# trinhvg/MoMA

Measured on AMD Instinct MI355X. Metric: images/sec MoMA train step (EffNet-B0 224px, K=65536), higher is better.
Workload: dtype bf16

## Files before the change

include/moma_hip.h:

```cpp
#ifndef MOMA_HIP_H
#define MOMA_HIP_H

#include <stddef.h>
#include <stdint.h>

#ifdef __cplusplus
extern "C" {
#endif

#define MOMA_ABI_VERSION 4

enum { MOMA_PREC_F32 = 0, MOMA_PREC_BF16 = 1 };
enum { MOMA_DT_F32 = 0, MOMA_DT_BF16 = 1 };

enum {
    MOMA_OK = 0,
    MOMA_E_NULL = -1,
    MOMA_E_SHAPE = -2,
    MOMA_E_DTYPE = -3,
    MOMA_E_ALIGN = -4,
    MOMA_E_WORKSPACE = -5,
    MOMA_E_UNSUPPORTED = -6
};

typedef void* moma_stream_t;

int moma_version(void);
const char* moma_error_string(int code);
int moma_debug_set_k2_target_wg(int n);

#define MOMA_EMA_BLOCK_ELEMS 4096
int moma_ema_multi(const int64_t* table, int n_tensors, int64_t total_blocks,
                   float m, float one_minus_m, moma_stream_t stream);

int moma_enqueue(void* queue, const float* rows, int n, int64_t index, int K, int d,
                 int qdtype, moma_stream_t stream);
int moma_enqueue_mirror(float* queue, void* mirror_bf16, const float* rows, int n, int64_t index, int K, int d,
                        moma_stream_t stream);

int moma_queue_prefetch(const void* queue, size_t bytes, moma_stream_t stream);

int moma_infonce_logits(const float* q, const float* k, const void* queue, float* out,
                        int B, int d, int K, float inv_T, int qdtype, int prec, moma_stream_t stream);
int moma_infonce_logits_bwd(const float* dlogits, const float* k, const void* queue, float* dq,
                            int B, int d, int K, float inv_T, int qdtype, int prec,
                            moma_stream_t stream);
size_t moma_infonce_logits_bwd_workspace_bytes(int B, int d, int K);
int moma_infonce_logits_bwd_ws(const float* dlogits, const float* k, const void* queue, float* dq,
                               int B, int d, int K, float inv_T, int qdtype, int prec,
                               void* workspace, size_t workspace_bytes, moma_stream_t stream);
int moma_infonce_logits_bwd_kq(const float* dlogits, const float* q, float* dk, float* dqueue,
                               int B, int d, int K, float inv_T, int prec, moma_stream_t stream);
size_t moma_infonce_fused_workspace_bytes(int B, int d, int K, int qdtype, int prec);
int moma_infonce_fused(const float* q, const float* k, const void* queue, int B, int d, int K,
                       float inv_T, float* loss_rows, float* lse, int32_t* top1, float* dq,
                       void* workspace, size_t workspace_bytes, int qdtype, int prec,
                       moma_stream_t stream);
int moma_infonce_fused_ex(const float* q, const float* k, const void* queue, int B, int d, int K,
                          float inv_T, float* loss_rows, float* lse, int32_t* top1, float* dq,
                          void* workspace, size_t workspace_bytes, int qdtype, int prec,
                          moma_stream_t stream, void* ev_begin, void* ev_end);
size_t moma_infonce_qpack_bytes(int B, int d);
int moma_infonce_fused_q(const float* q, const void* q_packed, const float* k, const void* queue, int B, int d, int K,
                         float inv_T, float* loss_rows, float* lse, int32_t* top1, float* dq,
                         void* workspace, size_t workspace_bytes, int qdtype, int prec,
                         moma_stream_t stream, void* ev_begin, void* ev_end, void* ev_call_end);
int moma_infonce_fused_enqueue(const float* q, const void* q_packed, const float* k, void* queue, int B, int d, int K,
                               float inv_T, float* loss_rows, float* lse, int32_t* top1, float* dq, void* workspace,
                               size_t workspace_bytes, int qdtype, int prec, const float* rows, int n, int64_t index,
                               float* queue_f32, moma_stream_t stream, void* ev_begin, void* ev_end, void* ev_call_end);

typedef struct moma_infonce_term {
    const float* q;
    const float* k;
    const void* queue;
    float* loss_rows;
    float* lse;
    int32_t* top1;
    float* dq;
} moma_infonce_term_t;
size_t moma_infonce_fused_multi_workspace_bytes(int n_terms, int B, int d, int K, int qdtype, int prec);
int moma_infonce_fused_multi(const moma_infonce_term_t* terms, int n_terms, int B, int d, int K, float inv_T,
                             void* workspace, size_t workspace_bytes, int qdtype, int prec, moma_stream_t stream);

size_t moma_crd_workspace_bytes(int B, int d, int K1);
int moma_crd_fused(const float* v1, const float* v2, const float* memory_v1, const float* memory_v2, const int64_t* idx,
                   int B, int d, int K1, int64_t n_data, float T, float* Z, int set_z, float* loss, float* dv1, float* dv2,
                   int32_t* bad_index, void* workspace, size_t workspace_bytes, moma_stream_t stream);
int moma_crd_scores(const float* v1, const float* v2, const float* memory_v1, const float* memory_v2, const int64_t* idx,
                    int B, int d, int K1, int64_t n_data, float T, float* Z, int set_z, float* out_v1, float* out_v2,
                    int32_t* bad_index, void* workspace, size_t workspace_bytes, moma_stream_t stream);
int moma_crd_scores_bwd(const float* dout_v1, const float* dout_v2, const float* out_v1, const float* out_v2,
                        const float* memory_v1, const float* memory_v2, const int64_t* idx, int B, int d, int K1,
                        int64_t n_data, float T, float* dv1, float* dv2, int32_t* bad_index, void* workspace,
                        size_t workspace_bytes, moma_stream_t stream);
int moma_crd_update(float* memory_v1, float* memory_v2, const float* v1, const float* v2, const int64_t* y, int B, int d,
                    int64_t n_data, float momentum, int32_t* bad_index, moma_stream_t stream);

enum { MOMA_LAYOUT_NCHW = 0, MOMA_LAYOUT_NHWC = 1 };
size_t moma_at_workspace_bytes(int B, int C, int H, int W, int oh, int ow, int dtype, int layout);
int moma_at_map(const void* f, float* a, int B, int C, int H, int W, int oh, int ow, int dtype, int layout, void* workspace,
                size_t workspace_bytes, moma_stream_t stream);
int moma_at_pair(const float* a_s, const float* a_t, int B, int n, float* norms, float* partials, float* loss, float* g_s,
                 float* g_t, float* ah_s, float* ah_t, moma_stream_t stream);
int moma_at_bwd(const void* f, const float* g_a, const float* g_loss, void* dF, int B, int C, int H, int W, int oh, int ow,
                int dtype, int layout, moma_stream_t stream);

enum { MOMA_MHA_SAVE_PROBS = 0, MOMA_MHA_SAVE_LSE = 1 };
int moma_mha_saved_state(int N, int d, int H, int prec);
int moma_mha_fwd(const float* x, const float* w_qkv, const float* b_qkv, const float* w_proj,
                 const float* b_proj, float* y, float* qkv, float* probs, float* attn_out,
                 int N, int d, int H, int prec, moma_stream_t stream);
size_t moma_mha_bwd_workspace_bytes(int N, int d, int H, int prec);
int moma_mha_bwd(const float* x, const float* w_qkv, const float* w_proj, const float* qkv,
                 const float* probs, const float* attn_out, const float* dy, float* dx,
                 float* dw_qkv, float* db_qkv, float* dw_proj, float* db_proj, void* workspace,
                 size_t workspace_bytes, int N, int d, int H, int prec, moma_stream_t stream);

typedef struct moma_mha_module {
    const void* x;
    const void* pack;
    const float* b_qkv;
    const float* b_proj;
    float* y;
    void* qkv16;
    void* attn16;
    float* lse;
    void* qpack;
    float qpack_scale;
    int x_dtype;
} moma_mha_module_t;
size_t moma_mha_pack_bytes(int d);
int moma_mha_pack_weights(const float* w_qkv, const float* w_proj, void* pack, int d, int with_transposed,
                          moma_stream_t stream);
int moma_mha_fwd_fast(const moma_mha_module_t* modules, int n_modules, int N, int d, int H, moma_stream_t stream);
size_t moma_mha_bwd_fast_workspace_bytes(int N, int d, int H);
int moma_mha_bwd_fast(const void* pack, const void* x, int x_dtype, const void* qkv16, const void* attn16, const float* lse,
                      const float* dy, float* dx, float* dw_qkv, float* db_qkv, float* dw_proj, float* db_proj,
                      void* workspace, size_t workspace_bytes, int N, int d, int H, moma_stream_t stream);

enum { MOMA_ACT_NONE = 0, MOMA_ACT_SILU = 1, MOMA_ACT_RELU = 2 };
size_t moma_bn_workspace_bytes(int C);
int moma_bn_fwd(const void* x, void* out, const float* gamma, const float* beta, float* running_mean,
                float* running_var, float* save_mean, float* save_invstd, void* workspace,
                size_t workspace_bytes, int N, int C, int HW, int dtype, int act, int training,
                float momentum, float eps, void* plane_mean, moma_stream_t stream);
int moma_bn_bwd(const void* x, const void* dout, const float* gamma, const float* beta,
                const float* save_mean, const float* save_invstd, void* dx, float* dgamma, float* dbeta,
                void* workspace, size_t workspace_bytes, int N, int C, int HW, int dtype, int act,
                int training, const void* dplane_mean, moma_stream_t stream);

size_t moma_dwconv_workspace_bytes(int C, int K);
int moma_dwconv_fwd(const void* x, const float* w, void* y, int N, int C, int H, int W, int OH, int OW,
                    int K, int stride, int pad_top, int pad_left, int dtype, moma_stream_t stream);
int moma_dwconv_bwd_data(const void* dy, const float* w, void* dx, int N, int C, int H, int W, int OH,
                         int OW, int K, int stride, int pad_top, int pad_left, int dtype,
                         moma_stream_t stream);
int moma_dwconv_bwd_weight(const void* x, const void* dy, float* dw, void* workspace,
                           size_t workspace_bytes, int N, int C, int H, int W, int OH, int OW, int K,
                           int stride, int pad_top, int pad_left, int dtype, moma_stream_t stream);

int moma_plane_mean(const void* x, void* mean, int NC, int HW, int dtype, moma_stream_t stream);
int moma_se_gate_fwd(const void* x, const void* s, void* out, int NC, int HW, int dtype, moma_stream_t stream);
int moma_se_gate_bwd(const void* x, const void* s, const void* dout, void* dx, void* ds, int NC, int HW,
                     int dtype, moma_stream_t stream);

#ifdef __cplusplus
}
#endif
#endif
```

moma_amd/_lib.py:

```python
from __future__ import annotations

import ctypes as C
import os

_HERE = os.path.dirname(os.path.abspath(__file__))
LIB_PATH = os.environ.get("MOMA_HIP_LIB", os.path.join(_HERE, "lib", "libmoma_hip.so"))

PREC_F32, PREC_BF16 = 0, 1
DT_F32, DT_BF16 = 0, 1
LAYOUT_NCHW, LAYOUT_NHWC = 0, 1
MHA_SAVE_PROBS, MHA_SAVE_LSE = 0, 1
ABI_VERSION = 4
EMA_BLOCK_ELEMS = 4096

_p = C.c_void_p
_i = C.c_int
_l = C.c_int64
_f = C.c_float
_z = C.c_size_t

SIGNATURES = {
    "moma_version": (_i, []),
    "moma_error_string": (C.c_char_p, [_i]),
    "moma_debug_set_k2_target_wg": (_i, [_i]),
    "moma_ema_multi": (_i, [_p, _i, _l, _f, _f, _p]),
    "moma_enqueue": (_i, [_p, _p, _i, _l, _i, _i, _i, _p]),
    "moma_enqueue_mirror": (_i, [_p, _p, _p, _i, _l, _i, _i, _p]),
    "moma_queue_prefetch": (_i, [_p, _z, _p]),
    "moma_infonce_logits": (_i, [_p, _p, _p, _p, _i, _i, _i, _f, _i, _i, _p]),
    "moma_infonce_logits_bwd": (_i, [_p, _p, _p, _p, _i, _i, _i, _f, _i, _i, _p]),
    "moma_infonce_logits_bwd_workspace_bytes": (_z, [_i, _i, _i]),
    "moma_infonce_logits_bwd_ws": (_i, [_p, _p, _p, _p, _i, _i, _i, _f, _i, _i, _p, _z, _p]),
    "moma_infonce_logits_bwd_kq": (_i, [_p, _p, _p, _p, _i, _i, _i, _f, _i, _p]),
    "moma_infonce_fused_workspace_bytes": (_z, [_i, _i, _i, _i, _i]),
    "moma_infonce_fused": (_i, [_p, _p, _p, _i, _i, _i, _f, _p, _p, _p, _p, _p, _z, _i, _i, _p]),
    "moma_infonce_fused_ex": (_i, [_p, _p, _p, _i, _i, _i, _f, _p, _p, _p, _p, _p, _z, _i, _i, _p, _p, _p]),
    "moma_infonce_qpack_bytes": (_z, [_i, _i]),
    "moma_infonce_fused_q": (_i, [_p, _p, _p, _p, _i, _i, _i, _f, _p, _p, _p, _p, _p, _z, _i, _i, _p, _p, _p, _p]),
    "moma_infonce_fused_enqueue": (_i, [_p, _p, _p, _p, _i, _i, _i, _f, _p, _p, _p, _p, _p, _z, _i, _i, _p, _i, _l, _p, _p, _p, _p, _p]),
    "moma_infonce_fused_multi_workspace_bytes": (_z, [_i, _i, _i, _i, _i, _i]),
    "moma_infonce_fused_multi": (_i, [_p, _i, _i, _i, _i, _f, _p, _z, _i, _i, _p]),
    "moma_crd_workspace_bytes": (_z, [_i, _i, _i]),
    "moma_crd_fused": (_i, [_p, _p, _p, _p, _p, _i, _i, _i, _l, _f, _p, _i, _p, _p, _p, _p, _p, _z, _p]),
    "moma_crd_scores": (_i, [_p, _p, _p, _p, _p, _i, _i, _i, _l, _f, _p, _i, _p, _p, _p, _p, _z, _p]),
    "moma_crd_scores_bwd": (_i, [_p, _p, _p, _p, _p, _p, _p, _i, _i, _i, _l, _f, _p, _p, _p, _p, _z, _p]),
    "moma_crd_update": (_i, [_p, _p, _p, _p, _p, _i, _i, _l, _f, _p, _p]),
    "moma_at_workspace_bytes": (_z, [_i] * 8),
    "moma_at_map": (_i, [_p, _p] + [_i] * 8 + [_p, _z, _p]),
    "moma_at_pair": (_i, [_p, _p, _i, _i, _p, _p, _p, _p, _p, _p, _p, _p]),
    "moma_at_bwd": (_i, [_p, _p, _p, _p] + [_i] * 8 + [_p]),
    "moma_mha_fwd": (_i,[_p, _p, _p, _p, _p, _p, _p, _p, _p, _i, _i, _i, _i, _p]),
    "moma_mha_saved_state": (_i, [_i, _i, _i, _i]),
    "moma_mha_pack_bytes": (_z, [_i]),
    "moma_mha_pack_weights": (_i, [_p, _p, _p, _i, _i, _p]),
    "moma_mha_fwd_fast": (_i, [_p, _i, _i, _i, _i, _p]),
    "moma_mha_bwd_fast_workspace_bytes": (_z, [_i, _i, _i]),
    "moma_mha_bwd_fast": (_i, [_p, _p, _i, _p, _p, _p, _p, _p, _p, _p, _p, _p, _p, _z, _i, _i, _i, _p]),
    "moma_dwconv_workspace_bytes": (_z, [_i, _i]),
    "moma_dwconv_fwd": (_i, [_p, _p, _p] + [_i] * 11 + [_p]),
    "moma_dwconv_bwd_data": (_i, [_p, _p, _p] + [_i] * 11 + [_p]),
    "moma_dwconv_bwd_weight": (_i, [_p, _p, _p, _p, _z] + [_i] * 11 + [_p]),
    "moma_plane_mean": (_i, [_p, _p, _i, _i, _i, _p]),
    "moma_se_gate_fwd": (_i, [_p, _p, _p, _i, _i, _i, _p]),
    "moma_se_gate_bwd": (_i, [_p, _p, _p, _p, _p, _i, _i, _i, _p]),
    "moma_bn_workspace_bytes": (_z, [_i]),
    "moma_bn_fwd": (_i, [_p, _p, _p, _p, _p, _p, _p, _p, _p, _z, _i, _i, _i, _i, _i, _i, _f, _f, _p, _p]),
    "moma_bn_bwd": (_i, [_p, _p, _p, _p, _p, _p, _p, _p, _p, _p, _z, _i, _i, _i, _i, _i, _i, _p, _p]),
    "moma_mha_bwd_workspace_bytes": (_z, [_i, _i, _i, _i]),
    "moma_mha_bwd": (_i, [_p, _p, _p, _p, _p, _p, _p, _p, _p, _p, _p, _p, _p, _z, _i, _i, _i, _i, _p]),
}



class InfoNCETerm(C.Structure):
    _fields_ = [("q", _p), ("k", _p), ("queue", _p), ("loss_rows", _p), ("lse", _p), ("top1", _p), ("dq", _p)]


class MhaModule(C.Structure):
    _fields_ = [("x", _p), ("pack", _p), ("b_qkv", _p), ("b_proj", _p), ("y", _p), ("qkv16", _p), ("attn16", _p),
                ("lse", _p), ("qpack", _p), ("qpack_scale", _f), ("x_dtype", _i)]


_lib = None


class MomaHipError(RuntimeError):
    pass


def load():
    global _lib
    if _lib is not None:
        return _lib
    import torch
    if not os.path.exists(LIB_PATH):
        raise MomaHipError(
            f"libmoma_hip.so not found at {LIB_PATH}: build it with `python -m moma_amd.build` "
            "(hipcc --offload-arch=gfx950). There is no CPU fallback for the MoMA hot path.")
    lib = C.CDLL(LIB_PATH)
    for name, (res, args) in SIGNATURES.items():
        try:
            fn = getattr(lib, name)
        except AttributeError as e:
            raise MomaHipError(f"{LIB_PATH} does not export {name}") from e
        fn.restype = res
        fn.argtypes = args
    v = lib.moma_version()
    if v != ABI_VERSION:
        raise MomaHipError(f"libmoma_hip ABI version {v} != binding version {ABI_VERSION}; rebuild")
    _lib = lib
    return lib


def check(rc: int, what: str):
    if rc != 0:
        msg = load().moma_error_string(rc)
        raise MomaHipError(f"{what} failed: rc={rc} ({msg.decode() if msg else '?'})")
```

moma_amd/backbones/efficientnet.py:

```python
import math
import os

import torch
import torch.nn as nn
import torch.nn.functional as F

_DW_MODE = os.environ.get("MOMA_DW", "hip")
_BN_MODE = os.environ.get("MOMA_BN", "hip")
_SE_MODE = os.environ.get("MOMA_SE", "hip")

_B0_STAGES = [
    (1, 3, 1, 1, 32, 16, 0.25),
    (2, 3, 2, 6, 16, 24, 0.25),
    (2, 5, 2, 6, 24, 40, 0.25),
    (3, 3, 2, 6, 40, 80, 0.25),
    (3, 5, 1, 6, 80, 112, 0.25),
    (4, 5, 2, 6, 112, 192, 0.25),
    (1, 3, 1, 6, 192, 320, 0.25),
]
_BN_MOM, _BN_EPS = 0.01, 1e-3


class _DepthwiseNative(torch.autograd.Function):

    @staticmethod
    def forward(ctx, x, w, stride, padding, groups):
        w = w.to(x.dtype)
        with torch.backends.cudnn.flags(enabled=False):
            y = F.conv2d(x, w, None, stride, padding, 1, groups)
        ctx.save_for_backward(x, w)
        ctx.cfg = (stride, padding, groups)
        return y

    @staticmethod
    def backward(ctx, gy):
        x, w = ctx.saved_tensors
        stride, padding, groups = ctx.cfg
        pad = padding if isinstance(padding, (tuple, list)) else (padding, padding)
        with torch.backends.cudnn.flags(enabled=False):
            gx, gw, _ = torch.ops.aten.convolution_backward(
                gy.contiguous(), x, w, None, list(stride), list(pad), [1, 1], False, [0, 0], groups,
                [ctx.needs_input_grad[0], ctx.needs_input_grad[1], False])
        return gx, (gw.float() if gw is not None else None), None, None, None


class _CachedCast(torch.autograd.Function):

    @staticmethod
    def forward(ctx, master, cached):
        ctx.dtype = master.dtype
        return cached.view_as(cached)

    @staticmethod
    def backward(ctx, g):
        return g.to(ctx.dtype), None


_WCACHE = os.environ.get("MOMA_WCACHE", "1") == "1"


class SamePadConv2d(nn.Conv2d):

    def __init__(self, cin, cout, kernel_size, stride=1, groups=1, bias=True):
        super().__init__(cin, cout, kernel_size, stride=stride, padding=0, groups=groups, bias=bias)
        self._wc = self._bc = None
        self._wc_live = False

    def _params(self, x):
        if self._wc_live and x.is_cuda and x.dtype == torch.bfloat16:
            track = torch.is_grad_enabled()
            w = _CachedCast.apply(self.weight, self._wc) if (track and self.weight.requires_grad) else self._wc
            b = None
            if self.bias is not None:
                b = _CachedCast.apply(self.bias, self._bc) if (track and self.bias.requires_grad) else self._bc
            return w, b
        return self.weight, self.bias

    def forward(self, x):
        ih, iw = x.shape[-2:]
        kh, kw = self.kernel_size
        sh, sw = self.stride
        ph = max((math.ceil(ih / sh) - 1) * sh + kh - ih, 0)
        pw = max((math.ceil(iw / sw) - 1) * sw + kw - iw, 0)
        depthwise = self.groups > 1 and self.groups == self.in_channels == self.out_channels and self.bias is None
        if depthwise and x.is_cuda and _DW_MODE == "hip" and kh == kw and sh == sw and self.dilation == (1, 1):
            from .. import ops
            if ops.dwconv_supported(kh, sh):
                if torch.is_autocast_enabled():
                    x = x.to(torch.get_autocast_dtype("cuda"))
                if x.dtype in (torch.float32, torch.bfloat16):
                    return ops.dwconv(x, self.weight, sh, ph // 2, pw // 2, math.ceil(ih / sh), math.ceil(iw / sw))
        pad = (ph // 2, pw // 2)
        if ph % 2 or pw % 2:
            x = F.pad(x, [pw // 2, pw - pw // 2, ph // 2, ph - ph // 2])
            pad = 0
        if depthwise and x.is_cuda and _DW_MODE in ("hip", "aten"):
            if torch.is_autocast_enabled():
                x = x.to(torch.get_autocast_dtype("cuda"))
            return _DepthwiseNative.apply(x, self.weight, self.stride, pad, self.groups)
        if self._wc_live and torch.is_autocast_enabled() and x.is_cuda and x.dtype != torch.bfloat16 and \
                torch.get_autocast_dtype("cuda") == torch.bfloat16:
            x = x.to(torch.bfloat16)
        w, b = self._params(x)
        return F.conv2d(x, w, b, self.stride, pad, self.dilation, self.groups)


class BatchNorm2d(nn.BatchNorm2d):

    _nbt_pending = 0

    def _flush_nbt(self):
        if self._nbt_pending and self.num_batches_tracked is not None:
            self.num_batches_tracked.add_(self._nbt_pending)
        self._nbt_pending = 0

    def _save_to_state_dict(self, destination, prefix, keep_vars):
        self._flush_nbt()
        super()._save_to_state_dict(destination, prefix, keep_vars)

    def _load_from_state_dict(self, *args, **kwargs):
        self._nbt_pending = 0
        super()._load_from_state_dict(*args, **kwargs)

    def forward(self, x, act=None, want_mean=False):
        if _BN_MODE == "hip" and x.is_cuda and x.dtype in (torch.float32, torch.bfloat16) and self.momentum is not None:
            from .. import ops
            use_batch = self.training or self.running_mean is None
            if self.training and self.track_running_stats and self.num_batches_tracked is not None:
                self._nbt_pending += 1
            return ops.bn_act(x, self.weight, self.bias, self.running_mean, self.running_var, use_batch,
                              self.momentum, self.eps, act, want_mean)
        if _BN_MODE == "aten" and x.is_cuda:
            with torch.backends.cudnn.flags(enabled=False):
                y = super().forward(x)
        else:
            y = super().forward(x)
        y = F.silu(y) if act == "silu" else (F.relu(y) if act == "relu" else y)
        return (y, F.adaptive_avg_pool2d(y, 1)) if want_mean else y


def _drop_connect(x, p, training):
    if not training or not p:
        return x
    keep = 1.0 - p
    mask = torch.floor(keep + torch.rand([x.shape[0], 1, 1, 1], dtype=x.dtype, device=x.device))
    return x / keep * mask


class MBConvBlock(nn.Module):
    def __init__(self, kernel, stride, expand, cin, cout, se_ratio):
        super().__init__()
        mid = cin * expand
        self.expand, self.stride, self.cin, self.cout = expand, stride, cin, cout
        if expand != 1:
            self._expand_conv = SamePadConv2d(cin, mid, 1, bias=False)
            self._bn0 = BatchNorm2d(mid, momentum=_BN_MOM, eps=_BN_EPS)
        self._depthwise_conv = SamePadConv2d(mid, mid, kernel, stride=stride, groups=mid, bias=False)
        self._bn1 = BatchNorm2d(mid, momentum=_BN_MOM, eps=_BN_EPS)
        sq = max(1, int(cin * se_ratio))
        self._se_reduce = SamePadConv2d(mid, sq, 1)
        self._se_expand = SamePadConv2d(sq, mid, 1)
        self._project_conv = SamePadConv2d(mid, cout, 1, bias=False)
        self._bn2 = BatchNorm2d(cout, momentum=_BN_MOM, eps=_BN_EPS)

    def forward(self, x, drop_connect_rate=None):
        inp = x
        if self.expand != 1:
            x = self._bn0(self._expand_conv(x), act="silu")
        x, pooled = self._bn1(self._depthwise_conv(x), act="silu", want_mean=True)
        s = self._se_expand(F.silu(self._se_reduce(pooled)))
        if _SE_MODE == "hip" and x.is_cuda and x.dtype in (torch.float32, torch.bfloat16):
            from .. import ops
            x = ops.se_gate(x, s)
        else:
            x = torch.sigmoid(s) * x
        x = self._bn2(self._project_conv(x))
        if self.stride == 1 and self.cin == self.cout:
            x = _drop_connect(x, drop_connect_rate, self.training) + inp
        return x


class EfficientNet(nn.Module):
    def __init__(self, num_classes=1000, dropout_rate=0.2, drop_connect_rate=0.2, in_channels=3):
        super().__init__()
        self.drop_connect_rate = drop_connect_rate
        self._conv_stem = SamePadConv2d(in_channels, 32, 3, stride=2, bias=False)
        self._bn0 = BatchNorm2d(32, momentum=_BN_MOM, eps=_BN_EPS)
        blocks = []
        for rep, k, s, e, cin, cout, se in _B0_STAGES:
            blocks.append(MBConvBlock(k, s, e, cin, cout, se))
            blocks += [MBConvBlock(k, 1, e, cout, cout, se) for _ in range(rep - 1)]
        self._blocks = nn.ModuleList(blocks)
        self._conv_head = SamePadConv2d(320, 1280, 1, bias=False)
        self._bn1 = BatchNorm2d(1280, momentum=_BN_MOM, eps=_BN_EPS)
        self._avg_pooling = nn.AdaptiveAvgPool2d(1)
        self.classifier_ = nn.Sequential(nn.Dropout(dropout_rate), nn.Linear(1280, num_classes))
        for m in self.modules():
            if isinstance(m, nn.Conv2d):
                nn.init.kaiming_normal_(m.weight, mode="fan_out")
                if m.bias is not None:
                    nn.init.zeros_(m.bias)
            elif isinstance(m, nn.BatchNorm2d):
                nn.init.ones_(m.weight)
                nn.init.zeros_(m.bias)
            elif isinstance(m, nn.Linear):
                nn.init.normal_(m.weight, 0, 0.01)
                nn.init.zeros_(m.bias)

    def extract_endpoints(self, x):
        feats = []
        x = self._bn0(self._conv_stem(x), act="silu")
        prev = x
        nb = len(self._blocks)
        for i, blk in enumerate(self._blocks):
            rate = self.drop_connect_rate * float(i) / nb if self.drop_connect_rate else self.drop_connect_rate
            x = blk(x, drop_connect_rate=rate)
            if prev.size(2) > x.size(2):
                feats.append(prev)
            prev = x
        feats.append(self._bn1(self._conv_head(x), act="silu"))
        return feats

    def get_feat_modules(self):
        return nn.ModuleList([self._conv_stem, self._bn0, self._blocks, self._conv_head, self._bn1, self.classifier_])

    def _refresh_weight_cache(self, x):
        live = (_WCACHE and x.is_cuda and torch.is_autocast_enabled() and torch.get_autocast_dtype("cuda") == torch.bfloat16)
        convs = getattr(self, "_wcache_convs", None)
        if convs is None:
            convs = [m for m in self.modules() if isinstance(m, SamePadConv2d) and not (m.groups > 1 and _DW_MODE == "hip")]
            object.__setattr__(self, "_wcache_convs", convs)
        if not live:
            for m in convs:
                m._wc_live = False
            return
        src, dst = [], []
        for m in convs:
            if m._wc is None or m._wc.device != m.weight.device:
                m._wc = torch.empty_like(m.weight, dtype=torch.bfloat16)
                m._bc = torch.empty_like(m.bias, dtype=torch.bfloat16) if m.bias is not None else None
            src.append(m.weight.detach()); dst.append(m._wc)
            if m.bias is not None:
                src.append(m.bias.detach()); dst.append(m._bc)
            m._wc_live = True
        with torch.no_grad():
            torch._foreach_copy_(dst, src)

    def forward(self, x, is_feat=False):
        self._refresh_weight_cache(x)
        out = self.extract_endpoints(x)
        pooled = self._avg_pooling(out[-1])
        out.append(pooled)
        logits = self.classifier_(pooled.flatten(start_dim=1))
        for m in self._wcache_convs:
            m._wc_live = False
        return (out, logits) if is_feat else logits


def efficientnet_b0(num_classes=1000, **kw):
    return EfficientNet(num_classes=num_classes, **kw)
```

moma_amd/csrc/api.hip:

```cpp
#include "common.hpp"

using namespace moma;

namespace {
inline int hip_rc(hipError_t e) { return e == hipSuccess ? MOMA_OK : (int)e; }
inline bool bad_prec(int p) { return p != MOMA_PREC_F32 && p != MOMA_PREC_BF16; }
inline bool bad_dt(int t) { return t != MOMA_DT_F32 && t != MOMA_DT_BF16; }
inline bool misaligned(const void* p, size_t a) { return ((uintptr_t)p % a) != 0; }
inline size_t align_up(size_t x, size_t a) { return (x + a - 1) / a * a; }

#define MOMA_TRY(expr)                         \
    do {                                       \
        hipError_t _e = (expr);                \
        if (_e != hipSuccess) return (int)_e;  \
    } while (0)

GemmArgs gemm(const float* A, const void* B, float* C, int M, int N, int K, long lda, long ldb, long ldc, int tA,
              int tB, float alpha, int prec) {
    GemmArgs g{};
    g.A = A; g.B = B; g.C = C; g.bias = nullptr;
    g.M = M; g.N = N; g.K = K; g.lda = lda; g.ldb = ldb; g.ldc = ldc;
    g.strideA = g.strideB = g.strideC = 0; g.batch = 1;
    g.transA = tA; g.transB = tB; g.alpha = alpha; g.splitk = 1; g.atomic = 0; g.splitC = 0;
    g.b_dtype = MOMA_DT_F32; g.prec = prec;
// ... 134 lines not shown
    }
    return MOMA_OK;
}

static bool f32_policy_widens_queue(int B, int d, int K, int qdtype, int prec) {
    return prec == MOMA_PREC_F32 && qdtype == MOMA_DT_BF16 && infonce_f32_flash_supported(B, d, K, MOMA_DT_F32, prec);
}

size_t moma_infonce_fused_workspace_bytes(int B, int d, int K, int qdtype, int prec) {
    if (B <= 0 || d <= 0 || K <= 0) return 0;
    if (infonce_flash_supported(B, d, K, qdtype, prec)) return infonce_flash_workspace_bytes(B, d, K);
    if (infonce_f32_flash_supported(B, d, K, qdtype, prec)) return infonce_f32_flash_workspace_bytes(B, d, K);
    if (f32_policy_widens_queue(B, d, K, qdtype, prec))
        return align_up((size_t)K * d * sizeof(float), 256) + infonce_f32_flash_workspace_bytes(B, d, K);
    return align_up((size_t)B * ((size_t)K + 1) * sizeof(float), 256) + logits_bwd_parts_bytes(B, d, K);
}

int moma_infonce_fused(const float* q, const float* k, const void* queue, int B, int d, int K, float inv_T,
                       float* loss_rows, float* lse, int32_t* top1, float* dq, void* workspace,
                       size_t workspace_bytes, int qdtype, int prec, moma_stream_t stream) {
    return moma_infonce_fused_ex(q, k, queue, B, d, K, inv_T, loss_rows, lse, top1, dq, workspace, workspace_bytes,
                                 qdtype, prec, stream, nullptr, nullptr);
}

int moma_infonce_fused_ex(const float* q, const float* k, const void* queue, int B, int d, int K, float inv_T,
                          float* loss_rows, float* lse, int32_t* top1, float* dq, void* workspace,
                          size_t workspace_bytes, int qdtype, int prec, moma_stream_t stream, void* ev_begin,
                          void* ev_end) {
    return moma_infonce_fused_q(q, nullptr, k, queue, B, d, K, inv_T, loss_rows, lse, top1, dq, workspace, workspace_bytes,
                                qdtype, prec, stream, ev_begin, ev_end, nullptr);
}

size_t moma_infonce_qpack_bytes(int B, int d) { return infonce_qpack_bytes(B, d); }

static int fused_impl(const float* q, const void* q_packed, const float* k, const void* queue, int B, int d, int K,
                      float inv_T, float* loss_rows, float* lse, int32_t* top1, float* dq, void* workspace,
                      size_t workspace_bytes, int qdtype, int prec, moma_stream_t stream, void* ev_begin, void* ev_end,
                      void* ev_call_end, const EnqueueJob* job, int* carried) {
    if (carried) *carried = 0;
    if (!q || !k || !queue || !loss_rows || !lse || !top1 || !workspace) return MOMA_E_NULL;
    if (B <= 0 || d <= 0 || K <= 0) return MOMA_E_SHAPE;
    if (bad_dt(qdtype) || bad_prec(prec)) return MOMA_E_DTYPE;
    if (workspace_bytes < moma_infonce_fused_workspace_bytes(B, d, K, qdtype, prec)) return MOMA_E_WORKSPACE;
    if (misaligned(workspace, 16)) return MOMA_E_ALIGN;
    hipStream_t st = (hipStream_t)stream;
    if (q_packed && (misaligned(q_packed, 16) || infonce_qpack_bytes(B, d) == 0 || !infonce_flash_supported(B, d, K, qdtype, prec)))
        return q_packed && misaligned(q_packed, 16) ? MOMA_E_ALIGN : MOMA_E_UNSUPPORTED;
    const bool one_pass = infonce_flash_supported(B, d, K, qdtype, prec) || infonce_f32_flash_supported(B, d, K, qdtype, prec) ||
                          f32_policy_widens_queue(B, d, K, qdtype, prec);
    if (one_pass && (misaligned(q, 16) || misaligned(k, 16) || misaligned(queue, 16) || (dq && misaligned(dq, 16)))) return MOMA_E_ALIGN;
    if (!one_pass && (misaligned(q, 4) || misaligned(k, 4) || misaligned(queue, qdtype == MOMA_DT_BF16 ? 2 : 4) || (dq && misaligned(dq, 4))))
        return MOMA_E_ALIGN;
    if (infonce_flash_supported(B, d, K, qdtype, prec)) {
        if (carried) *carried = 1;
        return hip_rc(launch_infonce_flash(q, k, queue, B, d, K, inv_T, loss_rows, lse, top1, dq, workspace, qdtype, st,
                                           (hipEvent_t)ev_begin, (hipEvent_t)ev_end, q_packed, (hipEvent_t)ev_call_end, job));
    }
    if (infonce_f32_flash_supported(B, d, K, qdtype, prec))
    {
        const int rc = hip_rc(launch_infonce_f32_flash(q, k, (const float*)queue, B, d, K, inv_T, loss_rows, lse, top1, dq, workspace, st,
                                                       (hipEvent_t)ev_begin, (hipEvent_t)ev_end));
        if (ev_call_end) (void)hipEventRecord((hipEvent_t)ev_call_end, st);
        return rc;
    }
    if (f32_policy_widens_queue(B, d, K, qdtype, prec)) {
        if (misaligned(queue, 16)) return MOMA_E_ALIGN;
        float* wide = (float*)workspace;
        void* ws2 = (char*)workspace + align_up((size_t)K * d * sizeof(float), 256);
        if (ev_begin) (void)hipEventRecord((hipEvent_t)ev_begin, st);
        MOMA_TRY(launch_widen_bf16(queue, wide, (size_t)K * d, st));
        const int rc = hip_rc(launch_infonce_f32_flash(q, k, wide, B, d, K, inv_T, loss_rows, lse, top1, dq, ws2, st,
                                                       (hipEvent_t) nullptr, (hipEvent_t)ev_end));
        if (ev_call_end) (void)hipEventRecord((hipEvent_t)ev_call_end, st);
        return rc;
    }
    float* logits = (float*)workspace;
    if (ev_begin) (void)hipEventRecord((hipEvent_t)ev_begin, st);
    int rc = moma_infonce_logits(q, k, queue, logits, B, d, K, inv_T, qdtype, prec, stream);
    if (ev_end) (void)hipEventRecord((hipEvent_t)ev_end, st);
    if (rc != MOMA_OK) return rc;
    MOMA_TRY(launch_infonce_rows(logits, B, K + 1, loss_rows, lse, top1, dq != nullptr, st));
    if (dq) {
        float* parts = (float*)((char*)workspace + align_up((size_t)B * ((size_t)K + 1) * sizeof(float), 256));
        rc = logits_bwd_impl(logits, k, queue, dq, B, d, K, inv_T, qdtype, prec, st, logits_bwd_parts_bytes(B, d, K) ? parts : nullptr);
    }
    if (ev_call_end) (void)hipEventRecord((hipEvent_t)ev_call_end, st);
    return rc;
}

int moma_infonce_fused_q(const float* q, const void* q_packed, const float* k, const void* queue, int B, int d, int K,
                         float inv_T, float* loss_rows, float* lse, int32_t* top1, float* dq, void* workspace,
                         size_t workspace_bytes, int qdtype, int prec, moma_stream_t stream, void* ev_begin, void* ev_end,
                         void* ev_call_end) {
    return fused_impl(q, q_packed, k, queue, B, d, K, inv_T, loss_rows, lse, top1, dq, workspace, workspace_bytes, qdtype, prec, stream,
                      ev_begin, ev_end, ev_call_end, nullptr, nullptr);
}

int moma_infonce_fused_enqueue(const float* q, const void* q_packed, const float* k, void* queue, int B, int d, int K,
                               float inv_T, float* loss_rows, float* lse, int32_t* top1, float* dq, void* workspace,
                               size_t workspace_bytes, int qdtype, int prec, const float* rows, int n, int64_t index,
                               float* queue_f32, moma_stream_t stream, void* ev_begin, void* ev_end, void* ev_call_end) {
    if (n < 0 || K <= 0 || index < 0 || index >= K) return MOMA_E_SHAPE;
    if (n > 0 && !rows) return MOMA_E_NULL;
    if (bad_dt(qdtype)) return MOMA_E_DTYPE;
    if (queue_f32 && qdtype != MOMA_DT_BF16) return MOMA_E_DTYPE;
    if (n > 0 && (misaligned(rows, 4) || misaligned(queue, qdtype == MOMA_DT_BF16 ? 2 : 4) || (queue_f32 && misaligned(queue_f32, 4))))
        return MOMA_E_ALIGN;
    EnqueueJob job{qdtype == MOMA_DT_BF16 ? queue : nullptr, qdtype == MOMA_DT_BF16 ? queue_f32 : (float*)queue, rows, n, index, K, d};
    int carried = 0;
    const int rc = fused_impl(q, q_packed, k, queue, B, d, K, inv_T, loss_rows, lse, top1, dq, workspace, workspace_bytes, qdtype, prec,
                              stream, ev_begin, ev_end, ev_call_end, n > 0 ? &job : nullptr, &carried);
    if (rc != MOMA_OK || carried || n == 0) return rc;
    if (queue_f32) return hip_rc(launch_enqueue_mirror(queue_f32, queue, rows, n, index, K, d, (hipStream_t)stream));
    return hip_rc(launch_enqueue(queue, rows, n, index, K, d, qdtype, (hipStream_t)stream));
}

size_t moma_infonce_fused_multi_workspace_bytes(int n_terms, int B, int d, int K, int qdtype, int prec) {
    if (n_terms < 1 || n_terms > 4 || B <= 0 || d <= 0 || K <= 0 || bad_dt(qdtype) || bad_prec(prec)) return 0;
    if (infonce_multi_supported(n_terms, B, d, K, qdtype, prec)) return infonce_multi_workspace_bytes(n_terms, B, d, K);
    return moma_infonce_fused_workspace_bytes(B, d, K, qdtype, prec);
}

int moma_infonce_fused_multi(const moma_infonce_term_t* terms, int n_terms, int B, int d, int K, float inv_T, void* workspace,
                             size_t workspace_bytes, int qdtype, int prec, moma_stream_t stream) {
    if (!terms || !workspace) return MOMA_E_NULL;
    if (n_terms < 1 || n_terms > 4 || B <= 0 || d <= 0 || K <= 0) return MOMA_E_SHAPE;
    if (bad_dt(qdtype) || bad_prec(prec)) return MOMA_E_DTYPE;
    for (int i = 0; i < n_terms; ++i) {
        const moma_infonce_term_t& t = terms[i];
        if (!t.q || !t.k || !t.queue || !t.loss_rows || !t.lse || !t.top1) return MOMA_E_NULL;
        if ((t.dq != nullptr) != (terms[0].dq != nullptr)) return MOMA_E_UNSUPPORTED;
        if (misaligned(t.q, 16) || misaligned(t.k, 4) || misaligned(t.queue, 16)) return MOMA_E_ALIGN;
    }
    if (workspace_bytes < moma_infonce_fused_multi_workspace_bytes(n_terms, B, d, K, qdtype, prec)) return MOMA_E_WORKSPACE;
    if (misaligned(workspace, 16)) return MOMA_E_ALIGN;
    if (infonce_multi_supported(n_terms, B, d, K, qdtype, prec))
        return hip_rc(launch_infonce_multi(terms, n_terms, B, d, K, inv_T, workspace, (hipStream_t)stream));
    for (int i = 0; i < n_terms; ++i) {
        const moma_infonce_term_t& t = terms[i];
        const int rc = moma_infonce_fused_q(t.q, nullptr, t.k, t.queue, B, d, K, inv_T, t.loss_rows, t.lse, t.top1, t.dq, workspace,
                                            workspace_bytes, qdtype, prec, stream, nullptr, nullptr, nullptr);
        if (rc != MOMA_OK) return rc;
    }
    return MOMA_OK;
}

int moma_mha_saved_state(int N, int d, int H, int prec) {
    if (N <= 0 || d <= 0 || H <= 0 || d % H != 0 || bad_prec(prec)) return MOMA_E_SHAPE;
    return mha_fast_supported(N, d, H, prec) ? MOMA_MHA_SAVE_LSE : MOMA_MHA_SAVE_PROBS;
}

int moma_mha_fwd(const float* x, const float* w_qkv, const float* b_qkv, const float* w_proj, const float* b_proj,
                 float* y, float* qkv, float* probs, float* attn_out, int N, int d, int H, int prec,
                 moma_stream_t stream) {
    if (!x || !w_qkv || !w_proj || !b_proj || !y || !qkv || !attn_out || !probs) return MOMA_E_NULL;
    if (N <= 0 || d <= 0 || H <= 0 || d % H != 0) return MOMA_E_SHAPE;
    if (bad_prec(prec)) return MOMA_E_DTYPE;
    hipStream_t st = (hipStream_t)stream;
    const int hd = d / H;
    const float scale = 1.0f / sqrtf((float)hd);
    GemmArgs g = gemm(x, w_qkv, qkv, N, 3 * d, d, d, d, 3L * d, 0, 0, 1.f, prec);
    g.bias = b_qkv;
    MOMA_TRY(launch_gemm(g, st));
    g = gemm(qkv, qkv + d, probs, N, N, hd, 3L * d, 3L * d, N, 0, 0, scale, prec);
    g.batch = H; g.strideA = hd; g.strideB = hd; g.strideC = (long)N * N;
    MOMA_TRY(launch_gemm(g, st));
    MOMA_TRY(launch_softmax_rows(probs, (long)H * N, N, st));
    g = gemm(probs, qkv + 2 * d, attn_out, N, hd, N, N, 3L * d, d, 0, 1, 1.f, prec);
    g.batch = H; g.strideA = (long)N * N; g.strideB = hd; g.strideC = hd;
    MOMA_TRY(launch_gemm(g, st));
    g = gemm(attn_out, w_proj, y, N, d, d, d, d, d, 0, 0, 1.f, prec);
    g.bias = b_proj;
    return hip_rc(launch_gemm(g, st));
}

size_t moma_mha_bwd_workspace_bytes(int N, int d, int H, int prec) {
    if (N <= 0 || d <= 0 || H <= 0 || d % H != 0 || bad_prec(prec)) return 0;
    return align_up(((size_t)N * d + (size_t)H * N * N + (size_t)N * 3 * d) * sizeof(float), 256);
}

int moma_mha_bwd(const float* x, const float* w_qkv, const float* w_proj, const float* qkv, const float* probs,
                 const float* attn_out, const float* dy, float* dx, float* dw_qkv, float* db_qkv,
                 float* dw_proj, float* db_proj, void* workspace, size_t workspace_bytes, int N, int d, int H, int prec,
                 moma_stream_t stream) {
    if (!x || !w_qkv || !w_proj || !qkv || !attn_out || !dy || !workspace || !probs) return MOMA_E_NULL;
    if (N <= 0 || d <= 0 || H <= 0 || d % H != 0) return MOMA_E_SHAPE;
    if (bad_prec(prec)) return MOMA_E_DTYPE;
    if (workspace_bytes < moma_mha_bwd_workspace_bytes(N, d, H, prec)) return MOMA_E_WORKSPACE;
    if (misaligned(workspace, 16)) return MOMA_E_ALIGN;
    hipStream_t st = (hipStream_t)stream;
    const int hd = d / H;
    const float scale = 1.0f / sqrtf((float)hd);
    float* dA = (float*)workspace;
    float* dP = dA + (size_t)N * d;
    float* dqkv = dP + (size_t)H * N * N;
    GemmArgs g;
    bool db_done = false;
    if (dw_proj) {
        g = gemm(dy, attn_out, dw_proj, d, d, N, d, d, d, 1, 1, 1.f, prec);
        if (db_proj && gemm_fuses_colsum(g)) { g.colsum_a = db_proj; db_done = true; }
        MOMA_TRY(launch_gemm(g, st));
    }
    if (db_proj && !db_done) MOMA_TRY(launch_colsum(dy, db_proj, N, d, d, st));
    g = gemm(dy, w_proj, dA, N, d, d, d, d, d, 0, 1, 1.f, prec);
    MOMA_TRY(launch_gemm(g, st));
    g = gemm(probs, dA, dqkv + 2 * d, N, hd, N, N, d, 3L * d, 1, 1, 1.f, prec);
    g.batch = H; g.strideA = (long)N * N; g.strideB = hd; g.strideC = hd;
    MOMA_TRY(launch_gemm(g, st));
    g = gemm(dA, qkv + 2 * d, dP, N, N, hd, d, 3L * d, N, 0, 0, 1.f, prec);
    g.batch = H; g.strideA = hd; g.strideB = hd; g.strideC = (long)N * N;
    MOMA_TRY(launch_gemm(g, st));
    MOMA_TRY(launch_softmax_bwd_rows(probs, dP, (long)H * N, N, scale, st));
    g = gemm(dP, qkv + d, dqkv, N, hd, N, N, 3L * d, 3L * d, 0, 1, 1.f, prec);
    g.batch = H; g.strideA = (long)N * N; g.strideB = hd; g.strideC = hd;
    MOMA_TRY(launch_gemm(g, st));
    g = gemm(dP, qkv, dqkv + d, N, hd, N, N, 3L * d, 3L * d, 1, 1, 1.f, prec);
    g.batch = H; g.strideA = (long)N * N; g.strideB = hd; g.strideC = hd;
    MOMA_TRY(launch_gemm(g, st));
    db_done = false;
    if (dw_qkv) {
        g = gemm(dqkv, x, dw_qkv, 3 * d, d, N, 3L * d, d, d, 1, 1, 1.f, prec);
        if (db_qkv && gemm_fuses_colsum(g)) { g.colsum_a = db_qkv; db_done = true; }
        MOMA_TRY(launch_gemm(g, st));
    }
    if (db_qkv && !db_done) MOMA_TRY(launch_colsum(dqkv, db_qkv, N, 3 * d, 3L * d, st));
    if (dx) {
        g = gemm(dqkv, w_qkv, dx, N, d, 3 * d, 3L * d, d, d, 0, 1, 1.f, prec);
        MOMA_TRY(launch_gemm(g, st));
    }
    return MOMA_OK;
}

size_t moma_mha_pack_bytes(int d) { return d > 0 ? (size_t)16 * d * d : 0; }

int moma_mha_pack_weights(const float* w_qkv, const float* w_proj, void* pack, int d, int with_transposed,
                          moma_stream_t stream) {
    if (!w_qkv || !w_proj || !pack) return MOMA_E_NULL;
    if (d <= 0 || d % 16 != 0) return MOMA_E_SHAPE;
    if (misaligned(pack, 16) || misaligned(w_qkv, 4) || misaligned(w_proj, 4)) return MOMA_E_ALIGN;
    return hip_rc(launch_mha_pack(w_qkv, w_proj, pack, d, with_transposed != 0, (hipStream_t)stream));
}

int moma_mha_fwd_fast(const moma_mha_module_t* mods, int n_modules, int N, int d, int H, moma_stream_t stream) {
    if (!mods) return MOMA_E_NULL;
    if (n_modules < 1 || n_modules > 4 || N <= 0 || d <= 0 || H <= 0 || d % H != 0) return MOMA_E_SHAPE;
    if (!mha_fast_supported(N, d, H, MOMA_PREC_BF16)) return MOMA_E_UNSUPPORTED;
    for (int i = 0; i < n_modules; ++i) {
        const moma_mha_module_t& m = mods[i];
        if (!m.x || !m.pack || !m.b_proj || !m.y || !m.qkv16 || !m.attn16) return MOMA_E_NULL;
        if (bad_dt(m.x_dtype)) return MOMA_E_DTYPE;
        if (misaligned(m.x, 16) || misaligned(m.pack, 16) || misaligned(m.y, 16) || misaligned(m.qkv16, 16) ||
            misaligned(m.attn16, 16) || misaligned(m.b_proj, 16) || (m.b_qkv && misaligned(m.b_qkv, 16)) ||
            (m.qpack && misaligned(m.qpack, 16)))
            return MOMA_E_ALIGN;
    }
    return hip_rc(launch_mha_fwd_fast(mods, n_modules, N, d, H, (hipStream_t)stream));
}

size_t moma_mha_bwd_fast_workspace_bytes(int N, int d, int H) {
    if (N <= 0 || d <= 0 || H <= 0 || d % H != 0) return 0;
    return mha_bwd_fast_workspace_bytes(N, d);
}

int moma_mha_bwd_fast(const void* pack, const void* x, int x_dtype, const void* qkv16, const void* attn16, const float* lse,
                      const float* dy, float* dx, float* dw_qkv, float* db_qkv, float* dw_proj, float* db_proj,
                      void* workspace, size_t workspace_bytes, int N, int d, int H, moma_stream_t stream) {
    if (!pack || !x || !qkv16 || !attn16 || !lse || !dy || !workspace) return MOMA_E_NULL;
    if (N <= 0 || d <= 0 || H <= 0 || d % H != 0) return MOMA_E_SHAPE;
    if (!mha_fast_supported(N, d, H, MOMA_PREC_BF16)) return MOMA_E_UNSUPPORTED;
    if (bad_dt(x_dtype)) return MOMA_E_DTYPE;
    if ((db_qkv && !dw_qkv) || (db_proj && !dw_proj)) return MOMA_E_UNSUPPORTED;
    if (workspace_bytes < mha_bwd_fast_workspace_bytes(N, d)) return MOMA_E_WORKSPACE;
    if (misaligned(workspace, 16) || misaligned(pack, 16) || misaligned(x, 16) || misaligned(qkv16, 16) ||
        misaligned(attn16, 16) || misaligned(dy, 16) || (dx && misaligned(dx, 16)) || (dw_qkv && misaligned(dw_qkv, 8)) ||
        (dw_proj && misaligned(dw_proj, 8)))
        return MOMA_E_ALIGN;
    return hip_rc(launch_mha_bwd_fast(pack, x, x_dtype, qkv16, attn16, lse, dy, dx, dw_qkv, db_qkv, dw_proj, db_proj, workspace, N, d,
                                      H, (hipStream_t)stream));
}

size_t moma_bn_workspace_bytes(int C) { return C > 0 ? align_up(bn_workspace_floats(C) * sizeof(float), 256) : 0; }

static int bn_check(int N, int C, int HW, int dtype, int act, const void* ws, size_t ws_bytes) {
    if (N <= 0 || C <= 0 || HW <= 0 || (long)N * C > 0x7fffffffL || (long)N * HW > 0x7fffffffL) return MOMA_E_SHAPE;
    if (dtype != MOMA_DT_F32 && dtype != MOMA_DT_BF16) return MOMA_E_DTYPE;
    if (act != MOMA_ACT_NONE && act != MOMA_ACT_SILU && act != MOMA_ACT_RELU) return MOMA_E_DTYPE;
    if (!ws) return MOMA_E_NULL;
    if (ws_bytes < moma_bn_workspace_bytes(C)) return MOMA_E_WORKSPACE;
    return MOMA_OK;
}

int moma_bn_fwd(const void* x, void* out, const float* gamma, const float* beta, float* running_mean,
                float* running_var, float* save_mean, float* save_invstd, void* workspace, size_t workspace_bytes,
                int N, int C, int HW, int dtype, int act, int training, float momentum, float eps, void* plane_mean,
                moma_stream_t stream) {
    if (!x || !out) return MOMA_E_NULL;
    if (!training && (!running_mean || !running_var)) return MOMA_E_NULL;
    const int rc = bn_check(N, C, HW, dtype, act, workspace, workspace_bytes);
    if (rc != MOMA_OK) return rc;
    return hip_rc(launch_bn_fwd(x, out, gamma, beta, running_mean, running_var, save_mean, save_invstd,
                                (float*)workspace, N, C, HW, dtype, act, training, momentum, eps, plane_mean, (hipStream_t)stream));
}

int moma_bn_bwd(const void* x, const void* dout, const float* gamma, const float* beta, const float* save_mean,
                const float* save_invstd, void* dx, float* dgamma, float* dbeta, void* workspace,
                size_t workspace_bytes, int N, int C, int HW, int dtype, int act, int training,
                const void* dplane_mean, moma_stream_t stream) {
    if (!x || !dout || !save_mean || !save_invstd) return MOMA_E_NULL;
    const int rc = bn_check(N, C, HW, dtype, act, workspace, workspace_bytes);
    if (rc != MOMA_OK) return rc;
    return hip_rc(launch_bn_bwd(x, dout, gamma, beta, save_mean, save_invstd, dx, dgamma, dbeta, (float*)workspace, N,
                                C, HW, dtype, act, training, dplane_mean, (hipStream_t)stream));
}

size_t moma_dwconv_workspace_bytes(int C, int K) {
    return (C > 0 && K > 0) ? align_up(dwconv_workspace_floats(C, K) * sizeof(float), 256) : 0;
}

static int dw_check(int N, int C, int H, int W, int OH, int OW, int K, int S, int pt, int pl, int dtype) {
    if (N <= 0 || C <= 0 || H <= 0 || W <= 0 || OH <= 0 || OW <= 0 || (long)N * C > 0x7fffffffL) return MOMA_E_SHAPE;
    if (!dwconv_supported(K, S)) return MOMA_E_SHAPE;
    if (pt < 0 || pl < 0 || pt >= K || pl >= K) return MOMA_E_SHAPE;
    if ((long)(OH - 1) * S - pt >= H || (long)(OW - 1) * S - pl >= W) return MOMA_E_SHAPE;
    if (dtype != MOMA_DT_F32 && dtype != MOMA_DT_BF16) return MOMA_E_DTYPE;
    return MOMA_OK;
}

int moma_dwconv_fwd(const void* x, const float* w, void* y, int N, int C, int H, int W, int OH, int OW, int K, int stride,
                    int pad_top, int pad_left, int dtype, moma_stream_t stream) {
    if (!x || !w || !y) return MOMA_E_NULL;
    const int rc = dw_check(N, C, H, W, OH, OW, K, stride, pad_top, pad_left, dtype);
    if (rc != MOMA_OK) return rc;
    return hip_rc(launch_dw_fwd(x, w, y, N, C, H, W, OH, OW, K, stride, pad_top, pad_left, dtype, (hipStream_t)stream));
}

int moma_dwconv_bwd_data(const void* dy, const float* w, void* dx, int N, int C, int H, int W, int OH, int OW, int K,
                         int stride, int pad_top, int pad_left, int dtype, moma_stream_t stream) {
    if (!dy || !w || !dx) return MOMA_E_NULL;
    const int rc = dw_check(N, C, H, W, OH, OW, K, stride, pad_top, pad_left, dtype);
    if (rc != MOMA_OK) return rc;
    return hip_rc(launch_dw_bwd_data(dy, w, dx, N, C, H, W, OH, OW, K, stride, pad_top, pad_left, dtype, (hipStream_t)stream));
}

int moma_dwconv_bwd_weight(const void* x, const void* dy, float* dw, void* workspace, size_t workspace_bytes, int N, int C,
                           int H, int W, int OH, int OW, int K, int stride, int pad_top, int pad_left, int dtype,
                           moma_stream_t stream) {
    if (!x || !dy || !dw || !workspace) return MOMA_E_NULL;
    const int rc = dw_check(N, C, H, W, OH, OW, K, stride, pad_top, pad_left, dtype);
    if (rc != MOMA_OK) return rc;
    if (workspace_bytes < moma_dwconv_workspace_bytes(C, K)) return MOMA_E_WORKSPACE;
    return hip_rc(launch_dw_bwd_weight(x, dy, dw, (float*)workspace, workspace_bytes / sizeof(float), N, C, H, W, OH, OW, K,
                                       stride, pad_top, pad_left, dtype, (hipStream_t)stream));
}

static int se_check(int NC, int HW, int dtype) {
    if (NC <= 0 || HW <= 0) return MOMA_E_SHAPE;
    if (dtype != MOMA_DT_F32 && dtype != MOMA_DT_BF16) return MOMA_E_DTYPE;
    return MOMA_OK;
}
int moma_plane_mean(const void* x, void* mean, int NC, int HW, int dtype, moma_stream_t stream) {
    if (!x || !mean) return MOMA_E_NULL;
    const int rc = se_check(NC, HW, dtype);
    return rc != MOMA_OK ? rc : hip_rc(launch_plane_mean(x, mean, NC, HW, dtype, (hipStream_t)stream));
}
int moma_se_gate_fwd(const void* x, const void* s, void* out, int NC, int HW, int dtype, moma_stream_t stream) {
    if (!x || !s || !out) return MOMA_E_NULL;
    const int rc = se_check(NC, HW, dtype);
    return rc != MOMA_OK ? rc : hip_rc(launch_se_gate_fwd(x, s, out, NC, HW, dtype, (hipStream_t)stream));
}
int moma_se_gate_bwd(const void* x, const void* s, const void* dout, void* dx, void* ds, int NC, int HW, int dtype,
                     moma_stream_t stream) {
    if (!x || !s || !dout || !dx || !ds) return MOMA_E_NULL;
    const int rc = se_check(NC, HW, dtype);
    return rc != MOMA_OK ? rc : hip_rc(launch_se_gate_bwd(x, s, dout, dx, ds, NC, HW, dtype, (hipStream_t)stream));
}

static int crd_check(int B, int d, int K1, int64_t n_data, float T) {
    if (B <= 0 || d < 4 || d % 4 != 0 || K1 < 2 || n_data <= 0 || !(T > 0.f)) return MOMA_E_SHAPE;
    if (d > 2048 || B > 65535) return MOMA_E_UNSUPPORTED;
    return MOMA_OK;
}
static bool crd_misaligned(const void* a, const void* b, const void* c, const void* d, const void* e = nullptr,
                           const void* f = nullptr, const void* g = nullptr, const void* h = nullptr) {
    return misaligned(a, 16) || misaligned(b, 16) || misaligned(c, 16) || misaligned(d, 16) || misaligned(e, 16) ||
           misaligned(f, 16) || misaligned(g, 16) || misaligned(h, 16);
}

size_t moma_crd_workspace_bytes(int B, int d, int K1) {
    if (crd_check(B, d, K1, 1, 1.f) != MOMA_OK) return 0;
    return crd_workspace_bytes(B, d, K1);
}

int moma_crd_fused(const float* v1, const float* v2, const float* memory_v1, const float* memory_v2, const int64_t* idx,
                   int B, int d, int K1, int64_t n_data, float T, float* Z, int set_z, float* loss, float* dv1, float* dv2,
                   int32_t* bad_index, void* workspace, size_t workspace_bytes, moma_stream_t stream) {
    if (!v1 || !v2 || !memory_v1 || !memory_v2 || !idx || !Z || !loss || !bad_index || !workspace) return MOMA_E_NULL;
    if ((dv1 == nullptr) != (dv2 == nullptr)) return MOMA_E_NULL;
    const int rc = crd_check(B, d, K1, n_data, T);
    if (rc != MOMA_OK) return rc;
    if (crd_misaligned(v1, v2, memory_v1, memory_v2, dv1, dv2, workspace) || misaligned(idx, 8) || misaligned(Z, 4) ||
        misaligned(loss, 4) || misaligned(bad_index, 4))
        return MOMA_E_ALIGN;
    if (workspace_bytes < crd_workspace_bytes(B, d, K1)) return MOMA_E_WORKSPACE;
    return hip_rc(launch_crd_fused(v1, v2, memory_v1, memory_v2, idx, B, d, K1, n_data, T, Z, set_z, loss, dv1, dv2, bad_index,
                                   workspace, (hipStream_t)stream));
}

int moma_crd_scores(const float* v1, const float* v2, const float* memory_v1, const float* memory_v2, const int64_t* idx,
                    int B, int d, int K1, int64_t n_data, float T, float* Z, int set_z, float* out_v1, float* out_v2,
                    int32_t* bad_index, void* workspace, size_t workspace_bytes, moma_stream_t stream) {
    if (!v1 || !v2 || !memory_v1 || !memory_v2 || !idx || !Z || !out_v1 || !out_v2 || !bad_index || !workspace) return MOMA_E_NULL;
    const int rc = crd_check(B, d, K1, n_data, T);
    if (rc != MOMA_OK) return rc;
    if (crd_misaligned(v1, v2, memory_v1, memory_v2, workspace) || misaligned(idx, 8) || misaligned(Z, 4) ||
        misaligned(out_v1, 4) || misaligned(out_v2, 4) || misaligned(bad_index, 4))
        return MOMA_E_ALIGN;
    if (workspace_bytes < crd_workspace_bytes(B, d, K1)) return MOMA_E_WORKSPACE;
    return hip_rc(launch_crd_scores(v1, v2, memory_v1, memory_v2, idx, B, d, K1, n_data, T, Z, set_z, out_v1, out_v2, bad_index,
                                    workspace, (hipStream_t)stream));
}

int moma_crd_scores_bwd(const float* dout_v1, const float* dout_v2, const float* out_v1, const float* out_v2,
                        const float* memory_v1, const float* memory_v2, const int64_t* idx, int B, int d, int K1,
                        int64_t n_data, float T, float* dv1, float* dv2, int32_t* bad_index, void* workspace,
                        size_t workspace_bytes, moma_stream_t stream) {
    if (!dout_v1 || !dout_v2 || !out_v1 || !out_v2 || !memory_v1 || !memory_v2 || !idx || !dv1 || !dv2 || !bad_index || !workspace)
        return MOMA_E_NULL;
    const int rc = crd_check(B, d, K1, n_data, T);
    if (rc != MOMA_OK) return rc;
    if (crd_misaligned(memory_v1, memory_v2, dv1, dv2, workspace) || misaligned(idx, 8) || misaligned(dout_v1, 4) ||
        misaligned(dout_v2, 4) || misaligned(out_v1, 4) || misaligned(out_v2, 4) || misaligned(bad_index, 4))
        return MOMA_E_ALIGN;
    if (workspace_bytes < crd_workspace_bytes(B, d, K1)) return MOMA_E_WORKSPACE;
    return hip_rc(launch_crd_scores_bwd(dout_v1, dout_v2, out_v1, out_v2, memory_v1, memory_v2, idx, B, d, K1, n_data, T, dv1, dv2,
                                        bad_index, workspace, (hipStream_t)stream));
}

int moma_crd_update(float* memory_v1, float* memory_v2, const float* v1, const float* v2, const int64_t* y, int B, int d,
                    int64_t n_data, float momentum, int32_t* bad_index, moma_stream_t stream) {
    if (!memory_v1 || !memory_v2 || !v1 || !v2 || !y || !bad_index) return MOMA_E_NULL;
    if (B <= 0 || d <= 0 || n_data <= 0) return MOMA_E_SHAPE;
    if (d > 2048 || B > 65535) return MOMA_E_UNSUPPORTED;
    if (misaligned(memory_v1, 4) || misaligned(memory_v2, 4) || misaligned(v1, 4) || misaligned(v2, 4) || misaligned(y, 8) ||
        misaligned(bad_index, 4))
        return MOMA_E_ALIGN;
    return hip_rc(launch_crd_update(memory_v1, memory_v2, v1, v2, y, B, d, n_data, momentum, bad_index, (hipStream_t)stream));
}

static int at_check(int B, int C, int H, int W, int oh, int ow, int dtype, int layout) {
    if (B <= 0 || C <= 0 || H <= 0 || W <= 0 || oh <= 0 || ow <= 0) return MOMA_E_SHAPE;
    if (bad_dt(dtype)) return MOMA_E_DTYPE;
    if (layout != MOMA_LAYOUT_NCHW && layout != MOMA_LAYOUT_NHWC) return MOMA_E_UNSUPPORTED;
    if (H % oh != 0 || W % ow != 0) return MOMA_E_SHAPE;
    if ((int64_t)oh * ow > INT32_MAX / 8) return MOMA_E_UNSUPPORTED;
    return MOMA_OK;
}

size_t moma_at_workspace_bytes(int B, int C, int H, int W, int oh, int ow, int dtype, int layout) {
    if (at_check(B, C, H, W, oh, ow, dtype, layout) != MOMA_OK) return 0;
    return at_workspace_bytes(B, C, H, W, oh, ow, layout);
}

int moma_at_map(const void* f, float* a, int B, int C, int H, int W, int oh, int ow, int dtype, int layout, void* workspace,
                size_t workspace_bytes, moma_stream_t stream) {
    if (!f || !a) return MOMA_E_NULL;
    const int rc = at_check(B, C, H, W, oh, ow, dtype, layout);
    if (rc != MOMA_OK) return rc;
    const size_t need = at_workspace_bytes(B, C, H, W, oh, ow, layout);
    if (need != 0 && !workspace) return MOMA_E_NULL;
    if (workspace_bytes < need) return MOMA_E_WORKSPACE;
    if (misaligned(f, dtype == MOMA_DT_BF16 ? 2 : 4) || misaligned(a, 4) || (need != 0 && misaligned(workspace, 16))) return MOMA_E_ALIGN;
    return hip_rc(launch_at_map(f, a, B, C, H, W, oh, ow, dtype, layout, workspace, (hipStream_t)stream));
}

int moma_at_pair(const float* a_s, const float* a_t, int B, int n, float* norms, float* partials, float* loss, float* g_s,
                 float* g_t, float* ah_s, float* ah_t, moma_stream_t stream) {
    if (!a_s || !a_t || !norms || !partials || !loss) return MOMA_E_NULL;
    if (B <= 0 || n <= 0) return MOMA_E_SHAPE;
    if (misaligned(a_s, 4) || misaligned(a_t, 4) || misaligned(norms, 4) || misaligned(partials, 4) || misaligned(loss, 4) ||
        misaligned(g_s, 4) || misaligned(g_t, 4) || misaligned(ah_s, 4) || misaligned(ah_t, 4))
        return MOMA_E_ALIGN;
    return hip_rc(launch_at_pair(a_s, a_t, B, n, norms, partials, loss, g_s, g_t, ah_s, ah_t, (hipStream_t)stream));
}

int moma_at_bwd(const void* f, const float* g_a, const float* g_loss, void* dF, int B, int C, int H, int W, int oh, int ow,
                int dtype, int layout, moma_stream_t stream) {
    if (!f || !g_a || !g_loss || !dF) return MOMA_E_NULL;
    const int rc = at_check(B, C, H, W, oh, ow, dtype, layout);
    if (rc != MOMA_OK) return rc;
    const size_t eb = dtype == MOMA_DT_BF16 ? 2 : 4;
    if (misaligned(f, eb) || misaligned(dF, eb) || misaligned(g_a, 4) || misaligned(g_loss, 4)) return MOMA_E_ALIGN;
    return hip_rc(launch_at_bwd(f, g_a, g_loss, dF, B, C, H, W, oh, ow, dtype, layout, (hipStream_t)stream));
}

}
```

moma_amd/csrc/bn.hip:

```cpp
#include "common.hpp"

namespace moma {
namespace {

constexpr int BN_THREADS = 256;

template <typename T, int VEC>
struct VecIO;
template <int VEC>
struct VecIO<float, VEC> {
    __device__ static void load(const float* p, float (&v)[VEC]) {
        if constexpr (VEC == 8) {
            const float4 a = *reinterpret_cast<const float4*>(p), b = *reinterpret_cast<const float4*>(p + 4);
            v[0] = a.x; v[1] = a.y; v[2] = a.z; v[3] = a.w; v[4] = b.x; v[5] = b.y; v[6] = b.z; v[7] = b.w;
        } else if constexpr (VEC == 4) {
            const float4 a = *reinterpret_cast<const float4*>(p);
            v[0] = a.x; v[1] = a.y; v[2] = a.z; v[3] = a.w;
        } else {
            v[0] = *p;
        }
    }
    __device__ static void store(float* p, const float (&v)[VEC]) {
        if constexpr (VEC == 8) {
            *reinterpret_cast<float4*>(p) = make_float4(v[0], v[1], v[2], v[3]);
            *reinterpret_cast<float4*>(p + 4) = make_float4(v[4], v[5], v[6], v[7]);
        } else if constexpr (VEC == 4) {
            *reinterpret_cast<float4*>(p) = make_float4(v[0], v[1], v[2], v[3]);
        } else {
            *p = v[0];
        }
    }
};
template <int VEC>
struct VecIO<bf16_raw, VEC> {
    __device__ static void load(const bf16_raw* p, float (&v)[VEC]) {
        if constexpr (VEC == 8) {
            const uint4 a = *reinterpret_cast<const uint4*>(p);
            const unsigned w[4] = {a.x, a.y, a.z, a.w};
#pragma unroll
            for (int i = 0; i < 4; ++i) {
                v[2 * i] = __uint_as_float(w[i] << 16);
                v[2 * i + 1] = __uint_as_float(w[i] & 0xffff0000u);
            }
        } else if constexpr (VEC == 4) {
            const uint2 a = *reinterpret_cast<const uint2*>(p);
            v[0] = __uint_as_float(a.x << 16); v[1] = __uint_as_float(a.x & 0xffff0000u);
            v[2] = __uint_as_float(a.y << 16); v[3] = __uint_as_float(a.y & 0xffff0000u);
        } else {
            v[0] = bf16_to_f32(*p);
        }
    }
    __device__ static void store(bf16_raw* p, const float (&v)[VEC]) {
        if constexpr (VEC == 8) {
            uint4 a;
            a.x = (unsigned)f32_to_bf16(v[0]) | ((unsigned)f32_to_bf16(v[1]) << 16);
            a.y = (unsigned)f32_to_bf16(v[2]) | ((unsigned)f32_to_bf16(v[3]) << 16);
            a.z = (unsigned)f32_to_bf16(v[4]) | ((unsigned)f32_to_bf16(v[5]) << 16);
            a.w = (unsigned)f32_to_bf16(v[6]) | ((unsigned)f32_to_bf16(v[7]) << 16);
            *reinterpret_cast<uint4*>(p) = a;
        } else if constexpr (VEC == 4) {
            uint2 a;
            a.x = (unsigned)f32_to_bf16(v[0]) | ((unsigned)f32_to_bf16(v[1]) << 16);
            a.y = (unsigned)f32_to_bf16(v[2]) | ((unsigned)f32_to_bf16(v[3]) << 16);
            *reinterpret_cast<uint2*>(p) = a;
        } else {
            *p = f32_to_bf16(v[0]);
        }
    }
};

__device__ __forceinline__ float act_fwd(float y, int act) {
    if (act == MOMA_ACT_SILU) return y / (1.f + __expf(-y));
    if (act == MOMA_ACT_RELU) return fmaxf(y, 0.f);
    return y;
}
__device__ __forceinline__ float act_grad(float y, int act) {
    if (act == MOMA_ACT_SILU) {
        const float s = 1.f / (1.f + __expf(-y));
        return s * (1.f + y * (1.f - s));
    }
    if (act == MOMA_ACT_RELU) return y > 0.f ? 1.f : 0.f;
    return 1.f;
}

__device__ __forceinline__ void merge(float& n, float& mean, float& m2, float nb, float meanb, float m2b) {
    const float nn = n + nb;
    if (nn > 0.f) {
        const float delta = meanb - mean, f = nb / nn;
        mean += delta * f;
        m2 += m2b + delta * delta * n * f;
    }
    n = nn;
}

template <typename T, int VEC>
__global__ __launch_bounds__(BN_THREADS) void bn_stats_kernel(const T* __restrict__ x, float* __restrict__ partial,
                                                              int N, int C, int HW) {
    const int c = blockIdx.y, s = blockIdx.x, S = gridDim.x;
    const unsigned hwv = HW / VEC, total = (unsigned)N * hwv;
    float sum = 0.f, sq = 0.f, cnt = 0.f;
    for (unsigned i = s * BN_THREADS + threadIdx.x; i < total; i += S * BN_THREADS) {
        const unsigned n = i / hwv, r = i - n * hwv;
        float v[VEC];
        VecIO<T, VEC>::load(x + ((size_t)n * C + c) * HW + (size_t)r * VEC, v);
#pragma unroll
        for (int j = 0; j < VEC; ++j) {
            sum += v[j];
            sq = fmaf(v[j], v[j], sq);
        }
        cnt += (float)VEC;
    }
    float mean = cnt > 0.f ? sum / cnt : 0.f;
    float m2 = fmaxf(sq - sum * mean, 0.f);
#pragma unroll
    for (int o = 32; o > 0; o >>= 1) {
        const float nb = __shfl_xor(cnt, o, 64), mb = __shfl_xor(mean, o, 64), qb = __shfl_xor(m2, o, 64);
        merge(cnt, mean, m2, nb, mb, qb);
    }
    __shared__ float red[BN_THREADS / 64][3];
    const int lane = threadIdx.x & 63, w = threadIdx.x >> 6;
    if (lane == 0) { red[w][0] = cnt; red[w][1] = mean; red[w][2] = m2; }
    __syncthreads();
    if (threadIdx.x == 0) {
        for (int k = 1; k < BN_THREADS / 64; ++k) merge(cnt, mean, m2, red[k][0], red[k][1], red[k][2]);
        float* p = partial + ((size_t)c * S + s) * 3;
        p[0] = cnt; p[1] = mean; p[2] = m2;
    }
}

__global__ __launch_bounds__(256) void bn_finalize_kernel(const float* __restrict__ partial, int S,
                                                          const float* __restrict__ gamma, const float* __restrict__ beta,
                                                          float* __restrict__ running_mean, float* __restrict__ running_var,
                                                          float* __restrict__ save_mean, float* __restrict__ save_invstd,
                                                          float* __restrict__ scale_shift, int C, int training,
                                                          float momentum, float eps) {
    const int lane = threadIdx.x & 63, c = blockIdx.x * 4 + (threadIdx.x >> 6);
    if (c >= C) return;
    float mean, invstd;
    if (training) {
        float n = 0.f, m2 = 0.f;
        mean = 0.f;
        if (lane < S) {
            const float* p = partial + ((size_t)c * S + lane) * 3;
            n = p[0]; mean = p[1]; m2 = p[2];
        }
#pragma unroll
        for (int o = 32; o > 0; o >>= 1) {
            const float nb = __shfl_xor(n, o, 64), mb = __shfl_xor(mean, o, 64), qb = __shfl_xor(m2, o, 64);
            if (lane & o) {
                float n2 = nb, mean2 = mb, m22 = qb;
                merge(n2, mean2, m22, n, mean, m2);
                n = n2; mean = mean2; m2 = m22;
            } else {
                merge(n, mean, m2, nb, mb, qb);
            }
        }
        const float var = m2 / n;
        invstd = rsqrtf(var + eps);
        if (lane == 0) {
            if (running_mean) running_mean[c] = (1.f - momentum) * running_mean[c] + momentum * mean;
            if (running_var) running_var[c] = (1.f - momentum) * running_var[c] + momentum * (n > 1.f ? m2 / (n - 1.f) : var);
        }
    } else {
        mean = running_mean[c];
        invstd = rsqrtf(running_var[c] + eps);
    }
    if (lane == 0) {
        if (save_mean) save_mean[c] = mean;
        if (save_invstd) save_invstd[c] = invstd;
        const float g = gamma ? gamma[c] : 1.f, b = beta ? beta[c] : 0.f;
        scale_shift[2 * c] = g * invstd;
        scale_shift[2 * c + 1] = b - mean * g * invstd;
    }
}

template <typename T, int VEC>
__global__ __launch_bounds__(BN_THREADS) void bn_apply_kernel(const T* __restrict__ x, T* __restrict__ out,
                                                              const float* __restrict__ scale_shift, int C, int HW,
                                                              size_t nvec, int act) {
    const unsigned hwv = HW / VEC;
    for (size_t i = (size_t)blockIdx.x * BN_THREADS + threadIdx.x; i < nvec; i += (size_t)gridDim.x * BN_THREADS) {
        const unsigned plane = (unsigned)(i / hwv), c = plane % (unsigned)C;
        const float sc = scale_shift[2 * c], sh = scale_shift[2 * c + 1];
        float v[VEC];
        VecIO<T, VEC>::load(x + i * VEC, v);
#pragma unroll
        for (int j = 0; j < VEC; ++j) v[j] = act_fwd(fmaf(v[j], sc, sh), act);
        VecIO<T, VEC>::store(out + i * VEC, v);
    }
}

template <typename T, int VEC>
__global__ __launch_bounds__(BN_THREADS) void bn_apply_mean_kernel(const T* __restrict__ x, T* __restrict__ out,
                                                                   T* __restrict__ pmean,
                                                                   const float* __restrict__ scale_shift, int NC, int C,
                                                                   int HW, int act) {
    const int lane = threadIdx.x & 63;
    const int nv = HW / VEC;
    for (int plane = blockIdx.x * (BN_THREADS / 64) + (threadIdx.x >> 6); plane < NC; plane += gridDim.x * (BN_THREADS / 64)) {
        const int c = plane % C;
        const float sc = scale_shift[2 * c], sh = scale_shift[2 * c + 1];
        const T* p = x + (size_t)plane * HW;
        T* o = out + (size_t)plane * HW;
        float acc = 0.f;
        for (int i = lane; i < nv; i += 64) {
            float v[VEC];
            VecIO<T, VEC>::load(p + (size_t)i * VEC, v);
#pragma unroll
            for (int j = 0; j < VEC; ++j) {
                v[j] = act_fwd(fmaf(v[j], sc, sh), act);
                acc += v[j];
            }
            VecIO<T, VEC>::store(o + (size_t)i * VEC, v);
        }
        acc = wave_sum(acc);
        if (lane == 0) {
            float m[1] = {acc / (float)HW};
            VecIO<T, 1>::store(pmean + plane, m);
        }
    }
}

template <typename T, int VEC>
__global__ __launch_bounds__(BN_THREADS) void bn_bwd_reduce_kernel(const T* __restrict__ x, const T* __restrict__ dout,
                                                                   const float* __restrict__ gamma,
                                                                   const float* __restrict__ beta,
                                                                   const float* __restrict__ save_mean,
                                                                   const float* __restrict__ save_invstd,
                                                                   float* __restrict__ partial, int N, int C, int HW,
                                                                   int act, const T* __restrict__ dpl) {
    const int c = blockIdx.y, s = blockIdx.x, S = gridDim.x;
    const unsigned hwv = HW / VEC, total = (unsigned)N * hwv;
    const float mean = save_mean[c], invstd = save_invstd[c];
    const float g = gamma ? gamma[c] : 1.f, b = beta ? beta[c] : 0.f;
    const float inv_hw = 1.f / (float)HW;
    float s1 = 0.f, s2 = 0.f;
    for (unsigned i = s * BN_THREADS + threadIdx.x; i < total; i += S * BN_THREADS) {
        const unsigned n = i / hwv, r = i - n * hwv;
        const size_t off = ((size_t)n * C + c) * HW + (size_t)r * VEC;
        float xv[VEC], dv[VEC];
        VecIO<T, VEC>::load(x + off, xv);
        VecIO<T, VEC>::load(dout + off, dv);
        float add = 0.f;
        if (dpl) { float t1[1]; VecIO<T, 1>::load(dpl + (size_t)n * C + c, t1); add = t1[0] * inv_hw; }
#pragma unroll
        for (int j = 0; j < VEC; ++j) {
            const float xh = (xv[j] - mean) * invstd;
            const float dy = (dv[j] + add) * act_grad(fmaf(xh, g, b), act);
            s1 += dy;
            s2 = fmaf(dy, xh, s2);
        }
    }
    s1 = wave_sum(s1);
    s2 = wave_sum(s2);
    __shared__ float red[BN_THREADS / 64][2];
    const int lane = threadIdx.x & 63, w = threadIdx.x >> 6;
    if (lane == 0) { red[w][0] = s1; red[w][1] = s2; }
    __syncthreads();
    if (threadIdx.x == 0) {
        for (int k = 1; k < BN_THREADS / 64; ++k) { s1 += red[k][0]; s2 += red[k][1]; }
        partial[((size_t)c * S + s) * 2] = s1;
        partial[((size_t)c * S + s) * 2 + 1] = s2;
    }
}

__global__ __launch_bounds__(256) void bn_bwd_finalize_kernel(const float* __restrict__ partial, int S,
                                                              const float* __restrict__ gamma,
                                                              const float* __restrict__ save_invstd, float* __restrict__ dgamma,
                                                              float* __restrict__ dbeta, float* __restrict__ coef, int C,
                                                              float count, int training) {
    const int lane = threadIdx.x & 63, c = blockIdx.x * 4 + (threadIdx.x >> 6);
    if (c >= C) return;
    float s1 = 0.f, s2 = 0.f;
    if (lane < S) {
        s1 = partial[((size_t)c * S + lane) * 2];
        s2 = partial[((size_t)c * S + lane) * 2 + 1];
    }
    s1 = wave_sum(s1);
    s2 = wave_sum(s2);
    if (lane != 0) return;
    if (dgamma) dgamma[c] = s2;
    if (dbeta) dbeta[c] = s1;
    const float a = (gamma ? gamma[c] : 1.f) * save_invstd[c];
    coef[3 * c] = a;
    coef[3 * c + 1] = training ? s1 / count : 0.f;
    coef[3 * c + 2] = training ? s2 / count : 0.f;
}

template <typename T, int VEC>
__global__ __launch_bounds__(BN_THREADS) void bn_bwd_apply_kernel(const T* __restrict__ x, const T* __restrict__ dout,
                                                                  T* __restrict__ dx, const float* __restrict__ gamma,
                                                                  const float* __restrict__ beta,
                                                                  const float* __restrict__ save_mean,
                                                                  const float* __restrict__ save_invstd,
                                                                  const float* __restrict__ coef, int C, int HW,
                                                                  size_t nvec, int act, const T* __restrict__ dpl) {
    const unsigned hwv = HW / VEC;
    const float inv_hw = 1.f / (float)HW;
    for (size_t i = (size_t)blockIdx.x * BN_THREADS + threadIdx.x; i < nvec; i += (size_t)gridDim.x * BN_THREADS) {
        const unsigned plane = (unsigned)(i / hwv), c = plane % (unsigned)C;
        const float mean = save_mean[c], invstd = save_invstd[c];
        const float g = gamma ? gamma[c] : 1.f, b = beta ? beta[c] : 0.f;
        const float a = coef[3 * c], b1 = coef[3 * c + 1], b2 = coef[3 * c + 2];
        float xv[VEC], dv[VEC];
        VecIO<T, VEC>::load(x + i * VEC, xv);
        VecIO<T, VEC>::load(dout + i * VEC, dv);
        float add = 0.f;
        if (dpl) { float t1[1]; VecIO<T, 1>::load(dpl + plane, t1); add = t1[0] * inv_hw; }
#pragma unroll
        for (int j = 0; j < VEC; ++j) {
            const float xh = (xv[j] - mean) * invstd;
            const float dy = (dv[j] + add) * act_grad(fmaf(xh, g, b), act);
            xv[j] = a * (dy - b1 - xh * b2);
        }
        VecIO<T, VEC>::store(dx + i * VEC, xv);
    }
}

int pick_vec(int HW, int elem_bytes, const void* a, const void* b, const void* c) {
    const uintptr_t bits = (uintptr_t)a | (uintptr_t)b | (uintptr_t)c;
    if (HW % 8 == 0 && bits % (8 * elem_bytes) == 0) return 8;
    if (HW % 4 == 0 && bits % (4 * elem_bytes) == 0) return 4;
    return 1;
}
int pick_splits(int N, int C, int HW, int vec) {
    const long per_channel = (long)N * (HW / vec);
    long S = (4096 + C - 1) / C;
    const long max_s = (per_channel + BN_THREADS * 2 - 1) / (BN_THREADS * 2);
    if (S > max_s) S = max_s;
    if (S > 64) S = 64;
    if (S < 1) S = 1;
    return (int)S;
}
unsigned apply_grid(size_t nvec) {
    size_t g = (nvec + BN_THREADS * 4 - 1) / (BN_THREADS * 4);
    if (g > 256u * 64u) g = 256u * 64u;
    if (g < 1) g = 1;
    return (unsigned)g;
}

template <typename T>
hipError_t bn_fwd_t(const T* x, T* out, const float* gamma, const float* beta, float* rm, float* rv, float* save_mean,
                    float* save_invstd, float* ws, int N, int C, int HW, int act, int training, float momentum,
                    float eps, T* pmean, hipStream_t st) {
    const int vec = pick_vec(HW, sizeof(T), x, out, nullptr);
    const int S = training ? pick_splits(N, C, HW, vec) : 1;
    float* scale_shift = ws;
    float* partial = ws + 2 * (size_t)C;
    const size_t nvec = (size_t)N * C * HW / vec;
    if (training) {
        dim3 grid(S, C);
        if (vec == 8) hipLaunchKernelGGL((bn_stats_kernel<T, 8>), grid, dim3(BN_THREADS), 0, st, x, partial, N, C, HW);
        else if (vec == 4) hipLaunchKernelGGL((bn_stats_kernel<T, 4>), grid, dim3(BN_THREADS), 0, st, x, partial, N, C, HW);
        else hipLaunchKernelGGL((bn_stats_kernel<T, 1>), grid, dim3(BN_THREADS), 0, st, x, partial, N, C, HW);
    }
    hipLaunchKernelGGL(bn_finalize_kernel, dim3((C + 3) / 4), dim3(256), 0, st, partial, S, gamma, beta, rm, rv,
                       save_mean, save_invstd, scale_shift, C, training, momentum, eps);
    if (pmean) {
        long gp = ((long)N * C + BN_THREADS / 64 - 1) / (BN_THREADS / 64);
        if (gp > 256 * 32) gp = 256 * 32;
        const dim3 pg((unsigned)gp);
        if (vec == 8) hipLaunchKernelGGL((bn_apply_mean_kernel<T, 8>), pg, dim3(BN_THREADS), 0, st, x, out, pmean, scale_shift, N * C, C, HW, act);
        else if (vec == 4) hipLaunchKernelGGL((bn_apply_mean_kernel<T, 4>), pg, dim3(BN_THREADS), 0, st, x, out, pmean, scale_shift, N * C, C, HW, act);
        else hipLaunchKernelGGL((bn_apply_mean_kernel<T, 1>), pg, dim3(BN_THREADS), 0, st, x, out, pmean, scale_shift, N * C, C, HW, act);
        return hipGetLastError();
    }
    const unsigned g = apply_grid(nvec);
    if (vec == 8) hipLaunchKernelGGL((bn_apply_kernel<T, 8>), dim3(g), dim3(BN_THREADS), 0, st, x, out, scale_shift, C, HW, nvec, act);
    else if (vec == 4) hipLaunchKernelGGL((bn_apply_kernel<T, 4>), dim3(g), dim3(BN_THREADS), 0, st, x, out, scale_shift, C, HW, nvec, act);
    else hipLaunchKernelGGL((bn_apply_kernel<T, 1>), dim3(g), dim3(BN_THREADS), 0, st, x, out, scale_shift, C, HW, nvec, act);
    return hipGetLastError();
}

template <typename T>
hipError_t bn_bwd_t(const T* x, const T* dout, const float* gamma, const float* beta, const float* save_mean,
                    const float* save_invstd, T* dx, float* dgamma, float* dbeta, float* ws, int N, int C, int HW,
                    int act, int training, const T* dpl, hipStream_t st) {
    const int vec = pick_vec(HW, sizeof(T), x, dout, dx);
    const int S = pick_splits(N, C, HW, vec);
    float* coef = ws;
    float* partial = ws + 3 * (size_t)C;
    const size_t nvec = (size_t)N * C * HW / vec;
    dim3 grid(S, C);
    if (vec == 8) hipLaunchKernelGGL((bn_bwd_reduce_kernel<T, 8>), grid, dim3(BN_THREADS), 0, st, x, dout, gamma, beta, save_mean, save_invstd, partial, N, C, HW, act, dpl);
    else if (vec == 4) hipLaunchKernelGGL((bn_bwd_reduce_kernel<T, 4>), grid, dim3(BN_THREADS), 0, st, x, dout, gamma, beta, save_mean, save_invstd, partial, N, C, HW, act, dpl);
    else hipLaunchKernelGGL((bn_bwd_reduce_kernel<T, 1>), grid, dim3(BN_THREADS), 0, st, x, dout, gamma, beta, save_mean, save_invstd, partial, N, C, HW, act, dpl);
    hipLaunchKernelGGL(bn_bwd_finalize_kernel, dim3((C + 3) / 4), dim3(256), 0, st, partial, S, gamma, save_invstd,
                       dgamma, dbeta, coef, C, (float)N * (float)HW, training);
    if (dx) {
        const unsigned g = apply_grid(nvec);
        if (vec == 8) hipLaunchKernelGGL((bn_bwd_apply_kernel<T, 8>), dim3(g), dim3(BN_THREADS), 0, st, x, dout, dx, gamma, beta, save_mean, save_invstd, coef, C, HW, nvec, act, dpl);
        else if (vec == 4) hipLaunchKernelGGL((bn_bwd_apply_kernel<T, 4>), dim3(g), dim3(BN_THREADS), 0, st, x, dout, dx, gamma, beta, save_mean, save_invstd, coef, C, HW, nvec, act, dpl);
        else hipLaunchKernelGGL((bn_bwd_apply_kernel<T, 1>), dim3(g), dim3(BN_THREADS), 0, st, x, dout, dx, gamma, beta, save_mean, save_invstd, coef, C, HW, nvec, act, dpl);
    }
    return hipGetLastError();
}
}

size_t bn_workspace_floats(int C) { return (size_t)C * (3 + 64 * 3); }

hipError_t launch_bn_fwd(const void* x, void* out, const float* gamma, const float* beta, float* rm, float* rv,
                         float* save_mean, float* save_invstd, float* ws, int N, int C, int HW, int dtype, int act,
                         int training, float momentum, float eps, void* plane_mean, hipStream_t st) {
    if (dtype == MOMA_DT_BF16)
        return bn_fwd_t<bf16_raw>((const bf16_raw*)x, (bf16_raw*)out, gamma, beta, rm, rv, save_mean, save_invstd, ws, N,
                                  C, HW, act, training, momentum, eps, (bf16_raw*)plane_mean, st);
    return bn_fwd_t<float>((const float*)x, (float*)out, gamma, beta, rm, rv, save_mean, save_invstd, ws, N, C, HW, act,
                           training, momentum, eps, (float*)plane_mean, st);
}
hipError_t launch_bn_bwd(const void* x, const void* dout, const float* gamma, const float* beta, const float* save_mean,
                         const float* save_invstd, void* dx, float* dgamma, float* dbeta, float* ws, int N, int C, int HW,
                         int dtype, int act, int training, const void* dplane_mean, hipStream_t st) {
    if (dtype == MOMA_DT_BF16)
        return bn_bwd_t<bf16_raw>((const bf16_raw*)x, (const bf16_raw*)dout, gamma, beta, save_mean, save_invstd,
                                  (bf16_raw*)dx, dgamma, dbeta, ws, N, C, HW, act, training, (const bf16_raw*)dplane_mean, st);
    return bn_bwd_t<float>((const float*)x, (const float*)dout, gamma, beta, save_mean, save_invstd, (float*)dx, dgamma,
                           dbeta, ws, N, C, HW, act, training, (const float*)dplane_mean, st);
}

}
```

moma_amd/csrc/common.hpp:

```cpp
#pragma once
#include <hip/hip_runtime.h>
#include <stdint.h>
#include "../../include/moma_hip.h"

namespace moma {

typedef __attribute__((ext_vector_type(8))) __bf16 bf16x8;
typedef __attribute__((ext_vector_type(4))) __bf16 bf16x4;
typedef __attribute__((ext_vector_type(4))) float f32x4;
typedef __attribute__((ext_vector_type(16))) float f32x16;
typedef unsigned short bf16_raw;

constexpr int WAVE = 64;

__device__ __forceinline__ float bf16_to_f32(bf16_raw v) {
    return __uint_as_float(((unsigned)v) << 16);
}
__device__ __forceinline__ bf16_raw f32_to_bf16(float f) {
    __bf16 b = (__bf16)f;
    return *reinterpret_cast<bf16_raw*>(&b);
}

__device__ __forceinline__ unsigned pack_bf16x2(float lo, float hi) {
    unsigned r;
    asm("v_cvt_pk_bf16_f32 %0, %1, %2" : "=v"(r) : "v"(lo), "v"(hi));
    return r;
}

__device__ __forceinline__ float other_half(float v) {
    const unsigned u = __float_as_uint(v);
    const auto r = __builtin_amdgcn_permlane32_swap(u, u, false, false);
    return __uint_as_float((threadIdx.x & 32) ? r[0] : r[1]);
}

template <int CTRL>
__device__ __forceinline__ float dpp_row(float v) {
    return __uint_as_float((unsigned)__builtin_amdgcn_update_dpp(0, (int)__float_as_uint(v), CTRL, 0xf, 0xf, false));
}
__device__ __forceinline__ float half32_sum(float v) {
    v += dpp_row<0x128>(v);
    v += dpp_row<0x124>(v);
    v += dpp_row<0x122>(v);
    v += dpp_row<0x121>(v);
    const unsigned u = __float_as_uint(v);
    const auto r = __builtin_amdgcn_permlane16_swap(u, u, false, false);
    return __uint_as_float(r[0]) + __uint_as_float(r[1]);
}
__device__ __forceinline__ float half32_max(float v) {
    v = fmaxf(v, dpp_row<0x128>(v));
    v = fmaxf(v, dpp_row<0x124>(v));
    v = fmaxf(v, dpp_row<0x122>(v));
    v = fmaxf(v, dpp_row<0x121>(v));
    const unsigned u = __float_as_uint(v);
    const auto r = __builtin_amdgcn_permlane16_swap(u, u, false, false);
    return fmaxf(__uint_as_float(r[0]), __uint_as_float(r[1]));
}

__device__ __forceinline__ float wave_max(float v) {
#pragma unroll
    for (int o = 32; o > 0; o >>= 1) v = fmaxf(v, __shfl_xor(v, o, 64));
    return v;
}
__device__ __forceinline__ float wave_sum(float v) {
#pragma unroll
    for (int o = 32; o > 0; o >>= 1) v += __shfl_xor(v, o, 64);
    return v;
}

template <typename T, int VEC> struct PV;
template <> struct PV<float, 4> {
    static __device__ void ld(const float* p, float* v) { const float4 a = *reinterpret_cast<const float4*>(p); v[0] = a.x; v[1] = a.y; v[2] = a.z; v[3] = a.w; }
    static __device__ void st(float* p, const float* v) { *reinterpret_cast<float4*>(p) = make_float4(v[0], v[1], v[2], v[3]); }
};
template <> struct PV<float, 1> {
    static __device__ void ld(const float* p, float* v) { v[0] = *p; }
    static __device__ void st(float* p, const float* v) { *p = v[0]; }
};
template <> struct PV<bf16_raw, 8> {
    static __device__ void ld(const bf16_raw* p, float* v) {
        const uint4 a = *reinterpret_cast<const uint4*>(p);
        const unsigned w[4] = {a.x, a.y, a.z, a.w};
#pragma unroll
        for (int i = 0; i < 4; ++i) { v[2 * i] = __uint_as_float(w[i] << 16); v[2 * i + 1] = __uint_as_float(w[i] & 0xffff0000u); }
    }
    static __device__ void st(bf16_raw* p, const float* v) {
        uint4 a;
        a.x = (unsigned)f32_to_bf16(v[0]) | ((unsigned)f32_to_bf16(v[1]) << 16);
        a.y = (unsigned)f32_to_bf16(v[2]) | ((unsigned)f32_to_bf16(v[3]) << 16);
        a.z = (unsigned)f32_to_bf16(v[4]) | ((unsigned)f32_to_bf16(v[5]) << 16);
        a.w = (unsigned)f32_to_bf16(v[6]) | ((unsigned)f32_to_bf16(v[7]) << 16);
        *reinterpret_cast<uint4*>(p) = a;
    }
};
template <> struct PV<bf16_raw, 4> {
    static __device__ void ld(const bf16_raw* p, float* v) {
        const uint2 a = *reinterpret_cast<const uint2*>(p);
        v[0] = __uint_as_float(a.x << 16); v[1] = __uint_as_float(a.x & 0xffff0000u);
        v[2] = __uint_as_float(a.y << 16); v[3] = __uint_as_float(a.y & 0xffff0000u);
    }
    static __device__ void st(bf16_raw* p, const float* v) {
        uint2 a;
        a.x = (unsigned)f32_to_bf16(v[0]) | ((unsigned)f32_to_bf16(v[1]) << 16);
        a.y = (unsigned)f32_to_bf16(v[2]) | ((unsigned)f32_to_bf16(v[3]) << 16);
        *reinterpret_cast<uint2*>(p) = a;
    }
};
template <> struct PV<bf16_raw, 1> {
    static __device__ void ld(const bf16_raw* p, float* v) { v[0] = bf16_to_f32(*p); }
    static __device__ void st(bf16_raw* p, const float* v) { *p = f32_to_bf16(v[0]); }
};
template <typename T> __device__ __forceinline__ float ld1(const T* p) { float v; PV<T, 1>::ld(p, &v); return v; }
template <typename T> __device__ __forceinline__ void st1(T* p, float v) { PV<T, 1>::st(p, &v); }

struct GemmArgs {
    const float* A;
    const void* B;
    float* C;
    const float* bias;
    int M, N, K;
    long lda, ldb, ldc;
    long strideA, strideB, strideC;
    int batch;
    int transA, transB;
    float alpha;
    int splitk;
    int atomic;
    long splitC;
    int b_dtype;
    int prec;
    float* colsum_a;
};
hipError_t launch_gemm(const GemmArgs& a, hipStream_t s);
bool gemm_fuses_colsum(const GemmArgs& a);

hipError_t launch_softmax_rows(float* s, long rows, int cols, hipStream_t st);
hipError_t launch_softmax_bwd_rows(const float* p, float* dp, long rows, int cols, float scale, hipStream_t st);
hipError_t launch_colsum(const float* x, float* out, int rows, int cols, long ld, hipStream_t st);
hipError_t launch_pos_logit(const float* q, const float* k, float* out, long ld_out, int B, int d, float inv_T, hipStream_t st);
hipError_t launch_infonce_rows(float* logits, int B, int ncols, float* loss_rows, float* lse, int32_t* top1,
                               int write_probs, hipStream_t st);
hipError_t launch_add_partials(float* dst, const float* parts, int nparts, long n, long stride, hipStream_t st);
hipError_t launch_pos_grad_init(const float* dlogits, long ld, const float* k, float* dq, int B, int d, float inv_T,
                                hipStream_t st);

hipError_t launch_enqueue(void* queue, const float* rows, int n, int64_t index, int K, int d, int qdtype, hipStream_t st);
hipError_t launch_enqueue_mirror(float* queue, void* mirror, const float* rows, int n, int64_t index, int K, int d, hipStream_t st);
hipError_t launch_prefetch(const void* p, size_t bytes, hipStream_t st);
hipError_t launch_widen_bf16(const void* src, float* dst, size_t n, hipStream_t st);
hipError_t launch_ema(const int64_t* table, int n_tensors, int64_t total_blocks, float m, float om, hipStream_t st);

size_t crd_workspace_bytes(int B, int d, int K1);
hipError_t launch_crd_fused(const float* v1, const float* v2, const float* memory_v1, const float* memory_v2, const int64_t* idx,
                            int B, int d, int K1, int64_t n_data, float T, float* Z, int set_z, float* loss, float* dv1, float* dv2,
                            int32_t* bad, void* ws, hipStream_t st);
hipError_t launch_crd_scores(const float* v1, const float* v2, const float* memory_v1, const float* memory_v2, const int64_t* idx,
                             int B, int d, int K1, int64_t n_data, float T, float* Z, int set_z, float* out_v1, float* out_v2,
                             int32_t* bad, void* ws, hipStream_t st);
hipError_t launch_crd_scores_bwd(const float* dout_v1, const float* dout_v2, const float* out_v1, const float* out_v2,
                                 const float* memory_v1, const float* memory_v2, const int64_t* idx, int B, int d, int K1,
                                 int64_t n_data, float T, float* dv1, float* dv2, int32_t* bad, void* ws, hipStream_t st);
hipError_t launch_crd_update(float* memory_v1, float* memory_v2, const float* v1, const float* v2, const int64_t* y, int B, int d,
                             int64_t n_data, float momentum, int32_t* bad, hipStream_t st);

size_t at_workspace_bytes(int B, int C, int H, int W, int oh, int ow, int layout);
hipError_t launch_at_map(const void* f, float* a, int B, int C, int H, int W, int oh, int ow, int dtype, int layout, void* ws,
                         hipStream_t st);
hipError_t launch_at_pair(const float* a_s, const float* a_t, int B, int n, float* norms, float* partials, float* loss, float* g_s,
                          float* g_t, float* ah_s, float* ah_t, hipStream_t st);
hipError_t launch_at_bwd(const void* f, const float* g_a, const float* g_loss, void* dF, int B, int C, int H, int W, int oh, int ow,
                         int dtype, int layout, hipStream_t st);

bool infonce_flash_supported(int B, int d, int K, int qdtype, int prec);
size_t infonce_flash_workspace_bytes(int B, int d, int K);
int set_k2_target_wg(int n);
struct EnqueueJob {
    void* queue16;
    float* queue32;
    const float* rows;
    int n;
    int64_t index;
    int K, d;
};
hipError_t launch_infonce_flash(const float* q, const float* k, const void* queue, int B, int d, int K, float inv_T,
                                float* loss_rows, float* lse, int32_t* top1, float* dq, void* ws, int qdtype,
                                hipStream_t st, hipEvent_t ev_begin = nullptr, hipEvent_t ev_end = nullptr,
                                const void* q_packed = nullptr, hipEvent_t ev_call_end = nullptr,
                                const EnqueueJob* enq = nullptr);
size_t infonce_qpack_bytes(int B, int d);
bool infonce_multi_supported(int n_terms, int B, int d, int K, int qdtype, int prec);
size_t infonce_multi_workspace_bytes(int n_terms, int B, int d, int K);
hipError_t launch_infonce_multi(const moma_infonce_term_t* terms, int n_terms, int B, int d, int K, float inv_T, void* ws,
                                hipStream_t st);

bool infonce_f32_flash_supported(int B, int d, int K, int qdtype, int prec);
size_t infonce_f32_flash_workspace_bytes(int B, int d, int K);
hipError_t launch_infonce_f32_flash(const float* q, const float* k, const float* queue, int B, int d, int K, float inv_T,
                                    float* loss_rows, float* lse, int32_t* top1, float* dq, void* ws, hipStream_t st,
                                    hipEvent_t ev_begin = nullptr, hipEvent_t ev_end = nullptr);

bool mha_fast_supported(int N, int d, int H, int prec);
hipError_t launch_mha_pack(const float* w_qkv, const float* w_proj, void* pack, int d, int with_t, hipStream_t st);
hipError_t launch_mha_fwd_fast(const moma_mha_module_t* mods, int n_modules, int N, int d, int H, hipStream_t st);
size_t mha_bwd_fast_workspace_bytes(int N, int d);
hipError_t launch_mha_bwd_fast(const void* pack, const void* x, int x_dtype, const void* qkv16, const void* attn16, const float* lse,
                               const float* dy, float* dx, float* dw_qkv, float* db_qkv, float* dw_proj, float* db_proj,
                               void* workspace, int N, int d, int H, hipStream_t st);

size_t bn_workspace_floats(int C);
hipError_t launch_bn_fwd(const void* x, void* out, const float* gamma, const float* beta, float* rm, float* rv,
                         float* save_mean, float* save_invstd, float* ws, int N, int C, int HW, int dtype, int act,
                         int training, float momentum, float eps, void* plane_mean, hipStream_t st);
hipError_t launch_bn_bwd(const void* x, const void* dout, const float* gamma, const float* beta, const float* save_mean,
                         const float* save_invstd, void* dx, float* dgamma, float* dbeta, float* ws, int N, int C, int HW,
                         int dtype, int act, int training, const void* dplane_mean, hipStream_t st);

bool dwconv_supported(int K, int S);
size_t dwconv_workspace_floats(int C, int K);
hipError_t launch_dw_fwd(const void* x, const float* w, void* y, int N, int C, int H, int W, int OH, int OW, int K, int S,
                         int pt, int pl, int dtype, hipStream_t st);
hipError_t launch_dw_bwd_data(const void* dy, const float* w, void* dx, int N, int C, int H, int W, int OH, int OW, int K,
                              int S, int pt, int pl, int dtype, hipStream_t st);
hipError_t launch_dw_bwd_weight(const void* x, const void* dy, float* dw, float* ws, size_t ws_floats, int N, int C, int H,
                                int W, int OH, int OW, int K, int S, int pt, int pl, int dtype, hipStream_t st);

hipError_t launch_plane_mean(const void* x, void* out, int NC, int HW, int dtype, hipStream_t st);
hipError_t launch_se_gate_fwd(const void* x, const void* s, void* out, int NC, int HW, int dtype, hipStream_t st);
hipError_t launch_se_gate_bwd(const void* x, const void* s, const void* dout, void* dx, void* ds, int NC, int HW, int dtype,
                              hipStream_t st);

}
```

moma_amd/csrc/dwconv.hip:

```cpp
#include "common.hpp"

namespace moma {
namespace {

constexpr int DW_WAVES = 4;
constexpr int XO = 4;
constexpr int LDS_BUDGET = 64 * 1024;

template <typename T, int VEC> struct Vec;
template <> struct Vec<float, 4> { static __device__ void ld(const float* p, float* v) { const float4 a = *reinterpret_cast<const float4*>(p); v[0] = a.x; v[1] = a.y; v[2] = a.z; v[3] = a.w; } };
template <> struct Vec<float, 2> { static __device__ void ld(const float* p, float* v) { const float2 a = *reinterpret_cast<const float2*>(p); v[0] = a.x; v[1] = a.y; } };
template <> struct Vec<float, 1> { static __device__ void ld(const float* p, float* v) { v[0] = *p; } };
template <> struct Vec<bf16_raw, 8> {
    static __device__ void ld(const bf16_raw* p, float* v) {
        const uint4 a = *reinterpret_cast<const uint4*>(p);
        const unsigned w[4] = {a.x, a.y, a.z, a.w};
#pragma unroll
        for (int i = 0; i < 4; ++i) { v[2 * i] = __uint_as_float(w[i] << 16); v[2 * i + 1] = __uint_as_float(w[i] & 0xffff0000u); }
    }
};
template <> struct Vec<bf16_raw, 4> {
    static __device__ void ld(const bf16_raw* p, float* v) {
        const uint2 a = *reinterpret_cast<const uint2*>(p);
        v[0] = __uint_as_float(a.x << 16); v[1] = __uint_as_float(a.x & 0xffff0000u);
        v[2] = __uint_as_float(a.y << 16); v[3] = __uint_as_float(a.y & 0xffff0000u);
    }
};
template <> struct Vec<bf16_raw, 2> {
    static __device__ void ld(const bf16_raw* p, float* v) {
        const unsigned a = *reinterpret_cast<const unsigned*>(p);
        v[0] = __uint_as_float(a << 16); v[1] = __uint_as_float(a & 0xffff0000u);
    }
};
template <> struct Vec<bf16_raw, 1> { static __device__ void ld(const bf16_raw* p, float* v) { v[0] = bf16_to_f32(*p); } };

template <int VEC> __device__ __forceinline__ void lds_store(float* p, const float* v) {
    if constexpr (VEC == 8) {
        *reinterpret_cast<float4*>(p) = make_float4(v[0], v[1], v[2], v[3]);
        *reinterpret_cast<float4*>(p + 4) = make_float4(v[4], v[5], v[6], v[7]);
    } else if constexpr (VEC == 4) {
        *reinterpret_cast<float4*>(p) = make_float4(v[0], v[1], v[2], v[3]);
    } else if constexpr (VEC == 2) {
        *reinterpret_cast<float2*>(p) = make_float2(v[0], v[1]);
    } else {
        *p = v[0];
    }
}
template <typename T> __device__ __forceinline__ void st(T* p, float v);
template <> __device__ __forceinline__ void st<float>(float* p, float v) { *p = v; }
template <> __device__ __forceinline__ void st<bf16_raw>(bf16_raw* p, float v) { *p = f32_to_bf16(v); }

struct DwShape {
    int NC, C, H, W, OH, OW, pt, pl;
    int TH, nbands, PB, ngroups;
    int IR, pitch;
    int GR, gpitch;
};

__device__ __forceinline__ int uniform(int v) { return __builtin_amdgcn_readfirstlane(v); }

__device__ __forceinline__ int fast_div(int i, int d, float inv_d) {
    int q = (int)((float)i * inv_d);
    q += (q + 1) * d <= i;
    q -= q * d > i;
    return q;
}

template <typename T, int VEC>
__device__ __forceinline__ void fill_tile(float* tile, const T* __restrict__ src, size_t plane_stride, int np, int H, int W,
                                          int y0, int rows, int pitch, int xo, int lane, bool zero_rows) {
    const int ya = max(y0, 0), yb = min(y0 + rows, H);
    const int wv = W / VEC, nvpp = max(yb - ya, 0) * wv, total = nvpp * np;
    const float inv_nvpp = 1.0f / (float)max(nvpp, 1), inv_wv = 1.0f / (float)wv;
    constexpr int U = 4;
    for (int v0 = 0; v0 < total; v0 += 64 * U) {
        float val[U][VEC];
        int dst[U];
#pragma unroll
        for (int u = 0; u < U; ++u) {
            const int v = min(v0 + u * 64 + lane, total - 1);
            const int p = fast_div(v, nvpp, inv_nvpp), e = v - p * nvpp, r = fast_div(e, wv, inv_wv), cv = e - r * wv;
            Vec<T, VEC>::ld(src + (size_t)p * plane_stride + (size_t)(ya + r) * W + cv * VEC, val[u]);
            dst[u] = (p * rows + (ya - y0) + r) * pitch + xo + cv * VEC;
        }
#pragma unroll
        for (int u = 0; u < U; ++u) asm volatile("" : "+v"(val[u][0]));
#pragma unroll
        for (int u = 0; u < U; ++u)
            if (v0 + u * 64 + lane < total) lds_store<VEC>(tile + dst[u], val[u]);
    }
    const int ztop = ya - y0, zbot = y0 + rows - max(yb, ya);
    if (zero_rows && (ztop > 0 || zbot > 0)) {
        for (int p = 0; p < np; ++p)
            for (int r = 0; r < rows; ++r)
                if (r < ztop || r >= rows - zbot)
                    for (int c = lane; c < W; c += 64) tile[(p * rows + r) * pitch + xo + c] = 0.f;
    }
}

template <typename T, int K, int S, int R, bool FLIP, int VEC>
__global__ __launch_bounds__(DW_WAVES * 64) void dw_fwd_kernel(const T* __restrict__ x, const float* __restrict__ w,
                                                             T* __restrict__ y, DwShape sh) {
    extern __shared__ float smem[];
    const int lane = threadIdx.x & 63, wave = threadIdx.x >> 6;
    const int tfl = sh.PB * sh.IR * sh.pitch;
    float* tile = smem + wave * (tfl + ((sh.PB * K * K + 3) & ~3));
    float* wl = tile + tfl;
    for (int i = lane; i < tfl; i += 64) tile[i] = 0.f;
    const int nitems = sh.ngroups * sh.nbands;
    const int nstrips = (sh.TH + R - 1) / R;
    constexpr int CR = (R - 1) * S + K;
    const int cbase = XO - sh.pl;
    for (int item = uniform(blockIdx.x * DW_WAVES + wave); item < nitems; item += gridDim.x * DW_WAVES) {
        const int grp = item / sh.nbands, band = item - grp * sh.nbands;
        const int plane0 = grp * sh.PB, np = min(sh.PB, sh.NC - plane0);
        const int oy0 = band * sh.TH, th = min(sh.TH, sh.OH - oy0);
        for (int i = lane; i < np * K * K; i += 64) {
            const int p = i / (K * K), t = i - p * (K * K);
            wl[i] = w[((plane0 + p) % sh.C) * K * K + (FLIP ? K * K - 1 - t : t)];
        }
        fill_tile<T, VEC>(tile, x + (size_t)plane0 * sh.H * sh.W, (size_t)sh.H * sh.W, np, sh.H, sh.W, oy0 * S - sh.pt, sh.IR,
                          sh.pitch, XO, lane, sh.nbands > 1);
        __builtin_amdgcn_s_waitcnt(0xc07f);
        const int nwork = nstrips * sh.OW;
        const float inv_ow = 1.0f / (float)sh.OW;
        for (int p = 0; p < np; ++p) {
            float wk[K * K];
#pragma unroll
            for (int t = 0; t < K * K; ++t) wk[t] = wl[p * K * K + t];
            const float* pt_ = tile + p * sh.IR * sh.pitch + cbase;
            T* yp = y + (size_t)(plane0 + p) * sh.OH * sh.OW;
            for (int i = lane; i < nwork; i += 64) {
                const int strip = fast_div(i, sh.OW, inv_ow), ox = i - strip * sh.OW;
                float acc[R];
#pragma unroll
                for (int r = 0; r < R; ++r) acc[r] = 0.f;
                const float* base = pt_ + (strip * R * S) * sh.pitch + ox * S;
#pragma unroll
                for (int kx = 0; kx < K; ++kx) {
                    float col[CR];
#pragma unroll
                    for (int rr = 0; rr < CR; ++rr) col[rr] = base[rr * sh.pitch + kx];
#pragma unroll
                    for (int r = 0; r < R; ++r)
#pragma unroll
                        for (int ky = 0; ky < K; ++ky) acc[r] = fmaf(wk[ky * K + kx], col[r * S + ky], acc[r]);
                }
                T* o = yp + (size_t)(oy0 + strip * R) * sh.OW + ox;
                if (strip * R + R <= th) {
#pragma unroll
                    for (int r = 0; r < R; ++r) st<T>(o + r * sh.OW, acc[r]);
                } else {
#pragma unroll
                    for (int r = 0; r < R; ++r)
                        if (strip * R + r < th) st<T>(o + r * sh.OW, acc[r]);
                }
            }
        }
        __builtin_amdgcn_s_waitcnt(0xc07f);
    }
}

template <typename T, int K, int S, int OWT, bool FLIP, int VEC>
__global__ __launch_bounds__(DW_WAVES * 64) void dw_small_kernel(const T* __restrict__ x, const float* __restrict__ w,
                                                               T* __restrict__ y, DwShape sh) {
    extern __shared__ float smem[];
    constexpr int IW = (OWT - 1) * S + K;
    const int lane = threadIdx.x & 63, wave = threadIdx.x >> 6;
    const int tfl = sh.PB * sh.IR * sh.pitch;
    float* tile = smem + wave * (tfl + ((sh.PB * K * K + 3) & ~3));
    float* wl = tile + tfl;
    for (int i = lane; i < tfl; i += 64) tile[i] = 0.f;
    const int p = lane / OWT, oy = lane - p * OWT;
    const int cbase = XO - sh.pl;
    for (int item = uniform(blockIdx.x * DW_WAVES + wave); item < sh.ngroups; item += gridDim.x * DW_WAVES) {
        const int plane0 = item * sh.PB, np = min(sh.PB, sh.NC - plane0);
        for (int i = lane; i < np * K * K; i += 64) {
            const int pp = i / (K * K), t = i - pp * (K * K);
            wl[i] = w[((plane0 + pp) % sh.C) * K * K + (FLIP ? K * K - 1 - t : t)];
        }
        fill_tile<T, VEC>(tile, x + (size_t)plane0 * sh.H * sh.W, (size_t)sh.H * sh.W, np, sh.H, sh.W, -sh.pt, sh.IR, sh.pitch,
                          XO, lane, false);
        __builtin_amdgcn_s_waitcnt(0xc07f);
        if (p < np) {
            float wk[K * K];
#pragma unroll
            for (int t = 0; t < K * K; ++t) wk[t] = wl[p * K * K + t];
            float acc[OWT];
#pragma unroll
            for (int ox = 0; ox < OWT; ++ox) acc[ox] = 0.f;
            const float* rowp = tile + (p * sh.IR + oy * S) * sh.pitch + cbase;
#pragma unroll
            for (int ky = 0; ky < K; ++ky) {
                float xr[IW];
#pragma unroll
                for (int c = 0; c < IW; ++c) xr[c] = rowp[ky * sh.pitch + c];
#pragma unroll
                for (int ox = 0; ox < OWT; ++ox)
#pragma unroll
                    for (int kx = 0; kx < K; ++kx) acc[ox] = fmaf(wk[ky * K + kx], xr[ox * S + kx], acc[ox]);
            }
            T* o = y + ((size_t)(plane0 + p) * OWT + oy) * OWT;
#pragma unroll
            for (int ox = 0; ox < OWT; ++ox) st<T>(o + ox, acc[ox]);
        }
        __builtin_amdgcn_s_waitcnt(0xc07f);
    }
}

template <typename T, int K, int VEC>
__global__ __launch_bounds__(DW_WAVES * 64) void dw_bwd_data_s2_kernel(const T* __restrict__ dy, const float* __restrict__ w,
                                                                     T* __restrict__ dx, DwShape sh) {
    extern __shared__ float smem[];
    constexpr int HT = (K - 1) / 2;
    const int lane = threadIdx.x & 63, wave = threadIdx.x >> 6;
    const int tfl = sh.PB * sh.IR * sh.pitch;
    float* tile = smem + wave * (tfl + ((sh.PB * K * K + 3) & ~3));
    float* wl = tile + tfl;
    for (int i = lane; i < tfl; i += 64) tile[i] = 0.f;
    const int nitems = sh.ngroups * sh.nbands;
    const int nb = (sh.OW + sh.pl + 2) / 2;
    for (int item = uniform(blockIdx.x * DW_WAVES + wave); item < nitems; item += gridDim.x * DW_WAVES) {
        const int grp = item / sh.nbands, band = item - grp * sh.nbands;
        const int plane0 = grp * sh.PB, np = min(sh.PB, sh.NC - plane0);
        const int a0 = band * sh.TH;
        for (int i = lane; i < np * K * K; i += 64) {
            const int p = i / (K * K), t = i - p * (K * K);
            wl[i] = w[((plane0 + p) % sh.C) * K * K + t];
        }
        fill_tile<T, VEC>(tile, dy + (size_t)plane0 * sh.H * sh.W, (size_t)sh.H * sh.W, np, sh.H, sh.W, a0 - HT, sh.IR, sh.pitch,
                          XO, lane, sh.nbands > 1);
        __builtin_amdgcn_s_waitcnt(0xc07f);
        const int nwork = sh.TH * nb;
        const float inv_nb = 1.0f / (float)nb;
        for (int p = 0; p < np; ++p) {
            float wk[K * K];
#pragma unroll
            for (int t = 0; t < K * K; ++t) wk[t] = wl[p * K * K + t];
            const float* pt_ = tile + p * sh.IR * sh.pitch + XO;
            T* xp = dx + (size_t)(plane0 + p) * sh.OH * sh.OW;
            for (int i = lane; i < nwork; i += 64) {
                const int ar = fast_div(i, nb, inv_nb), b = i - ar * nb;
                float g[HT + 1][HT + 1];
#pragma unroll
                for (int t = 0; t <= HT; ++t)
#pragma unroll
                    for (int s = 0; s <= HT; ++s) g[t][s] = pt_[(ar + HT - t) * sh.pitch + (b - s)];
#pragma unroll
                for (int e = 0; e < 2; ++e)
#pragma unroll
                    for (int f = 0; f < 2; ++f) {
                        float acc = 0.f;
#pragma unroll
                        for (int t = 0; e + 2 * t < K; ++t)
#pragma unroll
                            for (int s = 0; f + 2 * s < K; ++s) acc = fmaf(wk[(e + 2 * t) * K + f + 2 * s], g[t][s], acc);
                        const int iy = 2 * (a0 + ar) + e - sh.pt, ix = 2 * b + f - sh.pl;
                        if (iy >= 0 && iy < sh.OH && ix >= 0 && ix < sh.OW) st<T>(xp + (size_t)iy * sh.OW + ix, acc);
                    }
            }
        }
        __builtin_amdgcn_s_waitcnt(0xc07f);
    }
}

template <typename T, int K, int S, int R, int VEC, int GVEC, bool GDIRECT>
__global__ __launch_bounds__(DW_WAVES * 64) void dw_bwd_weight_kernel(const T* __restrict__ x, const T* __restrict__ dy,
                                                                    float* __restrict__ partial, DwShape sh, int N) {
    extern __shared__ float smem[];
    const int lane = threadIdx.x & 63, wave = threadIdx.x >> 6;
    const int xt = sh.PB * sh.IR * sh.pitch, gtn = GDIRECT ? 0 : sh.PB * sh.GR * sh.gpitch;
    float* tile = smem + wave * (xt + gtn);
    float* gt = tile + xt;
    for (int i = lane; i < xt + gtn; i += 64) tile[i] = 0.f;
    const int c = blockIdx.y;
    const int nsplit = gridDim.x * DW_WAVES, split = blockIdx.x * DW_WAVES + wave;
    const int nstrips = (sh.TH + R - 1) / R;
    constexpr int CR = (R - 1) * S + K;
    const int cbase = XO - sh.pl;
    float acc[K * K];
#pragma unroll
    for (int t = 0; t < K * K; ++t) acc[t] = 0.f;
    const size_t xs = (size_t)sh.C * sh.H * sh.W, gs = (size_t)sh.C * sh.OH * sh.OW;
    const int nitems = sh.ngroups * sh.nbands;
    for (int item = uniform(split); item < nitems; item += nsplit) {
        const int grp = item / sh.nbands, band = item - grp * sh.nbands;
        const int n0 = grp * sh.PB, np = min(sh.PB, N - n0);
        const int oy0 = band * sh.TH;
        fill_tile<T, VEC>(tile, x + ((size_t)n0 * sh.C + c) * sh.H * sh.W, xs, np, sh.H, sh.W, oy0 * S - sh.pt, sh.IR, sh.pitch, XO,
                          lane, sh.nbands > 1);
        if constexpr (!GDIRECT)
            fill_tile<T, GVEC>(gt, dy + ((size_t)n0 * sh.C + c) * sh.OH * sh.OW, gs, np, sh.OH, sh.OW, oy0, sh.GR, sh.gpitch, 0,
                               lane, sh.nbands > 1);
        __builtin_amdgcn_s_waitcnt(0xc07f);
        const int nwork = nstrips * sh.OW;
        const float inv_ow = 1.0f / (float)sh.OW;
        for (int p = 0; p < np; ++p) {
            const float* pt_ = tile + p * sh.IR * sh.pitch + cbase;
            const float* gp = gt + p * sh.GR * sh.gpitch;
            const T* gd = dy + ((size_t)(n0 + p) * sh.C + c) * sh.OH * sh.OW;
            for (int i = lane; i < nwork; i += 64) {
                const int strip = fast_div(i, sh.OW, inv_ow), ox = i - strip * sh.OW;
                float g[R];
                if constexpr (GDIRECT) {
#pragma unroll
                    for (int r = 0; r < R; ++r) {
                        float t1[1];
                        Vec<T, 1>::ld(gd + (size_t)min(oy0 + strip * R + r, sh.OH - 1) * sh.OW + ox, t1);
                        g[r] = t1[0];
                    }
#pragma unroll
                    for (int r = 0; r < R; ++r) {
                        asm volatile("" : "+v"(g[r]));
                        g[r] = (oy0 + strip * R + r < sh.OH) ? g[r] : 0.f;
                    }
                } else {
#pragma unroll
                    for (int r = 0; r < R; ++r) g[r] = gp[(strip * R + r) * sh.gpitch + ox];
                }
                const float* base = pt_ + (strip * R * S) * sh.pitch + ox * S;
#pragma unroll
                for (int kx = 0; kx < K; ++kx) {
                    float col[CR];
#pragma unroll
                    for (int rr = 0; rr < CR; ++rr) col[rr] = base[rr * sh.pitch + kx];
#pragma unroll
                    for (int r = 0; r < R; ++r)
#pragma unroll
                        for (int ky = 0; ky < K; ++ky) acc[ky * K + kx] = fmaf(g[r], col[r * S + ky], acc[ky * K + kx]);
                }
            }
        }
        __builtin_amdgcn_s_waitcnt(0xc07f);
    }
#pragma unroll
    for (int t = 0; t < K * K; ++t) acc[t] = wave_sum(acc[t]);
    if (lane == 0) {
        float* p = partial + ((size_t)c * nsplit + split) * K * K;
#pragma unroll
        for (int t = 0; t < K * K; ++t) p[t] = acc[t];
    }
}

__global__ void dw_bwd_weight_finalize_kernel(const float* __restrict__ partial, float* __restrict__ dw, int total, int nsplit,
                                              int kk) {
    const int i = blockIdx.x * blockDim.x + threadIdx.x;
    if (i >= total) return;
    const int c = i / kk, t = i - c * kk;
    float s = 0.f;
    for (int k = 0; k < nsplit; ++k) s += partial[((size_t)c * nsplit + k) * kk + t];
    dw[i] = s;
}

int round4(int v) { return (v + 3) & ~3; }
int pick_vec(int W, int elem_bytes, const void* a) {
    const int maxv = 16 / elem_bytes;
    for (int v = maxv; v > 1; v >>= 1)
        if (W % v == 0 && (uintptr_t)a % (v * elem_bytes) == 0) return v;
    return 1;
}
int strip_rows(int OH) { return OH >= 28 ? 4 : (OH >= 14 ? 2 : 1); }
int planes_per_item(int OH, int OW, int nbands) {
    if (nbands > 1) return 1;
    const int px = OH * OW;
    return px <= 64 ? 8 : (px <= 256 ? 4 : (px <= 1024 ? 2 : 1));
}
constexpr int WAVE_TILE_FLOATS = 2560;
int pick_th(int OH, int S, int K, int pitch, int extra_floats_per_row, int R) {
    int th = ((OH + R - 1) / R) * R;
    while (th > R && ((th - 1) * S + K) * (long)pitch + (long)th * extra_floats_per_row > WAVE_TILE_FLOATS) th -= R;
    const int nbands = (OH + th - 1) / th;
    return (((OH + nbands - 1) / nbands + R - 1) / R) * R;
}
int fit_planes(int pb, long floats_per_plane) {
    while (pb > 1 && pb * floats_per_plane > WAVE_TILE_FLOATS) pb >>= 1;
    return pb;
}
unsigned grid_for(long nitems) {
    long g = (nitems + DW_WAVES - 1) / DW_WAVES;
    if (g > 256 * 16) g = 256 * 16;
    return (unsigned)max(1L, g);
}

#define MOMA_DW_VEC_SWITCH(vec, MAXV, BODY)                                    \
    if (MAXV >= 8 && (vec) == 8) { constexpr int V = (MAXV >= 8 ? 8 : 4); BODY; } \
    else if ((vec) >= 4) { constexpr int V = 4; BODY; }                        \
    else if ((vec) == 2) { constexpr int V = 2; BODY; }                        \
    else { constexpr int V = 1; BODY; }

template <typename T, int K, int S>
hipError_t fwd_t(const T* x, const float* w, T* y, int NC, int C, int H, int W, int OH, int OW, int pt, int pl, bool flip,
                 hipStream_t st) {
    constexpr int MAXV = 16 / sizeof(T);
    DwShape sh{};
    sh.NC = NC; sh.C = C; sh.H = H; sh.W = W; sh.OH = OH; sh.OW = OW; sh.pt = pt; sh.pl = pl;
    sh.pitch = round4(XO + max(W, (OW - 1) * S + K - pl) + 1);
    if (S == 1 && OH == OW && (OW == 7 || OW == 14)) {
        sh.TH = OH; sh.nbands = 1;
        sh.IR = (OH - 1) * S + K;
        sh.PB = OW == 7 ? 8 : 4;
        sh.pitch |= 1;
        sh.ngroups = (NC + sh.PB - 1) / sh.PB;
        const size_t lds = (size_t)DW_WAVES * (sh.PB * sh.IR * sh.pitch + round4(sh.PB * K * K)) * sizeof(float);
        if (lds <= (size_t)LDS_BUDGET) {
            const dim3 grid(grid_for(sh.ngroups)), block(DW_WAVES * 64);
            const int vec = 1;
#define MOMA_DW_SMALL(OWT, FL) hipLaunchKernelGGL((dw_small_kernel<T, K, S, OWT, FL, V>), grid, block, lds, st, x, w, y, sh)
            MOMA_DW_VEC_SWITCH(vec, MAXV, {
                if (OW == 7) { if (flip) MOMA_DW_SMALL(7, true); else MOMA_DW_SMALL(7, false); }
                else { if (flip) MOMA_DW_SMALL(14, true); else MOMA_DW_SMALL(14, false); }
            })
#undef MOMA_DW_SMALL
            return hipGetLastError();
        }
    }
    const int R = strip_rows(OH);
    sh.TH = pick_th(OH, S, K, sh.pitch, 0, R);
    sh.nbands = (OH + sh.TH - 1) / sh.TH;
    sh.IR = (sh.TH - 1) * S + K;
    sh.PB = fit_planes(planes_per_item(OH, OW, sh.nbands), (long)sh.IR * sh.pitch);
    sh.ngroups = (NC + sh.PB - 1) / sh.PB;
    const size_t lds = (size_t)DW_WAVES * (sh.PB * sh.IR * sh.pitch + round4(sh.PB * K * K)) * sizeof(float);
    if (lds > (size_t)LDS_BUDGET) return hipErrorInvalidValue;
    const dim3 grid(grid_for((long)sh.ngroups * sh.nbands)), block(DW_WAVES * 64);
    const int vec = pick_vec(W, sizeof(T), x);
#define MOMA_DW_GO(RR, FL) hipLaunchKernelGGL((dw_fwd_kernel<T, K, S, RR, FL, V>), grid, block, lds, st, x, w, y, sh)
    MOMA_DW_VEC_SWITCH(vec, MAXV, {
        if (flip) { if (R == 4) MOMA_DW_GO(4, true); else if (R == 2) MOMA_DW_GO(2, true); else MOMA_DW_GO(1, true); }
        else { if (R == 4) MOMA_DW_GO(4, false); else if (R == 2) MOMA_DW_GO(2, false); else MOMA_DW_GO(1, false); }
    })
#undef MOMA_DW_GO
    return hipGetLastError();
}

template <typename T, int K>
hipError_t bwd_data_s2_t(const T* dy, const float* w, T* dx, int NC, int C, int H, int W, int OH, int OW, int pt, int pl,
                         hipStream_t st) {
    constexpr int MAXV = 16 / sizeof(T);
    constexpr int HT = (K - 1) / 2;
    DwShape sh{};
    sh.NC = NC; sh.C = C; sh.H = OH; sh.W = OW; sh.OH = H; sh.OW = W; sh.pt = pt; sh.pl = pl;
    const int nb = (W + pl + 2) / 2, na = (H + pt + 2) / 2;
    sh.pitch = round4(XO + max(OW, nb) + 1);
    int th = na;
    while (th > 1 && (long)(th + HT) * sh.pitch > WAVE_TILE_FLOATS) --th;
    th = (na + (na + th - 1) / th - 1) / ((na + th - 1) / th);
    sh.TH = th;
    sh.nbands = (na + th - 1) / th;
    sh.IR = th + HT;
    sh.PB = fit_planes(planes_per_item(H, W, sh.nbands), (long)sh.IR * sh.pitch);
    sh.ngroups = (NC + sh.PB - 1) / sh.PB;
    const size_t lds = (size_t)DW_WAVES * (sh.PB * sh.IR * sh.pitch + round4(sh.PB * K * K)) * sizeof(float);
    if (lds > (size_t)LDS_BUDGET) return hipErrorInvalidValue;
    const dim3 grid(grid_for((long)sh.ngroups * sh.nbands)), block(DW_WAVES * 64);
    const int vec = pick_vec(OW, sizeof(T), dy);
    MOMA_DW_VEC_SWITCH(vec, MAXV, { hipLaunchKernelGGL((dw_bwd_data_s2_kernel<T, K, V>), grid, block, lds, st, dy, w, dx, sh); })
    return hipGetLastError();
}

template <typename T, int K, int S>
hipError_t bwd_weight_t(const T* x, const T* dy, float* dw, float* ws, size_t ws_floats, int N, int C, int H, int W, int OH,
                        int OW, int pt, int pl, hipStream_t st) {
    constexpr int MAXV = 16 / sizeof(T);
    DwShape sh{};
    sh.NC = N * C; sh.C = C; sh.H = H; sh.W = W; sh.OH = OH; sh.OW = OW; sh.pt = pt; sh.pl = pl;
    sh.pitch = round4(XO + max(W, (OW - 1) * S + K - pl) + 1);
    const bool gdirect = !(K == 3 && OH >= 56);
    sh.gpitch = gdirect ? 0 : round4(OW + 1);
    const int R = strip_rows(OH);
    sh.TH = pick_th(OH, S, K, sh.pitch, sh.gpitch, R);
    sh.nbands = (OH + sh.TH - 1) / sh.TH;
    sh.IR = (sh.TH - 1) * S + K;
    sh.GR = gdirect ? 0 : sh.TH;
    sh.PB = fit_planes(min(planes_per_item(OH, OW, sh.nbands), N), (long)sh.IR * sh.pitch + (long)sh.GR * sh.gpitch);
    sh.ngroups = (N + sh.PB - 1) / sh.PB;
    const size_t lds = (size_t)DW_WAVES * sh.PB * (sh.IR * sh.pitch + sh.GR * sh.gpitch) * sizeof(float);
    if (lds > (size_t)LDS_BUDGET) return hipErrorInvalidValue;
    long nsplit_wg = max(1L, min((long)(2048 + C - 1) / C, ((long)sh.ngroups * sh.nbands + DW_WAVES - 1) / DW_WAVES));
    while (nsplit_wg > 1 && (size_t)C * nsplit_wg * DW_WAVES * K * K > ws_floats) --nsplit_wg;
    if ((size_t)C * nsplit_wg * DW_WAVES * K * K > ws_floats) return hipErrorInvalidValue;
    const dim3 grid((unsigned)nsplit_wg, C), block(DW_WAVES * 64);
    const int vec = pick_vec(W, sizeof(T), x), gvec = pick_vec(OW, sizeof(T), dy);
#define MOMA_DW_GO(RR, GV, GD) hipLaunchKernelGGL((dw_bwd_weight_kernel<T, K, S, RR, V, GV, GD>), grid, block, lds, st, x, dy, ws, sh, N)
    MOMA_DW_VEC_SWITCH(vec, MAXV, {
        if (gdirect) { if (R == 4) MOMA_DW_GO(4, 1, true); else if (R == 2) MOMA_DW_GO(2, 1, true); else MOMA_DW_GO(1, 1, true); }
        else if (gvec >= V) { if (R == 4) MOMA_DW_GO(4, V, false); else if (R == 2) MOMA_DW_GO(2, V, false); else MOMA_DW_GO(1, V, false); }
        else { if (R == 4) MOMA_DW_GO(4, 1, false); else if (R == 2) MOMA_DW_GO(2, 1, false); else MOMA_DW_GO(1, 1, false); }
    })
#undef MOMA_DW_GO
    const int total = C * K * K;
    hipLaunchKernelGGL(dw_bwd_weight_finalize_kernel, dim3((total + 255) / 256), dim3(256), 0, st, ws, dw, total,
                       (int)nsplit_wg * DW_WAVES, K * K);
    return hipGetLastError();
}
}

bool dwconv_supported(int K, int S) { return (K == 3 || K == 5) && (S == 1 || S == 2); }
size_t dwconv_workspace_floats(int C, int K) { return (size_t)C * 64 * DW_WAVES * K * K; }

#define MOMA_DW_DISPATCH(CALL)                                                   \
    if (K == 3 && S == 1) return CALL(3, 1);                                      \
    if (K == 3 && S == 2) return CALL(3, 2);                                      \
    if (K == 5 && S == 1) return CALL(5, 1);                                      \
    if (K == 5 && S == 2) return CALL(5, 2);                                      \
    return hipErrorInvalidValue;

hipError_t launch_dw_fwd(const void* x, const float* w, void* y, int N, int C, int H, int W, int OH, int OW, int K, int S,
                         int pt, int pl, int dtype, hipStream_t st) {
    if (dtype == MOMA_DT_BF16) {
#define CALL(KK, SS) fwd_t<bf16_raw, KK, SS>((const bf16_raw*)x, w, (bf16_raw*)y, N * C, C, H, W, OH, OW, pt, pl, false, st)
        MOMA_DW_DISPATCH(CALL)
#undef CALL
    }
#define CALL(KK, SS) fwd_t<float, KK, SS>((const float*)x, w, (float*)y, N * C, C, H, W, OH, OW, pt, pl, false, st)
    MOMA_DW_DISPATCH(CALL)
#undef CALL
}

hipError_t launch_dw_bwd_data(const void* dy, const float* w, void* dx, int N, int C, int H, int W, int OH, int OW, int K,
                              int S, int pt, int pl, int dtype, hipStream_t st) {
    if (S == 1) {
        if (dtype == MOMA_DT_BF16) {
            if (K == 3) return fwd_t<bf16_raw, 3, 1>((const bf16_raw*)dy, w, (bf16_raw*)dx, N * C, C, OH, OW, H, W, 2 - pt, 2 - pl, true, st);
            if (K == 5) return fwd_t<bf16_raw, 5, 1>((const bf16_raw*)dy, w, (bf16_raw*)dx, N * C, C, OH, OW, H, W, 4 - pt, 4 - pl, true, st);
        } else {
            if (K == 3) return fwd_t<float, 3, 1>((const float*)dy, w, (float*)dx, N * C, C, OH, OW, H, W, 2 - pt, 2 - pl, true, st);
            if (K == 5) return fwd_t<float, 5, 1>((const float*)dy, w, (float*)dx, N * C, C, OH, OW, H, W, 4 - pt, 4 - pl, true, st);
        }
        return hipErrorInvalidValue;
    }
    if (dtype == MOMA_DT_BF16) {
        if (K == 3) return bwd_data_s2_t<bf16_raw, 3>((const bf16_raw*)dy, w, (bf16_raw*)dx, N * C, C, H, W, OH, OW, pt, pl, st);
        if (K == 5) return bwd_data_s2_t<bf16_raw, 5>((const bf16_raw*)dy, w, (bf16_raw*)dx, N * C, C, H, W, OH, OW, pt, pl, st);
    } else {
        if (K == 3) return bwd_data_s2_t<float, 3>((const float*)dy, w, (float*)dx, N * C, C, H, W, OH, OW, pt, pl, st);
        if (K == 5) return bwd_data_s2_t<float, 5>((const float*)dy, w, (float*)dx, N * C, C, H, W, OH, OW, pt, pl, st);
    }
    return hipErrorInvalidValue;
}

hipError_t launch_dw_bwd_weight(const void* x, const void* dy, float* dw, float* ws, size_t ws_floats, int N, int C, int H,
                                int W, int OH, int OW, int K, int S, int pt, int pl, int dtype, hipStream_t st) {
    if (dtype == MOMA_DT_BF16) {
#define CALL(KK, SS) bwd_weight_t<bf16_raw, KK, SS>((const bf16_raw*)x, (const bf16_raw*)dy, dw, ws, ws_floats, N, C, H, W, OH, OW, pt, pl, st)
        MOMA_DW_DISPATCH(CALL)
#undef CALL
    }
#define CALL(KK, SS) bwd_weight_t<float, KK, SS>((const float*)x, (const float*)dy, dw, ws, ws_floats, N, C, H, W, OH, OW, pt, pl, st)
    MOMA_DW_DISPATCH(CALL)
#undef CALL
}

}
```

moma_amd/ops.py:

```python
from __future__ import annotations

import ctypes as C
from typing import Sequence, Tuple

import torch

from . import _lib
from ._lib import DT_BF16, DT_F32, PREC_BF16, PREC_F32, EMA_BLOCK_ELEMS, MomaHipError, check

_PREC = {"fp32": PREC_F32, "f32": PREC_F32, "float32": PREC_F32, PREC_F32: PREC_F32,
         "bf16": PREC_BF16, "bfloat16": PREC_BF16, PREC_BF16: PREC_BF16}


def prec_code(p) -> int:
    try:
        return _PREC[p]
    except KeyError:
        raise ValueError(f"unknown precision {p!r}; use 'fp32' or 'bf16'")


def _qdtype(queue: torch.Tensor) -> int:
    if queue.dtype == torch.float32:
        return DT_F32
    if queue.dtype == torch.bfloat16:
# ... 358 lines not shown
        qs = [tensors[3 * i].contiguous() for i in range(n)]
        ks = [tensors[3 * i + 1].contiguous() for i in range(n)]
        queues = [tensors[3 * i + 2] for i in range(n)]
        for q, k, queue in zip(qs, ks, queues):
            _check_qk(q, k, queue)
        B, d = qs[0].shape
        K = queues[0].shape[0]
        dev = qs[0].device
        need_grad = any(ctx.needs_input_grad[2 + 3 * i] for i in range(n))
        qd = _qdtype(queues[0])
        ws = torch.empty(max(lib.moma_infonce_fused_multi_workspace_bytes(n, B, d, K, qd, prec), 16), device=dev, dtype=torch.uint8)
        terms = (_lib.InfoNCETerm * n)()
        outs, dqs = [], []
        for i in range(n):
            loss_rows = torch.empty(B, device=dev, dtype=torch.float32)
            lse = torch.empty(B, device=dev, dtype=torch.float32)
            top1 = torch.empty(B, device=dev, dtype=torch.int32)
            dq = torch.empty(B, d, device=dev, dtype=torch.float32) if need_grad else None
            t = terms[i]
            t.q, t.k, t.queue = qs[i].data_ptr(), ks[i].data_ptr(), queues[i].data_ptr()
            t.loss_rows, t.lse, t.top1, t.dq = loss_rows.data_ptr(), lse.data_ptr(), top1.data_ptr(), (0 if dq is None else dq.data_ptr())
            outs += [loss_rows, lse, top1]
            dqs.append(dq)
        with _timed("moma_infonce_fused_multi"):
            check(lib.moma_infonce_fused_multi(C.cast(terms, C.c_void_p), n, B, d, K, float(1.0 / T), _ptr(ws), ws.numel(), qd,
                                               prec, _stream()), "moma_infonce_fused_multi")
        if need_grad:
            ctx.save_for_backward(*dqs)
        ctx.n = n
        ctx.mark_non_differentiable(*[o for i, o in enumerate(outs) if i % 3 != 0])
        return tuple(outs)

    @staticmethod
    def backward(ctx, *grads):
        dqs = ctx.saved_tensors
        res = [None, None]
        for i in range(ctx.n):
            g_loss = grads[3 * i]
            res += [dqs[i] * g_loss.unsqueeze(1) if (ctx.needs_input_grad[2 + 3 * i] and g_loss is not None) else None, None, None]
        return tuple(res)


def infonce_fused_multi(terms, T: float, prec="fp32"):
    pc = prec_code(prec)
    q0, _, queue0 = terms[0]
    same = all(q.shape == q0.shape and queue.shape == queue0.shape and queue.dtype == queue0.dtype for q, _, queue in terms)
    if len(terms) > 1 and len(terms) <= 4 and same and q0.is_cuda:
        flat = _InfoNCEFusedMulti.apply(float(T), pc, *[t for term in terms for t in term])
        return [tuple(flat[3 * i:3 * i + 3]) for i in range(len(terms))]
    return [infonce_fused(q, k, queue, T, prec) for q, k, queue in terms]


class MhaPack:

    def __init__(self):
        self.buf, self.key, self.has_t = None, None, False

    def invalidate(self):
        self.buf = None

    def get(self, w_qkv: torch.Tensor, w_proj: torch.Tensor, need_t: bool) -> torch.Tensor:
        key = (w_qkv.data_ptr(), w_qkv._version, w_proj.data_ptr(), w_proj._version, w_qkv.device)
        if self.buf is None or key != self.key or (need_t and not self.has_t):
            lib = _lib.load()
            d = w_proj.shape[0]
            buf = torch.empty(lib.moma_mha_pack_bytes(d), device=w_qkv.device, dtype=torch.uint8)
            check(lib.moma_mha_pack_weights(_ptr(w_qkv), _ptr(w_proj), _ptr(buf), d, int(need_t), _stream()),
                  "moma_mha_pack_weights")
            self.buf, self.key, self.has_t = buf, key, bool(need_t)
        return self.buf


def _mha_check(x, w_qkv, b_qkv, w_proj, b_proj, H):
    _dev(x, "x", None)
    if x.dtype not in (torch.float32, torch.bfloat16):
        raise TypeError(f"x: expected float32 or bfloat16, got {x.dtype}")
    for t, nm in ((w_qkv, "qkv.weight"), (w_proj, "proj.weight"), (b_proj, "proj.bias")):
        _dev(t, nm)
    if b_qkv is not None:
        _dev(b_qkv, "qkv.bias")
    N, d = x.shape
    if w_qkv.shape != (3 * d, d) or w_proj.shape != (d, d) or d % H:
        raise ValueError(f"bad attention shapes: x {tuple(x.shape)} Wqkv {tuple(w_qkv.shape)} H={H}")
    return N, d


def _mha_fast_fwd(items, H, want_lse, qpacks=None):
    lib = _lib.load()
    N, d = items[0][0].shape
    dev = items[0][0].device
    mods = (_lib.MhaModule * len(items))()
    outs = []
    for i, (x, pack, b_qkv, b_proj) in enumerate(items):
        y = torch.empty(N, d, device=dev, dtype=torch.float32)
        qkv16 = torch.empty(N, 3 * d, device=dev, dtype=torch.bfloat16)
        attn16 = torch.empty(N, d, device=dev, dtype=torch.bfloat16)
        lse = torch.empty(H, N, device=dev, dtype=torch.float32) if want_lse else None
        qp = qpacks[i] if qpacks is not None else None
        m = mods[i]
        m.x, m.pack, m.b_qkv, m.b_proj = x.data_ptr(), pack.data_ptr(), (0 if b_qkv is None else b_qkv.data_ptr()), b_proj.data_ptr()
        m.y, m.qkv16, m.attn16, m.lse = y.data_ptr(), qkv16.data_ptr(), attn16.data_ptr(), (0 if lse is None else lse.data_ptr())
        m.qpack, m.qpack_scale = (0, 0.0) if qp is None else (qp.buf.data_ptr(), float(qp.scale))
        m.x_dtype = DT_BF16 if x.dtype == torch.bfloat16 else DT_F32
        outs.append((y, qkv16, attn16, lse))
    with _timed("moma_mha_fwd" if len(items) == 1 else f"moma_mha_fwd_group{len(items)}"):
        check(lib.moma_mha_fwd_fast(C.cast(mods, C.c_void_p), len(items), N, d, H, _stream()), "moma_mha_fwd_fast")
    return outs


class _MHA(torch.autograd.Function):
    @staticmethod
    def forward(ctx, x, w_qkv, b_qkv, w_proj, b_proj, H, prec, grad_mode, holder, qpack):
        lib = _lib.load()
        x = x.contiguous()
        N, d = _mha_check(x, w_qkv, b_qkv, w_proj, b_proj, H)
        dev = x.device
        ctx.x_dtype = x.dtype
        need_bwd = grad_mode and any(ctx.needs_input_grad)
        fast = lib.moma_mha_saved_state(N, d, H, prec) == _lib.MHA_SAVE_LSE
        ctx.H, ctx.prec, ctx.has_bqkv, ctx.fast = H, prec, b_qkv is not None, fast
        if fast:
            pack = (holder if holder is not None else MhaPack()).get(w_qkv, w_proj, need_bwd)
            (y, qkv16, attn16, lse), = _mha_fast_fwd([(x, pack, b_qkv, b_proj)], H, need_bwd,
                                                     None if qpack is None else [qpack])
            if need_bwd:
                ctx.save_for_backward(x, pack, qkv16, attn16, lse)
            if qpack is not None:
                qpack.written_from(y, qpack.T)
            return y
        x = x.float()
        y = torch.empty(N, d, device=dev, dtype=torch.float32)
        qkv = torch.empty(N, 3 * d, device=dev, dtype=torch.float32)
        probs = torch.empty(H, N, N, device=dev, dtype=torch.float32)
        attn_out = torch.empty(N, d, device=dev, dtype=torch.float32)
        with _timed("moma_mha_fwd"):
            check(lib.moma_mha_fwd(_ptr(x), _ptr(w_qkv), _ptr(b_qkv), _ptr(w_proj), _ptr(b_proj), _ptr(y), _ptr(qkv),
                                   _ptr(probs), _ptr(attn_out), N, d, H, prec, _stream()), "moma_mha_fwd")
        if need_bwd:
            ctx.save_for_backward(x, w_qkv, w_proj, qkv, probs, attn_out)
        return y

    @staticmethod
    def backward(ctx, dy):
        lib = _lib.load()
        dy = dy.contiguous()
        H = ctx.H
        need = ctx.needs_input_grad
        if ctx.fast:
            x, pack, qkv16, attn16, lse = ctx.saved_tensors
        else:
            x, w_qkv, w_proj, qkv, probs, attn_out = ctx.saved_tensors
        N, d = x.shape
        dev = x.device
        dx = torch.empty(N, d, device=dev, dtype=torch.float32) if need[0] else None
        dw_qkv = torch.empty(3 * d, d, device=dev, dtype=torch.float32) if need[1] else None
        db_qkv = torch.empty(3 * d, device=dev, dtype=torch.float32) if (need[2] and ctx.has_bqkv) else None
        dw_proj = torch.empty(d, d, device=dev, dtype=torch.float32) if need[3] else None
        db_proj = torch.empty(d, device=dev, dtype=torch.float32) if need[4] else None
        if ctx.fast:
            t_wq = dw_qkv if (dw_qkv is not None or db_qkv is None) else torch.empty(3 * d, d, device=dev, dtype=torch.float32)
            t_wp = dw_proj if (dw_proj is not None or db_proj is None) else torch.empty(d, d, device=dev, dtype=torch.float32)
            ws = torch.empty(lib.moma_mha_bwd_fast_workspace_bytes(N, d, H), device=dev, dtype=torch.uint8)
            with _timed("moma_mha_bwd"):
                check(lib.moma_mha_bwd_fast(_ptr(pack), _ptr(x), DT_BF16 if x.dtype == torch.bfloat16 else DT_F32, _ptr(qkv16), _ptr(attn16), _ptr(lse), _ptr(dy), _ptr(dx),
                                            _ptr(t_wq), _ptr(db_qkv), _ptr(t_wp), _ptr(db_proj), _ptr(ws), ws.numel(), N, d, H,
                                            _stream()), "moma_mha_bwd_fast")
        else:
            ws = torch.empty(lib.moma_mha_bwd_workspace_bytes(N, d, H, ctx.prec), device=dev, dtype=torch.uint8)
            with _timed("moma_mha_bwd"):
                check(lib.moma_mha_bwd(_ptr(x), _ptr(w_qkv), _ptr(w_proj), _ptr(qkv), _ptr(probs), _ptr(attn_out),
                                       _ptr(dy), _ptr(dx), _ptr(dw_qkv), _ptr(db_qkv), _ptr(dw_proj), _ptr(db_proj), _ptr(ws),
                                       ws.numel(), N, d, H, ctx.prec, _stream()), "moma_mha_bwd")
        if dx is not None and dx.dtype != ctx.x_dtype:
            dx = dx.to(ctx.x_dtype)
        return dx, dw_qkv, db_qkv, dw_proj, db_proj, None, None, None, None, None


def mha(x, w_qkv, b_qkv, w_proj, b_proj, num_heads: int, prec="fp32", pack: "MhaPack | None" = None, qpack=None) -> torch.Tensor:
    return _MHA.apply(x, w_qkv, b_qkv, w_proj, b_proj, int(num_heads), prec_code(prec), torch.is_grad_enabled(), pack, qpack)


def mha_group(calls, num_heads: int, prec="fp32"):
    lib = _lib.load()
    pc = prec_code(prec)
    xs = [c[0].contiguous() for c in calls]
    same = all(x.shape == xs[0].shape for x in xs) and 1 < len(calls) <= 4
    wants_grad = torch.is_grad_enabled() and any(t is not None and t.requires_grad for c in calls for t in c[:5])
    if not same or wants_grad or lib.moma_mha_saved_state(xs[0].shape[0], xs[0].shape[1], int(num_heads), pc) != _lib.MHA_SAVE_LSE:
        return [mha(c[0], c[1], c[2], c[3], c[4], num_heads, prec, c[5]) for c in calls]
    items = []
    for x, c in zip(xs, calls):
        _mha_check(x, c[1], c[2], c[3], c[4], int(num_heads))
        holder = c[5] if c[5] is not None else MhaPack()
        items.append((x, holder.get(c[1], c[3], False), c[2], c[4]))
    return [o[0] for o in _mha_fast_fwd(items, int(num_heads), False)]


ACT_CODES = {None: 0, "none": 0, "silu": 1, "relu": 2}
_DT_CODES = {torch.float32: 0, torch.bfloat16: 1}


class _BNAct(torch.autograd.Function):
    @staticmethod
    def forward(ctx, x, weight, bias, running_mean, running_var, training, momentum, eps, act, want_mean):
        lib = _lib.load()
        _dev(x, "x", dtype=None, contiguous=False)
        if x.dim() < 2 or x.dtype not in _DT_CODES:
            raise ValueError(f"bn_act: expects [N, C, ...] float32 / bfloat16, got {tuple(x.shape)} {x.dtype}")
        x = x.contiguous()
        N, Cc = x.shape[0], x.shape[1]
        HW = x.numel() // (N * Cc)
        dev = x.device
        out = torch.empty_like(x)
        save_mean = torch.empty(Cc, device=dev, dtype=torch.float32)
        save_invstd = torch.empty(Cc, device=dev, dtype=torch.float32)
        ws = torch.empty(lib.moma_bn_workspace_bytes(Cc), device=dev, dtype=torch.uint8)
        pmean = torch.empty(N, Cc, 1, 1, device=dev, dtype=x.dtype) if want_mean else None
        check(lib.moma_bn_fwd(_ptr(x), _ptr(out), _ptr(weight), _ptr(bias), _ptr(running_mean), _ptr(running_var),
                              _ptr(save_mean), _ptr(save_invstd), _ptr(ws), ws.numel(), N, Cc, HW, _DT_CODES[x.dtype],
                              act, int(training), float(momentum), float(eps), _ptr(pmean), _stream()), "moma_bn_fwd")
        ctx.save_for_backward(x, weight, bias, save_mean, save_invstd)
        ctx.cfg = (N, Cc, HW, act, int(training))
        ctx.set_materialize_grads(False)
        return (out, pmean) if want_mean else out

    @staticmethod
    def backward(ctx, dout, dmean=None):
        lib = _lib.load()
        x, weight, bias, save_mean, save_invstd = ctx.saved_tensors
        N, Cc, HW, act, training = ctx.cfg
        if dout is None:
            dout = torch.zeros_like(x)
        dout = dout.contiguous()
        if dout.dtype != x.dtype:
            dout = dout.to(x.dtype)
        if dmean is not None:
            dmean = dmean.to(x.dtype).contiguous()
        dev = x.device
        dx = torch.empty_like(x) if ctx.needs_input_grad[0] else None
        dgamma = torch.empty(Cc, device=dev, dtype=torch.float32) if (weight is not None and ctx.needs_input_grad[1]) else None
        dbeta = torch.empty(Cc, device=dev, dtype=torch.float32) if (bias is not None and ctx.needs_input_grad[2]) else None
        ws = torch.empty(lib.moma_bn_workspace_bytes(Cc), device=dev, dtype=torch.uint8)
        check(lib.moma_bn_bwd(_ptr(x), _ptr(dout), _ptr(weight), _ptr(bias), _ptr(save_mean), _ptr(save_invstd), _ptr(dx),
                              _ptr(dgamma), _ptr(dbeta), _ptr(ws), ws.numel(), N, Cc, HW, _DT_CODES[x.dtype], act,
                              training, _ptr(dmean), _stream()), "moma_bn_bwd")
        return dx, dgamma, dbeta, None, None, None, None, None, None, None


def bn_act(x, weight, bias, running_mean, running_var, training: bool, momentum: float, eps: float, act=None,
           want_mean: bool = False):
    return _BNAct.apply(x, weight, bias, running_mean, running_var, bool(training), momentum, eps, ACT_CODES[act],
                        bool(want_mean))


class _DWConv(torch.autograd.Function):
    @staticmethod
    def forward(ctx, x, w, stride, pad_top, pad_left, out_h, out_w):
        lib = _lib.load()
        _dev(x, "x", dtype=None, contiguous=False)
        _dev(w, "weight")
        if x.dim() != 4 or x.dtype not in _DT_CODES or w.dim() != 4 or w.shape[1] != 1 or w.shape[0] != x.shape[1] \
                or w.shape[2] != w.shape[3]:
            raise ValueError(f"dwconv: x {tuple(x.shape)} {x.dtype}, weight {tuple(w.shape)}")
        x = x.contiguous()
        w = w.contiguous()
        N, Cc, H, W = x.shape
        K = w.shape[2]
        y = torch.empty(N, Cc, out_h, out_w, device=x.device, dtype=x.dtype)
        check(lib.moma_dwconv_fwd(_ptr(x), _ptr(w), _ptr(y), N, Cc, H, W, out_h, out_w, K, stride, pad_top, pad_left,
                                  _DT_CODES[x.dtype], _stream()), "moma_dwconv_fwd")
        ctx.save_for_backward(x, w)
        ctx.cfg = (N, Cc, H, W, out_h, out_w, K, stride, pad_top, pad_left)
        return y

    @staticmethod
    def backward(ctx, dy):
        lib = _lib.load()
        x, w = ctx.saved_tensors
        N, Cc, H, W, OH, OW, K, stride, pt, pl = ctx.cfg
        dy = dy.contiguous()
        if dy.dtype != x.dtype:
            dy = dy.to(x.dtype)
        dx = dw = None
        if ctx.needs_input_grad[0]:
            dx = torch.empty_like(x)
            check(lib.moma_dwconv_bwd_data(_ptr(dy), _ptr(w), _ptr(dx), N, Cc, H, W, OH, OW, K, stride, pt, pl,
                                           _DT_CODES[x.dtype], _stream()), "moma_dwconv_bwd_data")
        if ctx.needs_input_grad[1]:
            dw = torch.empty_like(w)
            ws = torch.empty(lib.moma_dwconv_workspace_bytes(Cc, K), device=x.device, dtype=torch.uint8)
            check(lib.moma_dwconv_bwd_weight(_ptr(x), _ptr(dy), _ptr(dw), _ptr(ws), ws.numel(), N, Cc, H, W, OH, OW, K,
                                             stride, pt, pl, _DT_CODES[x.dtype], _stream()), "moma_dwconv_bwd_weight")
        return dx, dw, None, None, None, None, None


def dwconv_supported(kernel: int, stride: int) -> bool:
    return kernel in (3, 5) and stride in (1, 2)


def dwconv(x, weight, stride: int, pad_top: int, pad_left: int, out_h: int, out_w: int):
    return _DWConv.apply(x, weight, int(stride), int(pad_top), int(pad_left), int(out_h), int(out_w))


class _PlaneMean(torch.autograd.Function):
    @staticmethod
    def forward(ctx, x):
        lib = _lib.load()
        _dev(x, "x", dtype=None, contiguous=False)
        if x.dim() != 4 or x.dtype not in _DT_CODES:
            raise ValueError(f"plane_mean: expects [N,C,H,W] float32 / bfloat16, got {tuple(x.shape)} {x.dtype}")
        x = x.contiguous()
        N, Cc, H, W = x.shape
        out = torch.empty(N, Cc, 1, 1, device=x.device, dtype=x.dtype)
        check(lib.moma_plane_mean(_ptr(x), _ptr(out), N * Cc, H * W, _DT_CODES[x.dtype], _stream()), "moma_plane_mean")
        ctx.shape = (N, Cc, H, W)
        return out

    @staticmethod
    def backward(ctx, dmean):
        N, Cc, H, W = ctx.shape
        return (dmean / (H * W)).expand(N, Cc, H, W)


class _SEGate(torch.autograd.Function):
    @staticmethod
    def forward(ctx, x, s):
        lib = _lib.load()
        _dev(x, "x", dtype=None, contiguous=False)
        _dev(s, "s", dtype=None, contiguous=False)
        if x.dim() != 4 or x.dtype not in _DT_CODES or s.numel() != x.shape[0] * x.shape[1]:
            raise ValueError(f"se_gate: x {tuple(x.shape)} {x.dtype}, s {tuple(s.shape)}")
        x = x.contiguous()
        s = s.to(x.dtype).contiguous()
        N, Cc, H, W = x.shape
        out = torch.empty_like(x)
        check(lib.moma_se_gate_fwd(_ptr(x), _ptr(s), _ptr(out), N * Cc, H * W, _DT_CODES[x.dtype], _stream()), "moma_se_gate_fwd")
        ctx.save_for_backward(x, s)
        return out

    @staticmethod
    def backward(ctx, dout):
        lib = _lib.load()
        x, s = ctx.saved_tensors
        N, Cc, H, W = x.shape
        dout = dout.contiguous()
        if dout.dtype != x.dtype:
            dout = dout.to(x.dtype)
        dx = torch.empty_like(x)
        ds = torch.empty_like(s)
        check(lib.moma_se_gate_bwd(_ptr(x), _ptr(s), _ptr(dout), _ptr(dx), _ptr(ds), N * Cc, H * W, _DT_CODES[x.dtype],
                                   _stream()), "moma_se_gate_bwd")
        return dx, ds


def plane_mean(x):
    return _PlaneMean.apply(x)


def se_gate(x, s):
    return _SEGate.apply(x, s)


def _crd_check(v1, v2, memory_v1, memory_v2, idx, n_data, Z, bad):
    _dev(v1, "v1"); _dev(v2, "v2"); _dev(memory_v1, "memory_v1"); _dev(memory_v2, "memory_v2")
    _dev(idx, "idx", torch.int64); _dev(Z, "Z"); _dev(bad, "bad_index", torch.int32)
    if (v1.dim() != 2 or v1.shape != v2.shape or memory_v1.dim() != 2 or memory_v1.shape != memory_v2.shape
            or memory_v1.shape[1] != v1.shape[1] or idx.dim() != 2 or idx.shape[0] != v1.shape[0]):
        raise ValueError(f"shape mismatch: v1 {tuple(v1.shape)} v2 {tuple(v2.shape)} memory_v1 {tuple(memory_v1.shape)} "
                         f"memory_v2 {tuple(memory_v2.shape)} idx {tuple(idx.shape)}")
    if int(n_data) != memory_v1.shape[0]:
        raise ValueError(f"n_data {n_data} != rows of the banks {memory_v1.shape[0]}")
    if Z.numel() != 2 or bad.numel() != 1:
        raise ValueError("Z must hold 2 floats (side 1, side 2) and bad_index one int32")


def _crd_workspace(lib, B, d, K1, dev):
    n = lib.moma_crd_workspace_bytes(B, d, K1)
    if n == 0:
        raise MomaHipError(f"moma_crd: unsupported shape B={B} d={d} K1={K1} (d a multiple of 4 up to 2048, nce_k >= 1)")
    return torch.empty(n, device=dev, dtype=torch.uint8), n


class _CRDFused(torch.autograd.Function):

    @staticmethod
    def forward(ctx, v1, v2, memory_v1, memory_v2, idx, T, n_data, Z, set_z, bad):
        lib = _lib.load()
        v1 = v1.contiguous() if isinstance(v1, torch.Tensor) else v1
        v2 = v2.contiguous() if isinstance(v2, torch.Tensor) else v2
        _crd_check(v1, v2, memory_v1, memory_v2, idx, n_data, Z, bad)
        B, d = v1.shape
        K1 = idx.shape[1]
        dev = v1.device
        need_grad = ctx.needs_input_grad[0] or ctx.needs_input_grad[1]
        loss = torch.empty(2, device=dev, dtype=torch.float32)
        dv1 = torch.empty(B, d, device=dev, dtype=torch.float32) if need_grad else None
        dv2 = torch.empty(B, d, device=dev, dtype=torch.float32) if need_grad else None
        ws, ws_bytes = _crd_workspace(lib, B, d, K1, dev)
        with _timed("moma_crd_fused"):
            check(lib.moma_crd_fused(_ptr(v1), _ptr(v2), _ptr(memory_v1), _ptr(memory_v2), _ptr(idx), B, d, K1, int(n_data),
                                     float(T), _ptr(Z), int(bool(set_z)), _ptr(loss), _ptr(dv1), _ptr(dv2), _ptr(bad), _ptr(ws),
                                     ws_bytes, _stream()), "moma_crd_fused")
        if need_grad:
            ctx.save_for_backward(dv1, dv2)
        return loss

    @staticmethod
    def backward(ctx, g):
        dv1, dv2 = ctx.saved_tensors
        return (dv1 * g[0] if ctx.needs_input_grad[0] else None, dv2 * g[1] if ctx.needs_input_grad[1] else None,
                None, None, None, None, None, None, None, None)


def crd_fused(v1, v2, memory_v1, memory_v2, idx, T: float, n_data: int, Z, set_z: bool, bad=None) -> torch.Tensor:
    if bad is None and isinstance(v1, torch.Tensor) and v1.is_cuda:
        bad = torch.zeros(1, device=v1.device, dtype=torch.int32)
    return _CRDFused.apply(v1, v2, memory_v1, memory_v2, idx, float(T), int(n_data), Z, bool(set_z), bad)


class _CRDScores(torch.autograd.Function):

    @staticmethod
    def forward(ctx, v1, v2, memory_v1, memory_v2, idx, T, n_data, Z, set_z, bad, update_y):
        lib = _lib.load()
        v1 = v1.contiguous() if isinstance(v1, torch.Tensor) else v1
        v2 = v2.contiguous() if isinstance(v2, torch.Tensor) else v2
        _crd_check(v1, v2, memory_v1, memory_v2, idx, n_data, Z, bad)
        B, d = v1.shape
        K1 = idx.shape[1]
        dev = v1.device
        out_v1 = torch.empty(B, K1, device=dev, dtype=torch.float32)
        out_v2 = torch.empty(B, K1, device=dev, dtype=torch.float32)
        ws, ws_bytes = _crd_workspace(lib, B, d, K1, dev)
        with _timed("moma_crd_scores"):
            check(lib.moma_crd_scores(_ptr(v1), _ptr(v2), _ptr(memory_v1), _ptr(memory_v2), _ptr(idx), B, d, K1, int(n_data),
                                      float(T), _ptr(Z), int(bool(set_z)), _ptr(out_v1), _ptr(out_v2), _ptr(bad), _ptr(ws),
                                      ws_bytes, _stream()), "moma_crd_scores")
        ctx.save_for_backward(out_v1, out_v2)
        ctx.banks, ctx.idx, ctx.bad, ctx.T, ctx.n_data = (memory_v1, memory_v2), idx, bad, T, n_data
        ctx.rows_at = ctx.old_rows = None
        if update_y is not None:
            ctx.rows_at = update_y.clamp(0, int(n_data) - 1)
            ctx.old_rows = (memory_v1.index_select(0, ctx.rows_at), memory_v2.index_select(0, ctx.rows_at))
        return out_v1, out_v2

    @staticmethod
    def backward(ctx, dout_v1, dout_v2):
        lib = _lib.load()
        out_v1, out_v2 = ctx.saved_tensors
        (memory_v1, memory_v2), idx, bad = ctx.banks, ctx.idx, ctx.bad
        B, K1 = out_v1.shape
        d = memory_v1.shape[1]
        dev = out_v1.device
        dout_v1 = dout_v1.contiguous(); dout_v2 = dout_v2.contiguous()
        dv1 = torch.empty(B, d, device=dev, dtype=torch.float32)
        dv2 = torch.empty(B, d, device=dev, dtype=torch.float32)
        ws, ws_bytes = _crd_workspace(lib, B, d, K1, dev)
        new_rows = None
        if ctx.old_rows is not None:
            with torch.no_grad():
                new_rows = (memory_v1.index_select(0, ctx.rows_at), memory_v2.index_select(0, ctx.rows_at))
                memory_v1.index_copy_(0, ctx.rows_at, ctx.old_rows[0]); memory_v2.index_copy_(0, ctx.rows_at, ctx.old_rows[1])
        with _timed("moma_crd_scores_bwd"):
            check(lib.moma_crd_scores_bwd(_ptr(dout_v1), _ptr(dout_v2), _ptr(out_v1), _ptr(out_v2), _ptr(memory_v1),
                                          _ptr(memory_v2), _ptr(idx), B, d, K1, int(ctx.n_data), float(ctx.T), _ptr(dv1), _ptr(dv2),
                                          _ptr(bad), _ptr(ws), ws_bytes, _stream()), "moma_crd_scores_bwd")
        if new_rows is not None:
            with torch.no_grad():
                memory_v1.index_copy_(0, ctx.rows_at, new_rows[0]); memory_v2.index_copy_(0, ctx.rows_at, new_rows[1])
        return dv1, dv2, None, None, None, None, None, None, None, None, None


def crd_scores(v1, v2, memory_v1, memory_v2, idx, T: float, n_data: int, Z, set_z: bool, bad=None, update_y=None):
    if bad is None and isinstance(v1, torch.Tensor) and v1.is_cuda:
        bad = torch.zeros(1, device=v1.device, dtype=torch.int32)
    return _CRDScores.apply(v1, v2, memory_v1, memory_v2, idx, float(T), int(n_data), Z, bool(set_z), bad, update_y)


def crd_update_(memory_v1, memory_v2, v1, v2, y, momentum: float, bad=None) -> None:
    lib = _lib.load()
    _dev(memory_v1, "memory_v1"); _dev(memory_v2, "memory_v2"); _dev(v1, "v1"); _dev(v2, "v2"); _dev(y, "y", torch.int64)
    if bad is None:
        bad = torch.zeros(1, device=v1.device, dtype=torch.int32)
    _dev(bad, "bad_index", torch.int32)
    B, d = v1.shape
    if v2.shape != v1.shape or memory_v1.shape != memory_v2.shape or memory_v1.shape[1] != d or y.shape != (B,):
        raise ValueError(f"shape mismatch: v1 {tuple(v1.shape)} v2 {tuple(v2.shape)} banks {tuple(memory_v1.shape)} / "
                         f"{tuple(memory_v2.shape)} y {tuple(y.shape)}")
    with trace_range("moma_crd_update"):
        check(lib.moma_crd_update(_ptr(memory_v1), _ptr(memory_v2), _ptr(v1), _ptr(v2), _ptr(y), B, d, memory_v1.shape[0],
                                  float(momentum), _ptr(bad), _stream()), "moma_crd_update")


def _at_side(f, name):
    _dev(f, name, dtype=None, contiguous=False)
    if f.dim() != 4 or f.dtype not in _DT_CODES:
        raise TypeError(f"attention_loss: {name} must be a 4-D float32 / bfloat16 tensor, got {tuple(f.shape)} {f.dtype}")
    if f.is_contiguous():
        return f, _lib.LAYOUT_NCHW
    if f.is_contiguous(memory_format=torch.channels_last):
        return f, _lib.LAYOUT_NHWC
    return f.contiguous(), _lib.LAYOUT_NCHW


def _at_map(lib, f, layout, oh, ow):
    B, Cc, H, W = f.shape
    a = torch.empty(B, oh * ow, device=f.device, dtype=torch.float32)
    dt = _DT_CODES[f.dtype]
    n = lib.moma_at_workspace_bytes(B, Cc, H, W, oh, ow, dt, layout)
    ws = torch.empty(n, device=f.device, dtype=torch.uint8) if n else None
    check(lib.moma_at_map(_ptr(f), _ptr(a), B, Cc, H, W, oh, ow, dt, layout, _ptr(ws), n, _stream()), "moma_at_map")
    return a


class _AttentionLoss(torch.autograd.Function):

    @staticmethod
    def forward(ctx, f_s, f_t, oh, ow):
        lib = _lib.load()
        f_s, lay_s = _at_side(f_s, "f_s")
        f_t, lay_t = _at_side(f_t, "f_t")
        B = f_s.shape[0]
        if f_t.shape[0] != B or f_s.shape[2] % oh or f_s.shape[3] % ow or f_t.shape[2] % oh or f_t.shape[3] % ow:
            raise ValueError(f"attention_loss: f_s {tuple(f_s.shape)} and f_t {tuple(f_t.shape)} have no common {oh} x {ow} grid")
        dev, n = f_s.device, oh * ow
        need_s, need_t = ctx.needs_input_grad[0], ctx.needs_input_grad[1]
        with _timed("moma_at_fwd"):
            a_s, a_t = _at_map(lib, f_s, lay_s, oh, ow), _at_map(lib, f_t, lay_t, oh, ow)
            norms = torch.empty(B, 2, device=dev, dtype=torch.float32)
            partials = torch.empty(B, device=dev, dtype=torch.float32)
            loss = torch.empty((), device=dev, dtype=torch.float32)
            g_s = torch.empty(B, n, device=dev, dtype=torch.float32) if need_s else None
            g_t = torch.empty(B, n, device=dev, dtype=torch.float32) if need_t else None
            check(lib.moma_at_pair(_ptr(a_s), _ptr(a_t), B, n, _ptr(norms), _ptr(partials), _ptr(loss), _ptr(g_s), _ptr(g_t),
                                   _ptr(None), _ptr(None), _stream()), "moma_at_pair")
        ctx.save_for_backward(*[t for t, need in ((f_s, need_s), (g_s, need_s), (f_t, need_t), (g_t, need_t)) if need])
        ctx.sides = (need_s, need_t)
        ctx.grid, ctx.layouts = (oh, ow), (lay_s, lay_t)
        return loss

    @staticmethod
    @torch.autograd.function.once_differentiable
    def backward(ctx, g):
        lib = _lib.load()
        saved = list(ctx.saved_tensors)
        oh, ow = ctx.grid
        g = g.to(torch.float32).contiguous()
        out = [None, None]
        with _timed("moma_at_bwd"):
            for side, need in enumerate(ctx.sides):
                if not need:
                    continue
                f, g_a = saved.pop(0), saved.pop(0)
                B, Cc, H, W = f.shape
                dF = torch.empty_like(f)
                check(lib.moma_at_bwd(_ptr(f), _ptr(g_a), _ptr(g), _ptr(dF), B, Cc, H, W, oh, ow, _DT_CODES[f.dtype],
                                      ctx.layouts[side], _stream()), "moma_at_bwd")
                out[side] = dF
        return out[0], out[1], None, None


def attention_loss(f_s, f_t) -> torch.Tensor:
    for t, nm in ((f_s, "f_s"), (f_t, "f_t")):
        _dev(t, nm, dtype=None, contiguous=False)
        if t.dim() != 4:
            raise ValueError(f"attention_loss: {nm} must be [B,C,H,W], got {tuple(t.shape)}")
    Hs, Ht = f_s.shape[2], f_t.shape[2]
    if Hs == Ht:
        oh, ow = Hs, f_s.shape[3]
        if f_t.shape[3] != ow:
            raise ValueError(f"attention_loss: equal heights but widths {ow} and {f_t.shape[3]}: the maps have no common grid")
    else:
        oh = ow = min(Hs, Ht)
        if Hs > Ht and (Hs % oh or f_s.shape[3] % ow):
            f_s = torch.nn.functional.adaptive_avg_pool2d(f_s, (oh, ow))
        elif Ht > Hs and (Ht % oh or f_t.shape[3] % ow):
            f_t = torch.nn.functional.adaptive_avg_pool2d(f_t, (oh, ow))
        small = f_t if Hs > Ht else f_s
        if small.shape[3] != ow:
            raise ValueError(f"attention_loss: the smaller map {tuple(small.shape)} is not square: no common {oh} x {ow} grid")
    return _AttentionLoss.apply(f_s, f_t, int(oh), int(ow))
```

Baseline: 6369.

## Fuse BN+SiLU into depthwise conv input load for no-grad encoder path

After: 6454 (median of 6 runs). +1.3%, better.

```diff
diff --git a/include/moma_hip.h b/include/moma_hip.h
--- a/include/moma_hip.h
+++ b/include/moma_hip.h
@@ -149,6 +149,10 @@
                 const float* save_mean, const float* save_invstd, void* dx, float* dgamma, float* dbeta,
                 void* workspace, size_t workspace_bytes, int N, int C, int HW, int dtype, int act,
                 int training, const void* dplane_mean, moma_stream_t stream);
+int moma_bn_prepare(const void* x, const float* gamma, const float* beta, float* running_mean,
+                    float* running_var, float* save_mean, float* save_invstd, float* scale_shift,
+                    void* workspace, size_t workspace_bytes, int N, int C, int HW, int dtype, int training,
+                    float momentum, float eps, moma_stream_t stream);
 
 size_t moma_dwconv_workspace_bytes(int C, int K);
 int moma_dwconv_fwd(const void* x, const float* w, void* y, int N, int C, int H, int W, int OH, int OW,
@@ -159,6 +163,13 @@
 int moma_dwconv_bwd_weight(const void* x, const void* dy, float* dw, void* workspace,
                            size_t workspace_bytes, int N, int C, int H, int W, int OH, int OW, int K,
                            int stride, int pad_top, int pad_left, int dtype, moma_stream_t stream);
+int moma_dwconv_fwd_pre(const void* x, const float* w, void* y, int N, int C, int H, int W, int OH, int OW,
+                        int K, int stride, int pad_top, int pad_left, int dtype, const float* scale_shift,
+                        int act, moma_stream_t stream);
+int moma_dwconv_bwd_weight_pre(const void* x, const void* dy, float* dw, void* workspace,
+                               size_t workspace_bytes, int N, int C, int H, int W, int OH, int OW, int K,
+                               int stride, int pad_top, int pad_left, int dtype, const float* scale_shift,
+                               int act, moma_stream_t stream);
 
 int moma_plane_mean(const void* x, void* mean, int NC, int HW, int dtype, moma_stream_t stream);
 int moma_se_gate_fwd(const void* x, const void* s, void* out, int NC, int HW, int dtype, moma_stream_t stream);
diff --git a/moma_amd/_lib.py b/moma_amd/_lib.py
--- a/moma_amd/_lib.py
+++ b/moma_amd/_lib.py
@@ -60,12 +60,15 @@
     "moma_dwconv_fwd": (_i, [_p, _p, _p] + [_i] * 11 + [_p]),
     "moma_dwconv_bwd_data": (_i, [_p, _p, _p] + [_i] * 11 + [_p]),
     "moma_dwconv_bwd_weight": (_i, [_p, _p, _p, _p, _z] + [_i] * 11 + [_p]),
+    "moma_dwconv_fwd_pre": (_i, [_p, _p, _p] + [_i] * 11 + [_p, _i, _p]),
+    "moma_dwconv_bwd_weight_pre": (_i, [_p, _p, _p, _p, _z] + [_i] * 11 + [_p, _i, _p]),
     "moma_plane_mean": (_i, [_p, _p, _i, _i, _i, _p]),
     "moma_se_gate_fwd": (_i, [_p, _p, _p, _i, _i, _i, _p]),
     "moma_se_gate_bwd": (_i, [_p, _p, _p, _p, _p, _i, _i, _i, _p]),
     "moma_bn_workspace_bytes": (_z, [_i]),
     "moma_bn_fwd": (_i, [_p, _p, _p, _p, _p, _p, _p, _p, _p, _z, _i, _i, _i, _i, _i, _i, _f, _f, _p, _p]),
     "moma_bn_bwd": (_i, [_p, _p, _p, _p, _p, _p, _p, _p, _p, _p, _z, _i, _i, _i, _i, _i, _i, _p, _p]),
+    "moma_bn_prepare": (_i, [_p, _p, _p, _p, _p, _p, _p, _p, _p, _z, _i, _i, _i, _i, _i, _f, _f, _p]),
     "moma_mha_bwd_workspace_bytes": (_z, [_i, _i, _i, _i]),
     "moma_mha_bwd": (_i, [_p, _p, _p, _p, _p, _p, _p, _p, _p, _p, _p, _p, _p, _z, _i, _i, _i, _i, _p]),
 }
diff --git a/moma_amd/backbones/efficientnet.py b/moma_amd/backbones/efficientnet.py
--- a/moma_amd/backbones/efficientnet.py
+++ b/moma_amd/backbones/efficientnet.py
@@ -8,6 +8,7 @@
 _DW_MODE = os.environ.get("MOMA_DW", "hip")
 _BN_MODE = os.environ.get("MOMA_BN", "hip")
 _SE_MODE = os.environ.get("MOMA_SE", "hip")
+_BNDW_FUSE = os.environ.get("MOMA_BNDW", "1")
 
 _B0_STAGES = [
     (1, 3, 1, 1, 32, 16, 0.25),
@@ -59,6 +60,10 @@
 _WCACHE = os.environ.get("MOMA_WCACHE", "1") == "1"
 
 
+def _same_pad(ih, iw, kh, kw, sh, sw):
+    return (max((math.ceil(ih / sh) - 1) * sh + kh - ih, 0), max((math.ceil(iw / sw) - 1) * sw + kw - iw, 0))
+
+
 class SamePadConv2d(nn.Conv2d):
 
     def __init__(self, cin, cout, kernel_size, stride=1, groups=1, bias=True):
@@ -76,13 +81,15 @@
             return w, b
         return self.weight, self.bias
 
+    def _is_depthwise(self):
+        return self.groups > 1 and self.groups == self.in_channels == self.out_channels and self.bias is None
+
     def forward(self, x):
         ih, iw = x.shape[-2:]
         kh, kw = self.kernel_size
         sh, sw = self.stride
-        ph = max((math.ceil(ih / sh) - 1) * sh + kh - ih, 0)
-        pw = max((math.ceil(iw / sw) - 1) * sw + kw - iw, 0)
-        depthwise = self.groups > 1 and self.groups == self.in_channels == self.out_channels and self.bias is None
+        ph, pw = _same_pad(ih, iw, kh, kw, sh, sw)
+        depthwise = self._is_depthwise()
         if depthwise and x.is_cuda and _DW_MODE == "hip" and kh == kw and sh == sw and self.dilation == (1, 1):
             from .. import ops
             if ops.dwconv_supported(kh, sh):
@@ -163,11 +170,40 @@
         self._project_conv = SamePadConv2d(mid, cout, 1, bias=False)
         self._bn2 = BatchNorm2d(cout, momentum=_BN_MOM, eps=_BN_EPS)
 
+    def _bn0_depthwise(self, e):
+        bn, dw = self._bn0, self._depthwise_conv
+        if not (_BNDW_FUSE in ("1", "grad") and _BN_MODE == "hip" and _DW_MODE == "hip" and e.is_cuda and bn.momentum is not None):
+            return None
+        if _BNDW_FUSE != "grad" and torch.is_grad_enabled() and (
+                e.requires_grad or dw.weight.requires_grad or bn.weight.requires_grad or bn.bias.requires_grad):
+            return None
+        (kh, kw), (sh, sw) = dw.kernel_size, dw.stride
+        if not (dw._is_depthwise() and kh == kw and sh == sw and dw.dilation == (1, 1)) or e.dtype not in (torch.float32, torch.bfloat16):
+            return None
+        if torch.is_autocast_enabled() and e.dtype != torch.get_autocast_dtype("cuda"):
+            return None
+        from .. import ops
+        if not ops.dwconv_supported(kh, sh):
+            return None
+        use_batch = bn.training or bn.running_mean is None
+        if bn.training and bn.track_running_stats and bn.num_batches_tracked is not None:
+            bn._nbt_pending += 1
+        ih, iw = e.shape[-2:]
+        ph, pw = _same_pad(ih, iw, kh, kw, sh, sw)
+        return ops.bn_act_dwconv(e, bn.weight, bn.bias, bn.running_mean, bn.running_var, use_batch, bn.momentum, bn.eps, "silu",
+                                 dw.weight, sh, ph // 2, pw // 2, math.ceil(ih / sh), math.ceil(iw / sw))
+
     def forward(self, x, drop_connect_rate=None):
         inp = x
+        d = None
         if self.expand != 1:
-            x = self._bn0(self._expand_conv(x), act="silu")
-        x, pooled = self._bn1(self._depthwise_conv(x), act="silu", want_mean=True)
+            x = self._expand_conv(x)
+            d = self._bn0_depthwise(x)
+            if d is None:
+                x = self._bn0(x, act="silu")
+        if d is None:
+            d = self._depthwise_conv(x)
+        x, pooled = self._bn1(d, act="silu", want_mean=True)
         s = self._se_expand(F.silu(self._se_reduce(pooled)))
         if _SE_MODE == "hip" and x.is_cuda and x.dtype in (torch.float32, torch.bfloat16):
             from .. import ops
diff --git a/moma_amd/csrc/api.hip b/moma_amd/csrc/api.hip
--- a/moma_amd/csrc/api.hip
+++ b/moma_amd/csrc/api.hip
@@ -460,6 +460,17 @@
                                 (float*)workspace, N, C, HW, dtype, act, training, momentum, eps, plane_mean, (hipStream_t)stream));
 }
 
+int moma_bn_prepare(const void* x, const float* gamma, const float* beta, float* running_mean, float* running_var,
+                    float* save_mean, float* save_invstd, float* scale_shift, void* workspace, size_t workspace_bytes, int N,
+                    int C, int HW, int dtype, int training, float momentum, float eps, moma_stream_t stream) {
+    if (!x || !save_mean || !save_invstd || !scale_shift) return MOMA_E_NULL;
+    if (!training && (!running_mean || !running_var)) return MOMA_E_NULL;
+    const int rc = bn_check(N, C, HW, dtype, MOMA_ACT_NONE, workspace, workspace_bytes);
+    if (rc != MOMA_OK) return rc;
+    return hip_rc(launch_bn_prepare(x, gamma, beta, running_mean, running_var, save_mean, save_invstd, scale_shift,
+                                    (float*)workspace, N, C, HW, dtype, training, momentum, eps, (hipStream_t)stream));
+}
+
 int moma_bn_bwd(const void* x, const void* dout, const float* gamma, const float* beta, const float* save_mean,
                 const float* save_invstd, void* dx, float* dgamma, float* dbeta, void* workspace,
                 size_t workspace_bytes, int N, int C, int HW, int dtype, int act, int training,
@@ -489,7 +500,20 @@
     if (!x || !w || !y) return MOMA_E_NULL;
     const int rc = dw_check(N, C, H, W, OH, OW, K, stride, pad_top, pad_left, dtype);
     if (rc != MOMA_OK) return rc;
-    return hip_rc(launch_dw_fwd(x, w, y, N, C, H, W, OH, OW, K, stride, pad_top, pad_left, dtype, (hipStream_t)stream));
+    return hip_rc(launch_dw_fwd(x, w, y, N, C, H, W, OH, OW, K, stride, pad_top, pad_left, dtype, nullptr, MOMA_ACT_NONE,
+                                (hipStream_t)stream));
+}
+
+static bool bad_act(int act) { return act != MOMA_ACT_NONE && act != MOMA_ACT_SILU && act != MOMA_ACT_RELU; }
+
+int moma_dwconv_fwd_pre(const void* x, const float* w, void* y, int N, int C, int H, int W, int OH, int OW, int K, int stride,
+                        int pad_top, int pad_left, int dtype, const float* scale_shift, int act, moma_stream_t stream) {
+    if (!x || !w || !y || !scale_shift) return MOMA_E_NULL;
+    const int rc = dw_check(N, C, H, W, OH, OW, K, stride, pad_top, pad_left, dtype);
+    if (rc != MOMA_OK) return rc;
+    if (bad_act(act)) return MOMA_E_DTYPE;
+    return hip_rc(launch_dw_fwd(x, w, y, N, C, H, W, OH, OW, K, stride, pad_top, pad_left, dtype, scale_shift, act,
+                                (hipStream_t)stream));
 }
 
 int moma_dwconv_bwd_data(const void* dy, const float* w, void* dx, int N, int C, int H, int W, int OH, int OW, int K,
@@ -508,7 +532,19 @@
     if (rc != MOMA_OK) return rc;
     if (workspace_bytes < moma_dwconv_workspace_bytes(C, K)) return MOMA_E_WORKSPACE;
     return hip_rc(launch_dw_bwd_weight(x, dy, dw, (float*)workspace, workspace_bytes / sizeof(float), N, C, H, W, OH, OW, K,
-                                       stride, pad_top, pad_left, dtype, (hipStream_t)stream));
+                                       stride, pad_top, pad_left, dtype, nullptr, MOMA_ACT_NONE, (hipStream_t)stream));
+}
+
+int moma_dwconv_bwd_weight_pre(const void* x, const void* dy, float* dw, void* workspace, size_t workspace_bytes, int N, int C,
+                               int H, int W, int OH, int OW, int K, int stride, int pad_top, int pad_left, int dtype,
+                               const float* scale_shift, int act, moma_stream_t stream) {
+    if (!x || !dy || !dw || !workspace || !scale_shift) return MOMA_E_NULL;
+    const int rc = dw_check(N, C, H, W, OH, OW, K, stride, pad_top, pad_left, dtype);
+    if (rc != MOMA_OK) return rc;
+    if (bad_act(act)) return MOMA_E_DTYPE;
+    if (workspace_bytes < moma_dwconv_workspace_bytes(C, K)) return MOMA_E_WORKSPACE;
+    return hip_rc(launch_dw_bwd_weight(x, dy, dw, (float*)workspace, workspace_bytes / sizeof(float), N, C, H, W, OH, OW, K,
+                                       stride, pad_top, pad_left, dtype, scale_shift, act, (hipStream_t)stream));
 }
 
 static int se_check(int NC, int HW, int dtype) {
diff --git a/moma_amd/csrc/bn.hip b/moma_amd/csrc/bn.hip
--- a/moma_amd/csrc/bn.hip
+++ b/moma_amd/csrc/bn.hip
@@ -69,11 +69,6 @@
     }
 };
 
-__device__ __forceinline__ float act_fwd(float y, int act) {
-    if (act == MOMA_ACT_SILU) return y / (1.f + __expf(-y));
-    if (act == MOMA_ACT_RELU) return fmaxf(y, 0.f);
-    return y;
-}
 __device__ __forceinline__ float act_grad(float y, int act) {
     if (act == MOMA_ACT_SILU) {
         const float s = 1.f / (1.f + __expf(-y));
@@ -340,14 +335,10 @@
 }
 
 template <typename T>
-hipError_t bn_fwd_t(const T* x, T* out, const float* gamma, const float* beta, float* rm, float* rv, float* save_mean,
-                    float* save_invstd, float* ws, int N, int C, int HW, int act, int training, float momentum,
-                    float eps, T* pmean, hipStream_t st) {
-    const int vec = pick_vec(HW, sizeof(T), x, out, nullptr);
+void bn_prepare_t(const T* x, const float* gamma, const float* beta, float* rm, float* rv, float* save_mean, float* save_invstd,
+                  float* scale_shift, float* partial, int N, int C, int HW, int vec, int training, float momentum, float eps,
+                  hipStream_t st) {
     const int S = training ? pick_splits(N, C, HW, vec) : 1;
-    float* scale_shift = ws;
-    float* partial = ws + 2 * (size_t)C;
-    const size_t nvec = (size_t)N * C * HW / vec;
     if (training) {
         dim3 grid(S, C);
         if (vec == 8) hipLaunchKernelGGL((bn_stats_kernel<T, 8>), grid, dim3(BN_THREADS), 0, st, x, partial, N, C, HW);
@@ -356,6 +347,18 @@
     }
     hipLaunchKernelGGL(bn_finalize_kernel, dim3((C + 3) / 4), dim3(256), 0, st, partial, S, gamma, beta, rm, rv,
                        save_mean, save_invstd, scale_shift, C, training, momentum, eps);
+}
+
+template <typename T>
+hipError_t bn_fwd_t(const T* x, T* out, const float* gamma, const float* beta, float* rm, float* rv, float* save_mean,
+                    float* save_invstd, float* ws, int N, int C, int HW, int act, int training, float momentum,
+                    float eps, T* pmean, hipStream_t st) {
+    const int vec = pick_vec(HW, sizeof(T), x, out, nullptr);
+    float* scale_shift = ws;
+    float* partial = ws + 2 * (size_t)C;
+    const size_t nvec = (size_t)N * C * HW / vec;
+    bn_prepare_t<T>(x, gamma, beta, rm, rv, save_mean, save_invstd, scale_shift, partial, N, C, HW, vec, training, momentum, eps,
+                    st);
     if (pmean) {
         long gp = ((long)N * C + BN_THREADS / 64 - 1) / (BN_THREADS / 64);
         if (gp > 256 * 32) gp = 256 * 32;
@@ -408,6 +411,18 @@
     return bn_fwd_t<float>((const float*)x, (float*)out, gamma, beta, rm, rv, save_mean, save_invstd, ws, N, C, HW, act,
                            training, momentum, eps, (float*)plane_mean, st);
 }
+hipError_t launch_bn_prepare(const void* x, const float* gamma, const float* beta, float* rm, float* rv, float* save_mean,
+                             float* save_invstd, float* scale_shift, float* ws, int N, int C, int HW, int dtype, int training,
+                             float momentum, float eps, hipStream_t st) {
+    float* partial = ws + 2 * (size_t)C;
+    if (dtype == MOMA_DT_BF16)
+        bn_prepare_t<bf16_raw>((const bf16_raw*)x, gamma, beta, rm, rv, save_mean, save_invstd, scale_shift, partial, N, C, HW,
+                               pick_vec(HW, sizeof(bf16_raw), x, nullptr, nullptr), training, momentum, eps, st);
+    else
+        bn_prepare_t<float>((const float*)x, gamma, beta, rm, rv, save_mean, save_invstd, scale_shift, partial, N, C, HW,
+                            pick_vec(HW, sizeof(float), x, nullptr, nullptr), training, momentum, eps, st);
+    return hipGetLastError();
+}
 hipError_t launch_bn_bwd(const void* x, const void* dout, const float* gamma, const float* beta, const float* save_mean,
                          const float* save_invstd, void* dx, float* dgamma, float* dbeta, float* ws, int N, int C, int HW,
                          int dtype, int act, int training, const void* dplane_mean, hipStream_t st) {
diff --git a/moma_amd/csrc/common.hpp b/moma_amd/csrc/common.hpp
--- a/moma_amd/csrc/common.hpp
+++ b/moma_amd/csrc/common.hpp
@@ -19,6 +19,12 @@
 __device__ __forceinline__ bf16_raw f32_to_bf16(float f) {
     __bf16 b = (__bf16)f;
     return *reinterpret_cast<bf16_raw*>(&b);
+}
+
+__device__ __forceinline__ float act_fwd(float y, int act) {
+    if (act == MOMA_ACT_SILU) return y / (1.f + __expf(-y));
+    if (act == MOMA_ACT_RELU) return fmaxf(y, 0.f);
+    return y;
 }
 
 __device__ __forceinline__ unsigned pack_bf16x2(float lo, float hi) {
@@ -210,6 +216,9 @@
 hipError_t launch_bn_fwd(const void* x, void* out, const float* gamma, const float* beta, float* rm, float* rv,
                          float* save_mean, float* save_invstd, float* ws, int N, int C, int HW, int dtype, int act,
                          int training, float momentum, float eps, void* plane_mean, hipStream_t st);
+hipError_t launch_bn_prepare(const void* x, const float* gamma, const float* beta, float* rm, float* rv, float* save_mean,
+                             float* save_invstd, float* scale_shift, float* ws, int N, int C, int HW, int dtype, int training,
+                             float momentum, float eps, hipStream_t st);
 hipError_t launch_bn_bwd(const void* x, const void* dout, const float* gamma, const float* beta, const float* save_mean,
                          const float* save_invstd, void* dx, float* dgamma, float* dbeta, float* ws, int N, int C, int HW,
                          int dtype, int act, int training, const void* dplane_mean, hipStream_t st);
@@ -217,11 +226,12 @@
 bool dwconv_supported(int K, int S);
 size_t dwconv_workspace_floats(int C, int K);
 hipError_t launch_dw_fwd(const void* x, const float* w, void* y, int N, int C, int H, int W, int OH, int OW, int K, int S,
-                         int pt, int pl, int dtype, hipStream_t st);
+                         int pt, int pl, int dtype, const float* scale_shift, int act, hipStream_t st);
 hipError_t launch_dw_bwd_data(const void* dy, const float* w, void* dx, int N, int C, int H, int W, int OH, int OW, int K,
                               int S, int pt, int pl, int dtype, hipStream_t st);
 hipError_t launch_dw_bwd_weight(const void* x, const void* dy, float* dw, float* ws, size_t ws_floats, int N, int C, int H,
-                                int W, int OH, int OW, int K, int S, int pt, int pl, int dtype, hipStream_t st);
+                                int W, int OH, int OW, int K, int S, int pt, int pl, int dtype, const float* scale_shift, int act,
+                                hipStream_t st);
 
 hipError_t launch_plane_mean(const void* x, void* out, int NC, int HW, int dtype, hipStream_t st);
 hipError_t launch_se_gate_fwd(const void* x, const void* s, void* out, int NC, int HW, int dtype, hipStream_t st);
diff --git a/moma_amd/csrc/dwconv.hip b/moma_amd/csrc/dwconv.hip
--- a/moma_amd/csrc/dwconv.hip
+++ b/moma_amd/csrc/dwconv.hip
@@ -66,9 +66,14 @@
     return q;
 }
 
-template <typename T, int VEC>
+template <typename T> __device__ __forceinline__ float storage_round(float v);
+template <> __device__ __forceinline__ float storage_round<float>(float v) { return v; }
+template <> __device__ __forceinline__ float storage_round<bf16_raw>(float v) { return bf16_to_f32(f32_to_bf16(v)); }
+
+template <typename T, int VEC, bool PRE = false>
 __device__ __forceinline__ void fill_tile(float* tile, const T* __restrict__ src, size_t plane_stride, int np, int H, int W,
-                                          int y0, int rows, int pitch, int xo, int lane, bool zero_rows) {
+                                          int y0, int rows, int pitch, int xo, int lane, bool zero_rows,
+                                          const float* ssl = nullptr, int ss_stride = 0, int act = 0) {
     const int ya = max(y0, 0), yb = min(y0 + rows, H);
     const int wv = W / VEC, nvpp = max(yb - ya, 0) * wv, total = nvpp * np;
     const float inv_nvpp = 1.0f / (float)max(nvpp, 1), inv_wv = 1.0f / (float)wv;
@@ -76,15 +81,23 @@
     for (int v0 = 0; v0 < total; v0 += 64 * U) {
         float val[U][VEC];
         int dst[U];
+        [[maybe_unused]] float sc[U], sf[U];
 #pragma unroll
         for (int u = 0; u < U; ++u) {
             const int v = min(v0 + u * 64 + lane, total - 1);
             const int p = fast_div(v, nvpp, inv_nvpp), e = v - p * nvpp, r = fast_div(e, wv, inv_wv), cv = e - r * wv;
             Vec<T, VEC>::ld(src + (size_t)p * plane_stride + (size_t)(ya + r) * W + cv * VEC, val[u]);
             dst[u] = (p * rows + (ya - y0) + r) * pitch + xo + cv * VEC;
+            if constexpr (PRE) { sc[u] = ssl[p * ss_stride]; sf[u] = ssl[p * ss_stride + 1]; }
         }
 #pragma unroll
         for (int u = 0; u < U; ++u) asm volatile("" : "+v"(val[u][0]));
+        if constexpr (PRE) {
+#pragma unroll
+            for (int u = 0; u < U; ++u)
+#pragma unroll
+                for (int j = 0; j < VEC; ++j) val[u][j] = storage_round<T>(act_fwd(fmaf(val[u][j], sc[u], sf[u]), act));
+        }
 #pragma unroll
         for (int u = 0; u < U; ++u)
             if (v0 + u * 64 + lane < total) lds_store<VEC>(tile + dst[u], val[u]);
@@ -98,14 +111,26 @@
     }
 }
 
-template <typename T, int K, int S, int R, bool FLIP, int VEC>
+__device__ __forceinline__ void stage_scale_shift(float* ssl, const float* __restrict__ ss, int plane0, int np, int C, int lane) {
+    if (lane < np) {
+        const int c = (plane0 + lane) % C;
+        ssl[2 * lane] = ss[2 * c];
+        ssl[2 * lane + 1] = ss[2 * c + 1];
+    }
+}
+
+template <typename T, int K, int S, int R, bool FLIP, int VEC, bool PRE>
 __global__ __launch_bounds__(DW_WAVES * 64) void dw_fwd_kernel(const T* __restrict__ x, const float* __restrict__ w,
-                                                             T* __restrict__ y, DwShape sh) {
+                                                             T* __restrict__ y, DwShape sh, const float* __restrict__ ss,
+                                                             int act) {
+    static_assert(!(PRE && FLIP), "the prologue belongs to the forward convolution");
     extern __shared__ float smem[];
     const int lane = threadIdx.x & 63, wave = threadIdx.x >> 6;
     const int tfl = sh.PB * sh.IR * sh.pitch;
-    float* tile = smem + wave * (tfl + ((sh.PB * K * K + 3) & ~3));
+    const int wfl = (sh.PB * K * K + 3) & ~3;
+    float* tile = smem + wave * (tfl + wfl + (PRE ? (2 * sh.PB + 3) & ~3 : 0));
     float* wl = tile + tfl;
+    [[maybe_unused]] float* ssl = wl + wfl;
     for (int i = lane; i < tfl; i += 64) tile[i] = 0.f;
     const int nitems = sh.ngroups * sh.nbands;
     const int nstrips = (sh.TH + R - 1) / R;
@@ -119,8 +144,9 @@
             const int p = i / (K * K), t = i - p * (K * K);
             wl[i] = w[((plane0 + p) % sh.C) * K * K + (FLIP ? K * K - 1 - t : t)];
         }
-        fill_tile<T, VEC>(tile, x + (size_t)plane0 * sh.H * sh.W, (size_t)sh.H * sh.W, np, sh.H, sh.W, oy0 * S - sh.pt, sh.IR,
-                          sh.pitch, XO, lane, sh.nbands > 1);
+        if constexpr (PRE) stage_scale_shift(ssl, ss, plane0, np, sh.C, lane);
+        fill_tile<T, VEC, PRE>(tile, x + (size_t)plane0 * sh.H * sh.W, (size_t)sh.H * sh.W, np, sh.H, sh.W, oy0 * S - sh.pt, sh.IR,
+                               sh.pitch, XO, lane, sh.nbands > 1, ssl, 2, act);
         __builtin_amdgcn_s_waitcnt(0xc07f);
         const int nwork = nstrips * sh.OW;
         const float inv_ow = 1.0f / (float)sh.OW;
@@ -161,15 +187,19 @@
     }
 }
 
-template <typename T, int K, int S, int OWT, bool FLIP, int VEC>
+template <typename T, int K, int S, int OWT, bool FLIP, int VEC, bool PRE>
 __global__ __launch_bounds__(DW_WAVES * 64) void dw_small_kernel(const T* __restrict__ x, const float* __restrict__ w,
-                                                               T* __restrict__ y, DwShape sh) {
+                                                               T* __restrict__ y, DwShape sh, const float* __restrict__ ss,
+                                                               int act) {
+    static_assert(!(PRE && FLIP), "the prologue belongs to the forward convolution");
     extern __shared__ float smem[];
     constexpr int IW = (OWT - 1) * S + K;
     const int lane = threadIdx.x & 63, wave = threadIdx.x >> 6;
     const int tfl = sh.PB * sh.IR * sh.pitch;
-    float* tile = smem + wave * (tfl + ((sh.PB * K * K + 3) & ~3));
+    const int wfl = (sh.PB * K * K + 3) & ~3;
+    float* tile = smem + wave * (tfl + wfl + (PRE ? (2 * sh.PB + 3) & ~3 : 0));
     float* wl = tile + tfl;
+    [[maybe_unused]] float* ssl = wl + wfl;
     for (int i = lane; i < tfl; i += 64) tile[i] = 0.f;
     const int p = lane / OWT, oy = lane - p * OWT;
     const int cbase = XO - sh.pl;
@@ -179,8 +209,9 @@
             const int pp = i / (K * K), t = i - pp * (K * K);
             wl[i] = w[((plane0 + pp) % sh.C) * K * K + (FLIP ? K * K - 1 - t : t)];
         }
-        fill_tile<T, VEC>(tile, x + (size_t)plane0 * sh.H * sh.W, (size_t)sh.H * sh.W, np, sh.H, sh.W, -sh.pt, sh.IR, sh.pitch,
-                          XO, lane, false);
+        if constexpr (PRE) stage_scale_shift(ssl, ss, plane0, np, sh.C, lane);
+        fill_tile<T, VEC, PRE>(tile, x + (size_t)plane0 * sh.H * sh.W, (size_t)sh.H * sh.W, np, sh.H, sh.W, -sh.pt, sh.IR, sh.pitch,
+                               XO, lane, false, ssl, 2, act);
         __builtin_amdgcn_s_waitcnt(0xc07f);
         if (p < np) {
             float wk[K * K];
@@ -264,16 +295,21 @@
     }
 }
 
-template <typename T, int K, int S, int R, int VEC, int GVEC, bool GDIRECT>
+template <typename T, int K, int S, int R, int VEC, int GVEC, bool GDIRECT, bool PRE>
 __global__ __launch_bounds__(DW_WAVES * 64) void dw_bwd_weight_kernel(const T* __restrict__ x, const T* __restrict__ dy,
-                                                                    float* __restrict__ partial, DwShape sh, int N) {
+                                                                    float* __restrict__ partial, DwShape sh, int N,
+                                                                    const float* __restrict__ ss, int act) {
     extern __shared__ float smem[];
     const int lane = threadIdx.x & 63, wave = threadIdx.x >> 6;
     const int xt = sh.PB * sh.IR * sh.pitch, gtn = GDIRECT ? 0 : sh.PB * sh.GR * sh.gpitch;
-    float* tile = smem + wave * (xt + gtn);
+    float* tile = smem + wave * (xt + gtn + (PRE ? 4 : 0));
     float* gt = tile + xt;
+    [[maybe_unused]] float* ssl = tile + xt + gtn;
     for (int i = lane; i < xt + gtn; i += 64) tile[i] = 0.f;
     const int c = blockIdx.y;
+    if constexpr (PRE) {
+        if (lane < 2) ssl[lane] = ss[2 * c + lane];
+    }
     const int nsplit = gridDim.x * DW_WAVES, split = blockIdx.x * DW_WAVES + wave;
     const int nstrips = (sh.TH + R - 1) / R;
     constexpr int CR = (R - 1) * S + K;
@@ -287,8 +323,8 @@
         const int grp = item / sh.nbands, band = item - grp * sh.nbands;
         const int n0 = grp * sh.PB, np = min(sh.PB, N - n0);
         const int oy0 = band * sh.TH;
-        fill_tile<T, VEC>(tile, x + ((size_t)n0 * sh.C + c) * sh.H * sh.W, xs, np, sh.H, sh.W, oy0 * S - sh.pt, sh.IR, sh.pitch, XO,
-                          lane, sh.nbands > 1);
+        fill_tile<T, VEC, PRE>(tile, x + ((size_t)n0 * sh.C + c) * sh.H * sh.W, xs, np, sh.H, sh.W, oy0 * S - sh.pt, sh.IR, sh.pitch,
+                               XO, lane, sh.nbands > 1, ssl, 0, act);
         if constexpr (!GDIRECT)
             fill_tile<T, GVEC>(gt, dy + ((size_t)n0 * sh.C + c) * sh.OH * sh.OW, gs, np, sh.OH, sh.OW, oy0, sh.GR, sh.gpitch, 0,
                                lane, sh.nbands > 1);
@@ -390,8 +426,9 @@
 
 template <typename T, int K, int S>
 hipError_t fwd_t(const T* x, const float* w, T* y, int NC, int C, int H, int W, int OH, int OW, int pt, int pl, bool flip,
-                 hipStream_t st) {
+                 const float* ss, int act, hipStream_t st) {
     constexpr int MAXV = 16 / sizeof(T);
+    if (flip && ss) return hipErrorInvalidValue;
     DwShape sh{};
     sh.NC = NC; sh.C = C; sh.H = H; sh.W = W; sh.OH = OH; sh.OW = OW; sh.pt = pt; sh.pl = pl;
     sh.pitch = round4(XO + max(W, (OW - 1) * S + K - pl) + 1);
@@ -401,14 +438,17 @@
         sh.PB = OW == 7 ? 8 : 4;
         sh.pitch |= 1;
         sh.ngroups = (NC + sh.PB - 1) / sh.PB;
-        const size_t lds = (size_t)DW_WAVES * (sh.PB * sh.IR * sh.pitch + round4(sh.PB * K * K)) * sizeof(float);
-        if (lds <= (size_t)LDS_BUDGET) {
+        const size_t lds0 = (size_t)DW_WAVES * (sh.PB * sh.IR * sh.pitch + round4(sh.PB * K * K)) * sizeof(float);
+        const size_t lds = lds0 + (ss ? (size_t)DW_WAVES * round4(2 * sh.PB) * sizeof(float) : 0);
+        if (lds0 <= (size_t)LDS_BUDGET) {
+            if (lds > (size_t)LDS_BUDGET) return hipErrorInvalidValue;
             const dim3 grid(grid_for(sh.ngroups)), block(DW_WAVES * 64);
             const int vec = 1;
-#define MOMA_DW_SMALL(OWT, FL) hipLaunchKernelGGL((dw_small_kernel<T, K, S, OWT, FL, V>), grid, block, lds, st, x, w, y, sh)
+#define MOMA_DW_SMALL(OWT, FL, PR) \
+    hipLaunchKernelGGL((dw_small_kernel<T, K, S, OWT, FL, V, PR>), grid, block, lds, st, x, w, y, sh, ss, act)
             MOMA_DW_VEC_SWITCH(vec, MAXV, {
-                if (OW == 7) { if (flip) MOMA_DW_SMALL(7, true); else MOMA_DW_SMALL(7, false); }
-                else { if (flip) MOMA_DW_SMALL(14, true); else MOMA_DW_SMALL(14, false); }
+                if (OW == 7) { if (flip) MOMA_DW_SMALL(7, true, false); else if (ss) MOMA_DW_SMALL(7, false, true); else MOMA_DW_SMALL(7, false, false); }
+                else { if (flip) MOMA_DW_SMALL(14, true, false); else if (ss) MOMA_DW_SMALL(14, false, true); else MOMA_DW_SMALL(14, false, false); }
             })
 #undef MOMA_DW_SMALL
             return hipGetLastError();
@@ -420,14 +460,17 @@
     sh.IR = (sh.TH - 1) * S + K;
     sh.PB = fit_planes(planes_per_item(OH, OW, sh.nbands), (long)sh.IR * sh.pitch);
     sh.ngroups = (NC + sh.PB - 1) / sh.PB;
-    const size_t lds = (size_t)DW_WAVES * (sh.PB * sh.IR * sh.pitch + round4(sh.PB * K * K)) * sizeof(float);
+    const size_t lds = (size_t)DW_WAVES * (sh.PB * sh.IR * sh.pitch + round4(sh.PB * K * K) + (ss ? round4(2 * sh.PB) : 0)) *
+                       sizeof(float);
     if (lds > (size_t)LDS_BUDGET) return hipErrorInvalidValue;
     const dim3 grid(grid_for((long)sh.ngroups * sh.nbands)), block(DW_WAVES * 64);
     const int vec = pick_vec(W, sizeof(T), x);
-#define MOMA_DW_GO(RR, FL) hipLaunchKernelGGL((dw_fwd_kernel<T, K, S, RR, FL, V>), grid, block, lds, st, x, w, y, sh)
+#define MOMA_DW_GO(RR, FL, PR) \
+    hipLaunchKernelGGL((dw_fwd_kernel<T, K, S, RR, FL, V, PR>), grid, block, lds, st, x, w, y, sh, ss, act)
     MOMA_DW_VEC_SWITCH(vec, MAXV, {
-        if (flip) { if (R == 4) MOMA_DW_GO(4, true); else if (R == 2) MOMA_DW_GO(2, true); else MOMA_DW_GO(1, true); }
-        else { if (R == 4) MOMA_DW_GO(4, false); else if (R == 2) MOMA_DW_GO(2, false); else MOMA_DW_GO(1, false); }
+        if (flip) { if (R == 4) MOMA_DW_GO(4, true, false); else if (R == 2) MOMA_DW_GO(2, true, false); else MOMA_DW_GO(1, true, false); }
+        else if (ss) { if (R == 4) MOMA_DW_GO(4, false, true); else if (R == 2) MOMA_DW_GO(2, false, true); else MOMA_DW_GO(1, false, true); }
+        else { if (R == 4) MOMA_DW_GO(4, false, false); else if (R == 2) MOMA_DW_GO(2, false, false); else MOMA_DW_GO(1, false, false); }
     })
 #undef MOMA_DW_GO
     return hipGetLastError();
@@ -460,7 +503,7 @@
 
 template <typename T, int K, int S>
 hipError_t bwd_weight_t(const T* x, const T* dy, float* dw, float* ws, size_t ws_floats, int N, int C, int H, int W, int OH,
-                        int OW, int pt, int pl, hipStream_t st) {
+                        int OW, int pt, int pl, const float* ss, int act, hipStream_t st) {
     constexpr int MAXV = 16 / sizeof(T);
     DwShape sh{};
     sh.NC = N * C; sh.C = C; sh.H = H; sh.W = W; sh.OH = OH; sh.OW = OW; sh.pt = pt; sh.pl = pl;
@@ -474,19 +517,22 @@
     sh.GR = gdirect ? 0 : sh.TH;
     sh.PB = fit_planes(min(planes_per_item(OH, OW, sh.nbands), N), (long)sh.IR * sh.pitch + (long)sh.GR * sh.gpitch);
     sh.ngroups = (N + sh.PB - 1) / sh.PB;
-    const size_t lds = (size_t)DW_WAVES * sh.PB * (sh.IR * sh.pitch + sh.GR * sh.gpitch) * sizeof(float);
+    const size_t lds = (size_t)DW_WAVES * (sh.PB * (sh.IR * sh.pitch + sh.GR * sh.gpitch) + (ss ? 4 : 0)) * sizeof(float);
     if (lds > (size_t)LDS_BUDGET) return hipErrorInvalidValue;
     long nsplit_wg = max(1L, min((long)(2048 + C - 1) / C, ((long)sh.ngroups * sh.nbands + DW_WAVES - 1) / DW_WAVES));
     while (nsplit_wg > 1 && (size_t)C * nsplit_wg * DW_WAVES * K * K > ws_floats) --nsplit_wg;
     if ((size_t)C * nsplit_wg * DW_WAVES * K * K > ws_floats) return hipErrorInvalidValue;
     const dim3 grid((unsigned)nsplit_wg, C), block(DW_WAVES * 64);
     const int vec = pick_vec(W, sizeof(T), x), gvec = pick_vec(OW, sizeof(T), dy);
-#define MOMA_DW_GO(RR, GV, GD) hipLaunchKernelGGL((dw_bwd_weight_kernel<T, K, S, RR, V, GV, GD>), grid, block, lds, st, x, dy, ws, sh, N)
+#define MOMA_DW_GO1(RR, GV, GD, PR) \
+    hipLaunchKernelGGL((dw_bwd_weight_kernel<T, K, S, RR, V, GV, GD, PR>), grid, block, lds, st, x, dy, ws, sh, N, ss, act)
+#define MOMA_DW_GO(RR, GV, GD) { if (ss) MOMA_DW_GO1(RR, GV, GD, true); else MOMA_DW_GO1(RR, GV, GD, false); }
     MOMA_DW_VEC_SWITCH(vec, MAXV, {
-        if (gdirect) { if (R == 4) MOMA_DW_GO(4, 1, true); else if (R == 2) MOMA_DW_GO(2, 1, true); else MOMA_DW_GO(1, 1, true); }
-        else if (gvec >= V) { if (R == 4) MOMA_DW_GO(4, V, false); else if (R == 2) MOMA_DW_GO(2, V, false); else MOMA_DW_GO(1, V, false); }
-        else { if (R == 4) MOMA_DW_GO(4, 1, false); else if (R == 2) MOMA_DW_GO(2, 1, false); else MOMA_DW_GO(1, 1, false); }
+        if (gdirect) { if (R == 4) MOMA_DW_GO(4, 1, true) else if (R == 2) MOMA_DW_GO(2, 1, true) else MOMA_DW_GO(1, 1, true) }
+        else if (gvec >= V) { if (R == 4) MOMA_DW_GO(4, V, false) else if (R == 2) MOMA_DW_GO(2, V, false) else MOMA_DW_GO(1, V, false) }
+        else { if (R == 4) MOMA_DW_GO(4, 1, false) else if (R == 2) MOMA_DW_GO(2, 1, false) else MOMA_DW_GO(1, 1, false) }
     })
+#undef MOMA_DW_GO1
 #undef MOMA_DW_GO
     const int total = C * K * K;
     hipLaunchKernelGGL(dw_bwd_weight_finalize_kernel, dim3((total + 255) / 256), dim3(256), 0, st, ws, dw, total,
@@ -506,13 +552,13 @@
     return hipErrorInvalidValue;
 
 hipError_t launch_dw_fwd(const void* x, const float* w, void* y, int N, int C, int H, int W, int OH, int OW, int K, int S,
-                         int pt, int pl, int dtype, hipStream_t st) {
+                         int pt, int pl, int dtype, const float* scale_shift, int act, hipStream_t st) {
     if (dtype == MOMA_DT_BF16) {
-#define CALL(KK, SS) fwd_t<bf16_raw, KK, SS>((const bf16_raw*)x, w, (bf16_raw*)y, N * C, C, H, W, OH, OW, pt, pl, false, st)
+#define CALL(KK, SS) fwd_t<bf16_raw, KK, SS>((const bf16_raw*)x, w, (bf16_raw*)y, N * C, C, H, W, OH, OW, pt, pl, false, scale_shift, act, st)
         MOMA_DW_DISPATCH(CALL)
 #undef CALL
     }
-#define CALL(KK, SS) fwd_t<float, KK, SS>((const float*)x, w, (float*)y, N * C, C, H, W, OH, OW, pt, pl, false, st)
+#define CALL(KK, SS) fwd_t<float, KK, SS>((const float*)x, w, (float*)y, N * C, C, H, W, OH, OW, pt, pl, false, scale_shift, act, st)
     MOMA_DW_DISPATCH(CALL)
 #undef CALL
 }
@@ -521,11 +567,11 @@
                               int S, int pt, int pl, int dtype, hipStream_t st) {
     if (S == 1) {
         if (dtype == MOMA_DT_BF16) {
-            if (K == 3) return fwd_t<bf16_raw, 3, 1>((const bf16_raw*)dy, w, (bf16_raw*)dx, N * C, C, OH, OW, H, W, 2 - pt, 2 - pl, true, st);
-            if (K == 5) return fwd_t<bf16_raw, 5, 1>((const bf16_raw*)dy, w, (bf16_raw*)dx, N * C, C, OH, OW, H, W, 4 - pt, 4 - pl, true, st);
+            if (K == 3) return fwd_t<bf16_raw, 3, 1>((const bf16_raw*)dy, w, (bf16_raw*)dx, N * C, C, OH, OW, H, W, 2 - pt, 2 - pl, true, nullptr, 0, st);
+            if (K == 5) return fwd_t<bf16_raw, 5, 1>((const bf16_raw*)dy, w, (bf16_raw*)dx, N * C, C, OH, OW, H, W, 4 - pt, 4 - pl, true, nullptr, 0, st);
         } else {
-            if (K == 3) return fwd_t<float, 3, 1>((const float*)dy, w, (float*)dx, N * C, C, OH, OW, H, W, 2 - pt, 2 - pl, true, st);
-            if (K == 5) return fwd_t<float, 5, 1>((const float*)dy, w, (float*)dx, N * C, C, OH, OW, H, W, 4 - pt, 4 - pl, true, st);
+            if (K == 3) return fwd_t<float, 3, 1>((const float*)dy, w, (float*)dx, N * C, C, OH, OW, H, W, 2 - pt, 2 - pl, true, nullptr, 0, st);
+            if (K == 5) return fwd_t<float, 5, 1>((const float*)dy, w, (float*)dx, N * C, C, OH, OW, H, W, 4 - pt, 4 - pl, true, nullptr, 0, st);
         }
         return hipErrorInvalidValue;
     }
@@ -540,13 +586,14 @@
 }
 
 hipError_t launch_dw_bwd_weight(const void* x, const void* dy, float* dw, float* ws, size_t ws_floats, int N, int C, int H,
-                                int W, int OH, int OW, int K, int S, int pt, int pl, int dtype, hipStream_t st) {
+                                int W, int OH, int OW, int K, int S, int pt, int pl, int dtype, const float* scale_shift, int act,
+                                hipStream_t st) {
     if (dtype == MOMA_DT_BF16) {
-#define CALL(KK, SS) bwd_weight_t<bf16_raw, KK, SS>((const bf16_raw*)x, (const bf16_raw*)dy, dw, ws, ws_floats, N, C, H, W, OH, OW, pt, pl, st)
+#define CALL(KK, SS) bwd_weight_t<bf16_raw, KK, SS>((const bf16_raw*)x, (const bf16_raw*)dy, dw, ws, ws_floats, N, C, H, W, OH, OW, pt, pl, scale_shift, act, st)
         MOMA_DW_DISPATCH(CALL)
 #undef CALL
     }
-#define CALL(KK, SS) bwd_weight_t<float, KK, SS>((const float*)x, (const float*)dy, dw, ws, ws_floats, N, C, H, W, OH, OW, pt, pl, st)
+#define CALL(KK, SS) bwd_weight_t<float, KK, SS>((const float*)x, (const float*)dy, dw, ws, ws_floats, N, C, H, W, OH, OW, pt, pl, scale_shift, act, st)
     MOMA_DW_DISPATCH(CALL)
 #undef CALL
 }
diff --git a/moma_amd/ops.py b/moma_amd/ops.py
--- a/moma_amd/ops.py
+++ b/moma_amd/ops.py
@@ -684,6 +684,76 @@
     return _DWConv.apply(x, weight, int(stride), int(pad_top), int(pad_left), int(out_h), int(out_w))
 
 
+class _BNActDWConv(torch.autograd.Function):
+    @staticmethod
+    def forward(ctx, x, weight, bias, running_mean, running_var, training, momentum, eps, act, w, stride, pad_top,
+                pad_left, out_h, out_w):
+        lib = _lib.load()
+        _dev(x, "x", dtype=None, contiguous=False)
+        _dev(w, "weight")
+        if x.dim() != 4 or x.dtype not in _DT_CODES or w.dim() != 4 or w.shape[1] != 1 or w.shape[0] != x.shape[1] \
+                or w.shape[2] != w.shape[3]:
+            raise ValueError(f"bn_act_dwconv: x {tuple(x.shape)} {x.dtype}, weight {tuple(w.shape)}")
+        x = x.contiguous()
+        w = w.contiguous()
+        N, Cc, H, W = x.shape
+        K = w.shape[2]
+        dev = x.device
+        save_mean = torch.empty(Cc, device=dev, dtype=torch.float32)
+        save_invstd = torch.empty(Cc, device=dev, dtype=torch.float32)
+        scale_shift = torch.empty(Cc, 2, device=dev, dtype=torch.float32)
+        ws = torch.empty(lib.moma_bn_workspace_bytes(Cc), device=dev, dtype=torch.uint8)
+        check(lib.moma_bn_prepare(_ptr(x), _ptr(weight), _ptr(bias), _ptr(running_mean), _ptr(running_var), _ptr(save_mean),
+                                  _ptr(save_invstd), _ptr(scale_shift), _ptr(ws), ws.numel(), N, Cc, H * W,
+                                  _DT_CODES[x.dtype], int(training), float(momentum), float(eps), _stream()), "moma_bn_prepare")
+        y = torch.empty(N, Cc, out_h, out_w, device=dev, dtype=x.dtype)
+        check(lib.moma_dwconv_fwd_pre(_ptr(x), _ptr(w), _ptr(y), N, Cc, H, W, out_h, out_w, K, stride, pad_top, pad_left,
+                                      _DT_CODES[x.dtype], _ptr(scale_shift), act, _stream()), "moma_dwconv_fwd_pre")
+        ctx.save_for_backward(x, weight, bias, save_mean, save_invstd, scale_shift, w)
+        ctx.cfg = (N, Cc, H, W, out_h, out_w, K, stride, pad_top, pad_left, act, int(training))
+        ctx.set_materialize_grads(False)
+        return y
+
+    @staticmethod
+    def backward(ctx, dy):
+        lib = _lib.load()
+        x, weight, bias, save_mean, save_invstd, scale_shift, w = ctx.saved_tensors
+        N, Cc, H, W, OH, OW, K, stride, pt, pl, act, training = ctx.cfg
+        dx = dgamma = dbeta = dw = None
+        if dy is None:
+            return (None,) * 15
+        dy = dy.contiguous()
+        if dy.dtype != x.dtype:
+            dy = dy.to(x.dtype)
+        dev, dt = x.device, _DT_CODES[x.dtype]
+        want_gamma = weight is not None and ctx.needs_input_grad[1]
+        want_beta = bias is not None and ctx.needs_input_grad[2]
+        if ctx.needs_input_grad[0] or want_gamma or want_beta:
+            da = torch.empty_like(x)
+            check(lib.moma_dwconv_bwd_data(_ptr(dy), _ptr(w), _ptr(da), N, Cc, H, W, OH, OW, K, stride, pt, pl, dt,
+                                           _stream()), "moma_dwconv_bwd_data")
+            dx = torch.empty_like(x) if ctx.needs_input_grad[0] else None
+            dgamma = torch.empty(Cc, device=dev, dtype=torch.float32) if want_gamma else None
+            dbeta = torch.empty(Cc, device=dev, dtype=torch.float32) if want_beta else None
+            ws = torch.empty(lib.moma_bn_workspace_bytes(Cc), device=dev, dtype=torch.uint8)
+            check(lib.moma_bn_bwd(_ptr(x), _ptr(da), _ptr(weight), _ptr(bias), _ptr(save_mean), _ptr(save_invstd), _ptr(dx),
+                                  _ptr(dgamma), _ptr(dbeta), _ptr(ws), ws.numel(), N, Cc, H * W, dt, act, training, None,
+                                  _stream()), "moma_bn_bwd")
+        if ctx.needs_input_grad[9]:
+            dw = torch.empty_like(w)
+            ws = torch.empty(lib.moma_dwconv_workspace_bytes(Cc, K), device=dev, dtype=torch.uint8)
+            check(lib.moma_dwconv_bwd_weight_pre(_ptr(x), _ptr(dy), _ptr(dw), _ptr(ws), ws.numel(), N, Cc, H, W, OH, OW, K,
+                                                 stride, pt, pl, dt, _ptr(scale_shift), act, _stream()),
+                  "moma_dwconv_bwd_weight_pre")
+        return dx, dgamma, dbeta, None, None, None, None, None, None, dw, None, None, None, None, None
+
+
+def bn_act_dwconv(x, weight, bias, running_mean, running_var, training: bool, momentum: float, eps: float, act, w_dw,
+                  stride: int, pad_top: int, pad_left: int, out_h: int, out_w: int):
+    return _BNActDWConv.apply(x, weight, bias, running_mean, running_var, bool(training), momentum, eps, ACT_CODES[act],
+                              w_dw, int(stride), int(pad_top), int(pad_left), int(out_h), int(out_w))
+
+
 class _PlaneMean(torch.autograd.Function):
     @staticmethod
     def forward(ctx, x):
```
